# tlinford/raytracer-challenge-rs

Measured on AMD Instinct MI355X. Metric: Mrays/s (primary+secondary) on 1920×1080/1000-sphere/depth-5; 1→8 GPU scaling, higher is better.
Workload: dtype f64; 1 GPU; c3: 1920x1080, floor plane + 1000 random spheres (splitmix64 seed 0x5EED0003), 1 light, reflect+refract depth 5; width=1920, height=1080, spheres=1000, depth=5, rays_per_frame=14667325, parallelism=1 GPU: wavefront pipeline; batches of 8 frames on 4 streams, frames_in_flight=32, batch=8, render_streams_n=4, render_streams=raw

## Files before the change

### raytracer-challenge-rs_amd/csrc/pybind/rtamd_py.cpp

```cpp
#include <pybind11/numpy.h>
#include <pybind11/operators.h>
#include <pybind11/pybind11.h>
#include <pybind11/stl.h>

#include <algorithm>
#include <cstring>
#include <thread>

#include "../host/obj_parser.hpp"
#include "../host/rt_world.hpp"
#include "../host/scene_parser.hpp"

namespace py = pybind11;
using namespace rt;

static py::dict stats_dict(const rt_stats& s) {
  py::dict d;
  d["rays_primary"] = s.rays_primary;
  d["rays_reflect"] = s.rays_reflect;
  d["rays_refract"] = s.rays_refract;
  d["rays_shadow"] = s.rays_shadow;
  d["sphere_tests"] = s.sphere_tests;
  d["plane_tests"] = s.plane_tests;
  if (s.sphere_disc_ge0 == RT_STATS_NOT_COUNTED) d["sphere_disc_ge0"] = py::none();
  else d["sphere_disc_ge0"] = s.sphere_disc_ge0;
  d["other_tests"] = s.other_tests;
  d["ms_kernel"] = s.ms_kernel;
  d["ms_total"] = s.ms_total;
  d["rays_shadow_traced"] = s.rays_shadow_traced;
  d["sphere_tests_executed"] = s.sphere_tests_executed;
  d["box_tests_executed"] = s.box_tests_executed;
  d["exhaustive"] = (bool)s.exhaustive;
  return d;
}

static uint32_t render_flags(bool want_stats, const py::object& exhaustive) {
  const bool ex = exhaustive.is_none() ? want_stats : exhaustive.cast<bool>();
  return ex ? (uint32_t)RT_RENDER_EXHAUSTIVE : 0u;
}

static py::bytes pod_bytes(const void* p, size_t n) { return py::bytes((const char*)p, n); }

static py::array_t<double> check_rays(py::array_t<double, py::array::c_style | py::array::forcecast> a,
                                      size_t width) {
  if (a.ndim() != 2 || (size_t)a.shape(1) != width)
    throw std::invalid_argument("expected an (n, " + std::to_string(width) + ") float64 array");
  return a;
}

static void parallel_copy(char* dst, const char* src, size_t n) {
  const size_t kMin = (size_t)4 << 20;
  const unsigned nt = n < kMin ? 1u : (unsigned)std::min<size_t>(8, std::max(1u, std::thread::hardware_concurrency() / 2));
  if (nt <= 1) {
    std::memcpy(dst, src, n);
    return;
  }
  const size_t part = ((n + nt - 1) / nt + 4095) & ~(size_t)4095;
  std::vector<std::thread> pool;
  unsigned t = 1;
  try {
    for (; t < nt && t * part < n; ++t)
      pool.emplace_back([=] { std::memcpy(dst + t * part, src + t * part, std::min(part, n - t * part)); });
  } catch (...) {
  }
  for (unsigned u = t; u < nt && u * part < n; ++u) std::memcpy(dst + u * part, src + u * part, std::min(part, n - u * part));
  std::memcpy(dst, src, std::min(part, n));
  for (std::thread& th : pool) th.join();
}

extern "C" int rtamd_tuning_set(const char* key, int value);
extern "C" int rtamd_stream_create(int cu_masked, void** out);
extern "C" int rtamd_nccl_unique_id(unsigned char* out, size_t size);
extern "C" int rtamd_nccl_comm_init(int nranks, const unsigned char* id, size_t size, int rank, int device,
                                    int timeout_ms, void** comm);
extern "C" int rtamd_nccl_comm_abort(void* comm);
extern "C" int rtamd_nccl_gather_f64(const double* send, double* recv, size_t count, int root, void* comm, void* stream);
extern "C" int rtamd_nccl_comm_destroy(void* comm);
extern "C" int rtamd_wf_profile(const rt_scene* s, int enable, double out[40]);
extern "C" int rtamd_wf_gen_counts(const rt_scene* s, unsigned* out, int max);
extern "C" int rtamd_pngz_kernel_times(const double* d_rgb, uint32_t width, uint32_t height, uint8_t* d_out, size_t cap,
                                       float* ms, void* stream);
extern "C" int rtamd_wf_plan(const rt_scene* s, long long out[16]);
extern "C" int rtamd_csg_plan(const rt_scene* s, long long out[6]);
extern "C" int rtamd_scene_tuning_set(const rt_scene* s, const char* key, int value);
extern "C" int rtamd_render_shard_host(const rt_scene* scene, const rt_camera_desc* camera, uint32_t max_depth,
                                       uint32_t aa_samples, uint32_t row_block, uint32_t shard, uint32_t n_shards,
                                       double* out_rgb, rt_stats* stats);

static py::object child_object(const GroupChild& c) {
  if (c.shape) return py::cast(*c.shape);
  if (c.group) return py::cast(*c.group);
  return py::cast(*c.csg);
}

PYBIND11_MODULE(_rtamd, m) {
  m.doc() = "MI355X-native render path of raytracer-challenge-rs (host API over the C-ABI)";
  py::register_exception<RtError>(m, "RtError");
  m.attr("EPSILON") = EPSILON;
  m.attr("ABI_VERSION") = RT_ABI_VERSION;
  m.def("equal", &equal);
  m.def("device_count", &rt_device_count);
  m.def("abi_version", &rt_abi_version);

  py::class_<Point>(m, "Point")
      .def(py::init<double, double, double>())
      .def_static("origin", &Point::origin)
      .def_readwrite("x", &Point::x).def_readwrite("y", &Point::y).def_readwrite("z", &Point::z)
      .def("__eq__", [](const Point& a, const Point& b) { return a == b; })
      .def("__add__", [](const Point& p, const Vector& v) { return p + v; })
      .def("__sub__", [](const Point& a, const Point& b) { return a - b; })
      .def("__sub__", [](const Point& p, const Vector& v) { return p - v; })
      .def("tuple", [](const Point& p) { return py::make_tuple(p.x, p.y, p.z); })
      .def("__repr__", [](const Point& p) { return "Point(" + std::to_string(p.x) + ", " + std::to_string(p.y) + ", " + std::to_string(p.z) + ")"; });
  py::class_<Vector>(m, "Vector")
      .def(py::init<double, double, double>())
      .def_readwrite("x", &Vector::x).def_readwrite("y", &Vector::y).def_readwrite("z", &Vector::z)
      .def("magnitude", &Vector::magnitude)
      .def("normalize", &Vector::normalize)
      .def("reflect", &Vector::reflect)
      .def("__eq__", [](const Vector& a, const Vector& b) { return a == b; })
      .def("__add__", [](const Vector& a, const Vector& b) { return a + b; })
      .def("__sub__", [](const Vector& a, const Vector& b) { return a - b; })
      .def("__neg__", [](const Vector& a) { return -a; })
      .def("__mul__", [](const Vector& a, double s) { return a * s; })
      .def("tuple", [](const Vector& p) { return py::make_tuple(p.x, p.y, p.z); })
      .def("__repr__", [](const Vector& p) { return "Vector(" + std::to_string(p.x) + ", " + std::to_string(p.y) + ", " + std::to_string(p.z) + ")"; });
  m.def("dot", &dot);
  m.def("cross", &cross);
  py::class_<Color>(m, "Color")
      .def(py::init<double, double, double>())
      .def_static("black", &Color::black)
      .def_static("white", &Color::white)
      .def_readwrite("red", &Color::red).def_readwrite("green", &Color::green).def_readwrite("blue", &Color::blue)
      .def("__eq__", [](const Color& a, const Color& b) { return a == b; })
      .def("tuple", [](const Color& c) { return py::make_tuple(c.red, c.green, c.blue); })
      .def("__repr__", [](const Color& c) { return "Color(" + std::to_string(c.red) + ", " + std::to_string(c.green) + ", " + std::to_string(c.blue) + ")"; });
  py::class_<Ray>(m, "Ray")
      .def(py::init<const Point&, const Vector&>())
      .def_readwrite("origin", &Ray::origin)
      .def_readwrite("direction", &Ray::direction)
      .def("position", &Ray::position)
      .def("transform", [](const Ray& r, const Matrix& mm) { return transform(r, mm); });

  py::class_<Matrix>(m, "Matrix")
      .def(py::init<int, int>())
      .def_static("identity", &Matrix::identity)
      .def_static("from_rows", [](const std::vector<std::vector<double>>& rows) {
        int r = (int)rows.size(), c = r ? (int)rows[0].size() : 0;
        Matrix mm(r, c);
        for (int i = 0; i < r; ++i) {
          if ((int)rows[i].size() != c) throw std::invalid_argument("ragged rows");
          for (int j = 0; j < c; ++j) mm(i, j) = rows[i][j];
        }
        return mm;
      })
      .def("rows", &Matrix::rows)
      .def("columns", &Matrix::columns)
      .def("__getitem__", [](const Matrix& mm, std::pair<int, int> ij) {
        if (ij.first < 0 || ij.first >= mm.rows() || ij.second < 0 || ij.second >= mm.columns())
          throw py::index_error();
        return mm(ij.first, ij.second);
      })
      .def("__setitem__", [](Matrix& mm, std::pair<int, int> ij, double v) {
        if (ij.first < 0 || ij.first >= mm.rows() || ij.second < 0 || ij.second >= mm.columns())
          throw py::index_error();
        mm(ij.first, ij.second) = v;
      })
      .def("transpose", &Matrix::transpose)
      .def("determinant", &Matrix::determinant)
      .def("submatrix", &Matrix::submatrix)
      .def("minor", &Matrix::minor)
      .def("cofactor", &Matrix::cofactor)
      .def("is_invertible", &Matrix::is_invertible)
      .def("inverse", [](const Matrix& mm) {
        if (!mm.is_invertible()) throw RtError(RT_ERR_NOT_INVERTIBLE, "matrix is not invertible");
        return mm.inverse();
      })
      .def("translate", &Matrix::translate)
      .def("scale", &Matrix::scale)
      .def("rotate_x", &Matrix::rotate_x)
      .def("rotate_y", &Matrix::rotate_y)
      .def("rotate_z", &Matrix::rotate_z)
      .def("shear", &Matrix::shear)
      .def("__eq__", [](const Matrix& a, const Matrix& b) { return a == b; })
      .def("__mul__", [](const Matrix& a, const Matrix& b) { return a * b; })
      .def("__mul__", [](const Matrix& a, const Point& p) { return a * p; })
      .def("__mul__", [](const Matrix& a, const Vector& v) { return a * v; })
      .def("to_list", [](const Matrix& mm) {
        std::vector<double> v(mm.data(), mm.data() + mm.rows() * mm.columns());
        return v;
      });
  m.def("translation", &translation);
  m.def("scaling", &scaling);
  m.def("rotation_x", &rotation_x);
  m.def("rotation_y", &rotation_y);
  m.def("rotation_z", &rotation_z);
  m.def("shearing", &shearing);
  m.def("view_transform", &view_transform);

  py::class_<Pattern>(m, "Pattern")
      .def_readonly("kind", &Pattern::kind)
      .def_readwrite("a", &Pattern::a)
      .def_readwrite("b", &Pattern::b)
      .def_readonly("transform", &Pattern::transform)
      .def_readonly("transform_inverse", &Pattern::transform_inverse)
      .def("set_transform", &Pattern::set_transform);
  m.def("test_pattern", &test_pattern);
  m.def("stripe_pattern", &stripe_pattern);
  m.def("gradient_pattern", &gradient_pattern);
  m.def("ring_pattern", &ring_pattern);
  m.def("checkers_pattern", &checkers_pattern);

  py::class_<Material>(m, "Material")
      .def(py::init<>())
      .def_readwrite("color", &Material::color)
      .def_readwrite("ambient", &Material::ambient)
      .def_readwrite("diffuse", &Material::diffuse)
      .def_readwrite("specular", &Material::specular)
      .def_readwrite("shininess", &Material::shininess)
      .def_readwrite("reflective", &Material::reflective)
      .def_readwrite("transparency", &Material::transparency)
      .def_readwrite("refractive_index", &Material::refractive_index)
      .def_readonly("has_pattern", &Material::has_pattern)
      .def_readonly("pattern", &Material::pattern)
      .def("set_pattern", &Material::set_pattern)
      .def("copy", [](const Material& mm) { return mm; });

  py::class_<PointLight>(m, "PointLight")
      .def(py::init<const Point&, const Color&>())
      .def_readwrite("position", &PointLight::position)
      .def_readwrite("intensity", &PointLight::intensity);

  py::class_<Shape>(m, "Shape")
      .def_readonly("kind", &Shape::kind)
      .def_readwrite("material", &Shape::material)
      .def_readwrite("minimum", &Shape::minimum)
      .def_readwrite("maximum", &Shape::maximum)
      .def_readwrite("closed", &Shape::closed)
      .def_readonly("transform", &Shape::transform)
      .def_readonly("transform_inverse", &Shape::transform_inverse)
      .def("transform_inverse_transpose", &Shape::transform_inverse_transpose)
      .def("set_transform", &Shape::set_transform)
      .def("set_material", &Shape::set_material)
      .def("no_shadow", &Shape::no_shadow)
      .def("has_shadow", &Shape::has_shadow)
      .def("get_bounds", [](const Shape& s) { return s.bbox; })
      .def("parent_space_bounds", &Shape::parent_space_bounds)
      .def_readonly("p1", &Shape::p1).def_readonly("p2", &Shape::p2).def_readonly("p3", &Shape::p3)
      .def_readonly("n1", &Shape::n1).def_readonly("n2", &Shape::n2).def_readonly("n3", &Shape::n3)
      .def_readonly("e1", &Shape::e1).def_readonly("e2", &Shape::e2).def_readonly("normal", &Shape::normal)
      .def("desc_bytes", [](const Shape& s) { rt_shape_desc d = to_desc(s); return pod_bytes(&d, sizeof d); });
  py::class_<Group>(m, "Group")
      .def(py::init<>())
      .def("add_child", [](Group& g, const Shape& s) { g.add_child(s); })
      .def("add_child", [](Group& g, const Group& c) { g.add_child(c); })
      .def("add_child", [](Group& g, const Csg& c) { g.add_child(c); })
      .def("set_transform", &Group::set_transform)
      .def("set_material", &Group::set_material)
      .def_readonly("transform", &Group::transform)
      .def_readonly("transform_inverse", &Group::transform_inverse)
      .def_readonly("material", &Group::material)
      .def("n_children", [](const Group& g) { return g.children.size(); })
      .def("child", [](const Group& g, size_t i) -> py::object {
        return child_object(g.children.at(i));
      })
      .def("get_bounds", [](const Group& g) { return g.bbox; })
      .def("parent_space_bounds", &Group::parent_space_bounds)
      .def("divide", &Group::divide, py::arg("threshold"));
  py::enum_<Operation>(m, "Operation")
      .value("Union", Operation::Union).value("Intersection", Operation::Intersection)
      .value("Difference", Operation::Difference);
  py::class_<Csg>(m, "Csg")
      .def(py::init([](Operation op, py::object l, py::object r) {
        auto child = [](py::object o) -> GroupChild {
          if (py::isinstance<Shape>(o)) return make_child(o.cast<const Shape&>());
          if (py::isinstance<Group>(o)) return make_child(o.cast<const Group&>());
          if (py::isinstance<Csg>(o)) return make_child(o.cast<const Csg&>());
          throw std::invalid_argument("Csg: left / right must be a Shape, a Group or a Csg");
        };
        const GroupChild a = child(l), b = child(r);
        auto with_left = [&](auto& lv) {
          if (b.shape) return Csg(op, lv, *b.shape);
          if (b.group) return Csg(op, lv, *b.group);
          return Csg(op, lv, *b.csg);
        };
        if (a.shape) return with_left(*a.shape);
        if (a.group) return with_left(*a.group);
        return with_left(*a.csg);
      }), py::arg("operation"), py::arg("left"), py::arg("right"))
      .def_property_readonly("operation", [](const Csg& c) { return c.operation; })
      .def_property_readonly("left", [](const Csg& c) { return child_object(c.left); })
      .def_property_readonly("right", [](const Csg& c) { return child_object(c.right); })
      .def("set_transform", &Csg::set_transform)
      .def("set_material", &Csg::set_material)
      .def_readonly("transform", &Csg::transform)
      .def_readonly("transform_inverse", &Csg::transform_inverse)
      .def_readonly("material", &Csg::material)
      .def("get_bounds", [](const Csg& c) { return c.bbox; })
      .def("parent_space_bounds", &Csg::parent_space_bounds)
      .def("divide", &Csg::divide, py::arg("threshold"));
  py::class_<BoundingBox>(m, "BoundingBox")
      .def(py::init<>())
      .def(py::init<const Point&, const Point&>())
      .def_readwrite("min", &BoundingBox::min)
      .def_readwrite("max", &BoundingBox::max)
      .def("add_point", &BoundingBox::add_point)
      .def("add_bounding_box", &BoundingBox::add_box)
      .def("contains_point", &BoundingBox::contains_point)
      .def("contains_bounding_box", &BoundingBox::contains_box)
      .def("transform", &BoundingBox::transform)
      .def("intersects", &BoundingBox::intersects)
      .def("split", &BoundingBox::split);
  m.def("Sphere", &Sphere);
  m.def("glass_sphere", &glass_sphere);
  m.def("Plane", &Plane);
  m.def("Cube", &Cube);
  m.def("Cylinder", &Cylinder, py::arg("minimum") = -std::numeric_limits<double>::infinity(),
        py::arg("maximum") = std::numeric_limits<double>::infinity(), py::arg("closed") = false);
  m.def("Triangle", &Triangle, py::arg("p1"), py::arg("p2"), py::arg("p3"));
  m.def("SmoothTriangle", &SmoothTriangle, py::arg("p1"), py::arg("p2"), py::arg("p3"), py::arg("n1"), py::arg("n2"),
        py::arg("n3"));
  py::class_<ObjParser>(m, "ObjParser")
      .def(py::init<>())
      .def("parse", &ObjParser::parse)
      .def("parse_line", &ObjParser::parse_line)
      .def_readonly("ignored", &ObjParser::ignored)
      .def_readonly("vertices", &ObjParser::vertices)
      .def_readonly("normals", &ObjParser::normals)
      .def("group", [](const ObjParser& p, const std::string& name) { return p.group(name); })
      .def("group_names", &ObjParser::group_names)
      .def("as_group", &ObjParser::as_group);
  m.def("parse_obj_file", &parse_obj_file, py::arg("path"));
  m.def("parse_obj_string", &parse_obj_string, py::arg("text"));
  m.def("Cone", &Cone, py::arg("minimum") = -std::numeric_limits<double>::infinity(),
        py::arg("maximum") = std::numeric_limits<double>::infinity(), py::arg("closed") = false);

  py::enum_<AASamples>(m, "AASamples")
      .value("X1", AASamples::X1).value("X2", AASamples::X2).value("X4", AASamples::X4)
      .value("X8", AASamples::X8).value("X16", AASamples::X16);
  py::class_<RenderOpts>(m, "RenderOpts")
      .def("num_threads", &RenderOpts::num_threads)
      .def("aa_samples", &RenderOpts::aa_samples)
      .def_property_readonly("samples", [](const RenderOpts& o) { return (int)o.samples; });

  py::class_<Canvas>(m, "Canvas")
      .def(py::init<size_t, size_t>())
      .def("width", &Canvas::width)
      .def("height", &Canvas::height)
      .def("get_pixel", &Canvas::get_pixel)
      .def("set_pixel", &Canvas::set_pixel)
      .def("to_ppm", [](const Canvas& c) { return py::bytes(c.to_ppm()); })
      .def("to_png", [](const Canvas& c) { return py::bytes(c.to_png()); })
      .def("save", &Canvas::save, py::arg("path"))
      .def("to_png_deflate", [](const Canvas& c) { return py::bytes(c.to_png_deflate()); })
      .def("save_compressed", &Canvas::save_compressed, py::arg("path"))
      .def("to_numpy", [](const Canvas& c) {
        py::array_t<double> a({(py::ssize_t)c.height(), (py::ssize_t)c.width(), (py::ssize_t)3});
        std::memcpy(a.mutable_data(), c.data(), c.width() * c.height() * 3 * sizeof(double));
        return a;
      });
  m.def("canvas_to_ppm", [](py::array_t<double, py::array::c_style | py::array::forcecast> rgb) {
    if (rgb.ndim() != 3 || rgb.shape(2) != 3) throw std::invalid_argument("expected (h, w, 3)");
    size_t len = 0;
    const uint32_t h = (uint32_t)rgb.shape(0), w = (uint32_t)rgb.shape(1);
    const size_t bound = (size_t)12 * w * h + h + 32;
    PyObject* obj = PyBytes_FromStringAndSize(nullptr, (Py_ssize_t)bound);
    if (!obj) throw py::error_already_set();
    int rc;
    {
      py::gil_scoped_release nogil;
      rc = rt_canvas_to_ppm(rgb.data(), w, h, PyBytes_AS_STRING(obj), bound, &len);
    }
    if (rc != RT_OK) {
      Py_DECREF(obj);
      check(rc, "rt_canvas_to_ppm");
    }
    if (_PyBytes_Resize(&obj, (Py_ssize_t)len) != 0) throw py::error_already_set();
    return py::reinterpret_steal<py::bytes>(obj);
  });
  m.def("canvas_to_ppm_device", [](uintptr_t d_rgb, uint32_t w, uint32_t h, uintptr_t d_out, size_t cap,
                                   uintptr_t stream) {
    size_t len = 0;
    {
      py::gil_scoped_release nogil;
      check(rt_canvas_to_ppm_device((const double*)d_rgb, w, h, (char*)d_out, cap, &len, (void*)stream),
// ... 172 lines not shown
      .def_property_readonly("field_of_view", &Camera::field_of_view)
      .def("ray_for_pixel", &Camera::ray_for_pixel)
      .def("desc_bytes", [](const Camera& c) { return pod_bytes(&c.desc(), sizeof(rt_camera_desc)); })
      .def("render", [](const Camera& c, const World& w, unsigned max_depth, bool want_stats, py::object exhaustive) {
        rt_stats st{};
        Canvas* out;
        const uint32_t flags = render_flags(want_stats, exhaustive);
        {
          py::gil_scoped_release nogil;
          out = new Canvas(c.render(w, max_depth, want_stats ? &st : nullptr, flags));
        }
        return py::make_tuple(std::unique_ptr<Canvas>(out), stats_dict(st));
      }, py::arg("world"), py::arg("max_depth") = 5, py::arg("want_stats") = true, py::arg("exhaustive") = py::none())
      .def("render_ppm", [](const Camera& c, const World& w, unsigned max_depth, unsigned aa_samples, bool want_stats) {
        rt_stats st{};
        py::object out;
        {
          py::gil_scoped_release nogil;
          c.render_ppm_with(w, max_depth, aa_samples, want_stats ? &st : nullptr, [&](const char* p, size_t n) {
            char* dst = nullptr;
            {
              py::gil_scoped_acquire gil;
              PyObject* b = PyBytes_FromStringAndSize(nullptr, (Py_ssize_t)n);
              if (!b) throw py::error_already_set();
              out = py::reinterpret_steal<py::object>(b);
              dst = PyBytes_AS_STRING(b);
            }
            parallel_copy(dst, p, n);
          });
        }
        return py::make_tuple(out, stats_dict(st));
      }, py::arg("world"), py::arg("max_depth") = 5, py::arg("aa_samples") = 1, py::arg("want_stats") = false)
      .def("render_ppm_into", [](const Camera& c, const World& w, py::buffer out, unsigned max_depth,
                                 unsigned aa_samples) {
        py::buffer_info bi = out.request(true);
        if (bi.ndim != 1 || bi.itemsize != 1) throw std::invalid_argument("expected a writable 1-D byte buffer");
        size_t len = 0;
        int rc;
        {
          py::gil_scoped_release nogil;
          rc = rt_render_ppm(w.scene(), &c.desc(), max_depth, aa_samples, (char*)bi.ptr, (size_t)bi.size, &len,
                             nullptr);
        }
        check(rc, "rt_render_ppm");
        return len;
      }, py::arg("world"), py::arg("out"), py::arg("max_depth") = 5, py::arg("aa_samples") = 1)
      .def("render_png", [](const Camera& c, const World& w, unsigned max_depth, unsigned aa_samples, bool want_stats) {
        rt_stats st{};
        py::object out;
        {
          py::gil_scoped_release nogil;
          c.render_png_with(w, max_depth, aa_samples, want_stats ? &st : nullptr, [&](const char* p, size_t n) {
            char* dst = nullptr;
            {
              py::gil_scoped_acquire gil;
              PyObject* b = PyBytes_FromStringAndSize(nullptr, (Py_ssize_t)n);
              if (!b) throw py::error_already_set();
              out = py::reinterpret_steal<py::object>(b);
              dst = PyBytes_AS_STRING(b);
            }
            parallel_copy(dst, p, n);
          });
        }
        return py::make_tuple(out, stats_dict(st));
      }, py::arg("world"), py::arg("max_depth") = 5, py::arg("aa_samples") = 1, py::arg("want_stats") = false)
      .def("render_png_into", [](const Camera& c, const World& w, py::buffer out, unsigned max_depth,
                                 unsigned aa_samples) {
        py::buffer_info bi = out.request(true);
        if (bi.ndim != 1 || bi.itemsize != 1) throw std::invalid_argument("expected a writable 1-D byte buffer");
        size_t len = 0;
        int rc;
        {
          py::gil_scoped_release nogil;
          rc = rt_render_png(w.scene(), &c.desc(), max_depth, aa_samples, (uint8_t*)bi.ptr, (size_t)bi.size, &len,
                             nullptr);
        }
        check(rc, "rt_render_png");
        return len;
      }, py::arg("world"), py::arg("out"), py::arg("max_depth") = 5, py::arg("aa_samples") = 1)
      .def("render_png_deflate", [](const Camera& c, const World& w, unsigned max_depth, unsigned aa_samples,
                                    bool want_stats) {
        rt_stats st{};
        py::object out;
        {
          py::gil_scoped_release nogil;
          c.render_png_deflate_with(w, max_depth, aa_samples, want_stats ? &st : nullptr, [&](const char* p, size_t n) {
            py::gil_scoped_acquire gil;
            out = py::bytes(p, n);
          });
        }
        return py::make_tuple(out, stats_dict(st));
      }, py::arg("world"), py::arg("max_depth") = 5, py::arg("aa_samples") = 1, py::arg("want_stats") = false)
      .def("render_png_deflate_into", [](const Camera& c, const World& w, py::buffer out, unsigned max_depth,
                                         unsigned aa_samples) {
        py::buffer_info bi = out.request(true);
        if (bi.ndim != 1 || bi.itemsize != 1) throw std::invalid_argument("expected a writable 1-D byte buffer");
        size_t len = 0;
        int rc;
        {
          py::gil_scoped_release nogil;
          rc = rt_render_png_deflate(w.scene(), &c.desc(), max_depth, aa_samples, (uint8_t*)bi.ptr, (size_t)bi.size,
                                     &len, nullptr);
        }
        check(rc, "rt_render_png_deflate");
        return len;
      }, py::arg("world"), py::arg("out"), py::arg("max_depth") = 5, py::arg("aa_samples") = 1)
      .def_readwrite("render_opts", &Camera::render_opts, py::return_value_policy::reference_internal)
      .def("render_multithreaded", [](const Camera& c, const World& w, unsigned max_depth, bool want_stats,
                                      py::object exhaustive) {
        rt_stats st{};
        Canvas* out;
        const uint32_t flags = render_flags(want_stats, exhaustive);
        {
          py::gil_scoped_release nogil;
          out = new Canvas(c.render_multithreaded(w, max_depth, want_stats ? &st : nullptr, flags));
        }
        return py::make_tuple(std::unique_ptr<Canvas>(out), stats_dict(st));
      }, py::arg("world"), py::arg("max_depth") = 5, py::arg("want_stats") = true, py::arg("exhaustive") = py::none())
      .def("render_shard_device", [](const Camera& c, const World& w, unsigned max_depth, unsigned row_block,
                                     unsigned shard, unsigned n_shards, uintptr_t d_out, uintptr_t stream,
                                     bool want_stats, unsigned aa_samples, py::object exhaustive) {
        rt_stats st{};
        int rc;
        const uint32_t flags = render_flags(want_stats, exhaustive);
        {
          py::gil_scoped_release nogil;
          rc = rt_render_shard_device_ex(w.scene(), &c.desc(), max_depth, aa_samples, row_block, shard, n_shards,
                                         flags, (double*)d_out, (void*)stream, want_stats ? &st : nullptr);
        }
        check(rc, "rt_render_shard_device");
        return stats_dict(st);
      }, py::arg("world"), py::arg("max_depth"), py::arg("row_block"), py::arg("shard"), py::arg("n_shards"),
         py::arg("d_out"), py::arg("stream") = 0, py::arg("want_stats") = false, py::arg("aa_samples") = 1,
         py::arg("exhaustive") = py::none())
      .def("render_multi", [](const Camera& c, std::vector<World*> worlds, unsigned max_depth, unsigned row_block,
                              unsigned aa_samples, bool want_stats) {
        std::vector<rt_scene*> sc;
        for (size_t i = 0; i < worlds.size(); ++i) sc.push_back(const_cast<rt_scene*>(worlds[i]->scene((int)i)));
        Canvas* out = new Canvas(c.hsize(), c.vsize(), Canvas::Uninit{});
        rt_stats st{};
        int rc;
        {
          py::gil_scoped_release nogil;
          rc = rt_render_multi(sc.data(), (int)sc.size(), &c.desc(), max_depth, aa_samples, row_block, out->data(),
                               want_stats ? &st : nullptr);
        }
        if (rc != RT_OK) { delete out; check(rc, "rt_render_multi"); }
        return py::make_tuple(std::unique_ptr<Canvas>(out), stats_dict(st));
      }, py::arg("worlds"), py::arg("max_depth") = 5, py::arg("row_block") = 8, py::arg("aa_samples") = 1,
         py::arg("want_stats") = true);
  m.def("shard_rows", &rt_shard_rows);
  m.def("host_buffer", [](size_t bytes) {
    void* p = rt_host_buffer_alloc(bytes);
    if (!p) throw RtError(RT_ERR_HOST, std::string("rt_host_buffer_alloc: ") + rt_last_error());
    py::capsule owner(p, [](void* q) { rt_host_buffer_free(q); });
    return py::array_t<uint8_t>({(py::ssize_t)bytes}, {(py::ssize_t)1}, (uint8_t*)p, owner);
  }, py::arg("bytes"));
  m.def("_render_shard_host", [](const World& w, const Camera& c, unsigned max_depth, unsigned row_block,
                                 unsigned shard, unsigned n_shards,
                                 py::array_t<double, py::array::c_style> out, unsigned aa_samples, bool want_stats) {
    if (out.ndim() != 3 || (size_t)out.shape(0) != c.vsize() || (size_t)out.shape(1) != c.hsize() || out.shape(2) != 3)
      throw std::invalid_argument("expected a (vsize, hsize, 3) float64 canvas");
    double* p = out.mutable_data();
    rt_stats st{};
    int rc;
    {
      py::gil_scoped_release nogil;
      rc = rtamd_render_shard_host(w.scene(), &c.desc(), max_depth, aa_samples, row_block, shard, n_shards, p,
                                   want_stats ? &st : nullptr);
    }
    check(rc, "rtamd_render_shard_host");
    return stats_dict(st);
  }, py::arg("world"), py::arg("camera"), py::arg("max_depth"), py::arg("row_block"), py::arg("shard"),
     py::arg("n_shards"), py::arg("out"), py::arg("aa_samples") = 1, py::arg("want_stats") = false);
  m.def("render_frames_device", [](const World& w, std::vector<const Camera*> cams, unsigned max_depth,
                                   unsigned row_block, unsigned shard, unsigned n_shards, std::vector<uintptr_t> d_outs,
                                   uintptr_t stream, bool want_stats, unsigned aa_samples) {
    if (cams.size() != d_outs.size()) throw std::invalid_argument("one device buffer per camera");
    std::vector<rt_camera_desc> descs;
    for (const Camera* c : cams) descs.push_back(c->desc());
    std::vector<double*> outs;
    for (uintptr_t p : d_outs) outs.push_back((double*)p);
    rt_stats st{};
    int rc;
    {
      py::gil_scoped_release nogil;
      rc = rt_render_frames_device(w.scene(), descs.data(), (uint32_t)descs.size(), max_depth, aa_samples, row_block,
                                   shard, n_shards, outs.data(), (void*)stream, want_stats ? &st : nullptr);
    }
    check(rc, "rt_render_frames_device");
    return stats_dict(st);
  }, py::arg("world"), py::arg("cameras"), py::arg("max_depth"), py::arg("row_block"), py::arg("shard"),
     py::arg("n_shards"), py::arg("d_outs"), py::arg("stream") = 0, py::arg("want_stats") = false,
     py::arg("aa_samples") = 1);
  m.def("pattern_rows", &rt_pattern_rows);
  m.def("render_block_pattern_device", [](const World& w, std::vector<const Camera*> cams, unsigned max_depth,
                                          unsigned row_block, unsigned period, uint64_t mask,
                                          std::vector<uintptr_t> d_outs, uintptr_t stream, bool want_stats,
                                          unsigned aa_samples, bool exhaustive) {
    if (cams.size() != d_outs.size()) throw std::invalid_argument("one device buffer per camera");
    std::vector<rt_camera_desc> descs;
    for (const Camera* c : cams) descs.push_back(c->desc());
    std::vector<double*> outs;
    for (uintptr_t p : d_outs) outs.push_back((double*)p);
    rt_stats st{};
    int rc;
    {
      py::gil_scoped_release nogil;
      rc = rt_render_block_pattern_device(w.scene(), descs.data(), (uint32_t)descs.size(), max_depth, aa_samples,
                                          row_block, period, mask, exhaustive ? RT_RENDER_EXHAUSTIVE : 0u,
                                          outs.data(), (void*)stream, want_stats ? &st : nullptr);
    }
    check(rc, "rt_render_block_pattern_device");
    return stats_dict(st);
  }, py::arg("world"), py::arg("cameras"), py::arg("max_depth"), py::arg("row_block"), py::arg("period"),
     py::arg("mask"), py::arg("d_outs"), py::arg("stream") = 0, py::arg("want_stats") = false,
     py::arg("aa_samples") = 1, py::arg("exhaustive") = false);

  py::register_exception<SceneParserError>(m, "SceneParserError");
  py::register_exception<yaml::ParseError>(m, "YamlError");
  py::class_<SceneParser>(m, "SceneParser")
      .def(py::init<>())
      .def("load_file", &SceneParser::load_file)
      .def("load_str", &SceneParser::load_str, py::arg("text"), py::arg("name") = "<string>")
      .def_readonly("messages", &SceneParser::messages)
      .def_property_readonly("camera", [](const SceneParser& p) -> py::object {
        if (!p.scene().camera) return py::none();
        return py::cast(*p.scene().camera);
      })
      .def_property_readonly("lights", [](const SceneParser& p) { return p.scene().lights; })
      .def_property_readonly("shapes", [](const SceneParser& p) { return p.scene().shapes; })
      .def_property_readonly("materials", [](const SceneParser& p) { return p.scene().materials; })
      .def_property_readonly("transforms", [](const SceneParser& p) { return p.scene().transforms; })
      .def("build_world", &SceneParser::build_world)
      .def("render", [](const SceneParser& p, unsigned max_depth) {
        rt_stats st{};
        Canvas* out;
        {
          py::gil_scoped_release nogil;
          out = new Canvas(p.render(max_depth, &st));
        }
        return py::make_tuple(std::unique_ptr<Canvas>(out), stats_dict(st));
      }, py::arg("max_depth") = 5)
      .def("render_to", &SceneParser::render_to, py::arg("path"), py::arg("max_depth") = 5,
           py::arg("compress") = false);
  m.def("_wf_gen_counts", [](const World& w) {
    unsigned o[66] = {0};
    const int n = rtamd_wf_gen_counts(w.scene(), o, 66);
    if (n < 0) check(n, "wf_gen_counts");
    py::list l;
    for (int i = 0; i < n; ++i) l.append(o[i]);
    return l;
  }, py::arg("world"));
  m.def("_wf_profile", [](const World& w, int enable, bool read) {
    double o[40] = {0};
    check(rtamd_wf_profile(w.scene(), enable, read ? o : nullptr), "wf_profile");
    py::dict d;
    if (read) {
      const char* cls[5] = {"primary", "closest", "shadow", "prep", "combine"};
      py::dict ms, rays, disc;
      for (int i = 0; i < 5; ++i) ms[cls[i]] = o[i];
      for (int i = 0; i < 3; ++i) { rays[cls[i]] = o[5 + i]; disc[cls[i]] = o[8 + i]; }
      d["ms"] = ms; d["rays"] = rays; d["disc"] = disc;
      d["n_diag"] = o[11]; d["n_gen"] = o[12]; d["n_planes"] = o[13]; d["n_lights"] = o[14];
      d["n_quads"] = o[15];
      py::dict tests, boxes;
      for (int i = 0; i < 3; ++i) { tests[cls[i]] = o[16 + i]; boxes[cls[i]] = o[19 + i]; }
      d["tests"] = tests; d["boxes"] = boxes; d["bvh"] = (bool)o[22]; d["n_bvh_nodes"] = o[23]; d["bvh_depth"] = o[24];
      d["n_obvh_nodes"] = o[25]; d["n_other_culled"] = o[26];
      d["lb_res"] = o[27]; d["lb_items"] = o[28];
      py::dict shr, sht;
      shr["primary"] = o[29]; shr["closest"] = o[30]; sht["primary"] = o[31]; sht["closest"] = o[32];
      d["shadow_rays_in"] = shr; d["shadow_tests_in"] = sht; d["fused"] = (bool)o[33];
      d["n_bvh_wide"] = (int)o[34]; d["wide_stack"] = (int)o[35];
      d["n_lbvh_nodes"] = (int)o[36]; d["n_line_culled"] = (int)o[37];
      d["lane_primary"] = (int)o[38]; d["lane_secondary"] = (int)o[39];
    }
    return d;
  }, py::arg("world"), py::arg("enable") = -1, py::arg("read") = true);
  m.def("_wf_plan", [](const World& w) {
    long long o[16] = {0};
    check(rtamd_wf_plan(w.scene(), o), "wf_plan");
    py::dict d;
    const char* which[2] = {"primary", "secondary"};
    for (int i = 0; i < 2; ++i) {
      py::dict p;
      p["lane"] = (int)o[4 * i];
      p["lds_flags"] = (int)o[4 * i + 1];
      p["lds_spheres"] = (o[4 * i + 1] & 1) != 0;
      p["lds_deltas"] = (o[4 * i + 1] & 2) != 0;
      p["n_top"] = o[4 * i + 2];
      p["dyn"] = o[4 * i + 3];
      d[which[i]] = p;
    }
    py::dict t;
    t["records"] = o[8]; t["depth"] = o[9]; t["nodes"] = o[10]; t["ran"] = o[11] != 0;
    d["triangles"] = t;
    d["n_tris"] = o[12];
    d["n_csg_units"] = o[13];
    d["n_alias_members"] = o[14];
    d["n_alias_classes"] = o[15];
    return d;
  }, py::arg("world"));
  m.def("_csg_plan", [](const World& w) {
    long long o[6] = {0};
    check(rtamd_csg_plan(w.scene(), o), "csg_plan");
    py::dict d;
    d["units"] = o[0]; d["records"] = o[1]; d["remainder"] = o[2];
    d["nodes"] = o[3]; d["depth"] = o[4]; d["ran"] = o[5] != 0;
    return d;
  }, py::arg("world"));
  m.def("_tuning_set", [](const std::string& k, int v) { check(rtamd_tuning_set(k.c_str(), v), "tuning"); });
  m.def("_nccl_unique_id", []() {
    std::string id(128, '\0');
    check(rtamd_nccl_unique_id((unsigned char*)&id[0], id.size()), "nccl unique id");
    return py::bytes(id);
  });
  m.def("_nccl_comm_init", [](int nranks, py::bytes id, int rank, int device, int timeout_ms) {
    std::string s = id;
    void* comm = nullptr;
    int rc;
    {
      py::gil_scoped_release nogil;
      rc = rtamd_nccl_comm_init(nranks, (const unsigned char*)s.data(), s.size(), rank, device, timeout_ms, &comm);
    }
    check(rc, "nccl comm init");
    return (uintptr_t)comm;
  }, py::arg("nranks"), py::arg("id"), py::arg("rank"), py::arg("device"), py::arg("timeout_ms") = 60000);
  m.def("_nccl_comm_abort", [](uintptr_t comm) { check(rtamd_nccl_comm_abort((void*)comm), "nccl comm abort"); });
  m.def("_nccl_gather_f64", [](uintptr_t send, uintptr_t recv, size_t count, int root, uintptr_t comm, uintptr_t stream) {
    check(rtamd_nccl_gather_f64((const double*)send, (double*)recv, count, root, (void*)comm, (void*)stream), "nccl gather");
  });
  m.def("_nccl_comm_destroy", [](uintptr_t comm) { check(rtamd_nccl_comm_destroy((void*)comm), "nccl comm destroy"); });
  m.def("_stream_create", [](bool cu_masked) {
    void* st = nullptr;
    check(rtamd_stream_create(cu_masked ? 1 : 0, &st), "stream");
    return (uintptr_t)st;
  });
}
```

### raytracer-challenge-rs_amd/csrc/rt_api.cpp

```cpp
#include "rt_api_internal.hpp"
#include "rt_pow.hpp"

namespace rtapi {

thread_local std::string g_err;
int g_bvh_leaf = 0;
int g_bvh_ct = 70;
int g_lb_res = -1;
constexpr int kCsgHierMinDefault = 16;
int g_csg_hier_min = kCsgHierMinDefault;
int g_csg_wide_all = 0;
std::mutex g_tune_mu;
WfTuning g_tune_defaults;

namespace {
std::mutex g_pin_mu;
std::vector<std::pair<void*, size_t>> g_pin_live, g_pin_free;
size_t g_pin_free_bytes = 0;
constexpr size_t kPinPoolBytes = (size_t)1 << 30;
}

bool pinned_block(const void* p, size_t n) {
  std::lock_guard<std::mutex> lk(g_pin_mu);
  for (const auto& b : g_pin_live)
    if ((const char*)p >= (const char*)b.first && (const char*)p + n <= (const char*)b.first + b.second) return true;
  return false;
}

}

using namespace rtapi;

extern "C" __attribute__((visibility("hidden"))) int rtamd_fail(int code, const char* msg) noexcept {
  try {
    g_err = msg ? msg : "";
  } catch (...) {
    g_err.clear();
  }
  return code;
}

extern "C" {

const char* rt_last_error(void) { return g_err.c_str(); }

int rtamd_wf_profile(const rt_scene* cs, int enable, double out[40]) {
  if (!cs) return fail(RT_ERR_INVALID_ARGUMENT, "null scene");
  rt_scene* s = const_cast<rt_scene*>(cs);
  std::lock_guard<std::mutex> lk(s->mu);
  if (enable >= 0) {
    s->prof_on = enable != 0;
    s->prof_mask = enable > 1 ? (enable >> 1) : (1 << WF_NCLASS) - 1;
    for (rt_scene::WfSlot& w : s->wfs) w.wf->set_profiling(s->prof_on, s->prof_mask);
  }
  if (out) {
    RT_DEVICE(s->device);
    WfProfile p{};
    double ms_sum[WF_NCLASS] = {};
    size_t frames = 0;
    for (rt_scene::WfSlot& w : s->wfs) {
      WfProfile q;
      RT_HIP(w.wf->last_profile(&q));
      const size_t f = w.wf->profiled_frames();
      for (int c = 0; c < WF_NCLASS; ++c) ms_sum[c] += q.ms[c] * (double)(f > 1 ? f : 1);
      frames += f > 1 ? f : (f == 1 ? 1 : 0);
      if (&w == s->last_wf) p = q;
    }
    for (int c = 0; c < WF_NCLASS; ++c) p.ms[c] = frames ? ms_sum[c] / (double)frames : 0.0;
    for (int i = 0; i < 5; ++i) out[i] = p.ms[i];
    for (int i = 0; i < 3; ++i) { out[5 + i] = p.rays[i]; out[8 + i] = p.disc[i]; }
    out[11] = s->dev.n_diag; out[12] = s->dev.n_gen; out[13] = s->dev.n_planes;
    out[14] = s->dev.n_lights; out[15] = s->dev.n_quads;
    for (int i = 0; i < 3; ++i) {
      out[16 + i] = p.bvh ? p.tests[i] : p.rays[i] * s->dev.n_diag;
      out[19 + i] = p.boxes[i];
    }
    out[22] = p.bvh;
    out[23] = s->dev.n_bvh;
    out[24] = s->dev.bvh_depth;
    out[25] = s->dev.n_obvh;
    out[26] = s->dev.n_orec;
    out[27] = s->dev.lb_cells ? s->dev.lb_res : 0;
    out[28] = s->dev.lb_cells ? s->dev.lb_n_items : 0;
    for (int i = 0; i < 2; ++i) { out[29 + i] = p.sh_rays[i]; out[31 + i] = p.sh_tests[i]; }
    out[33] = p.fused;
    out[34] = s->dev.bvhw ? s->dev.n_bvhw : 0;
    out[35] = s->dev.bvhw ? s->dev.bvhw_stack : 0;
    out[36] = s->dev.n_lbvh;
    out[37] = s->dev.n_lrec;
    out[38] = s->last_wf ? p.lane_primary : -1;
    out[39] = s->last_wf ? p.lane_secondary : -1;
  }
  return RT_OK;
}

int rtamd_wf_plan(const rt_scene* cs, long long out[16]) {
  if (!cs || !out) return fail(RT_ERR_INVALID_ARGUMENT, "null scene or output");
  rt_scene* s = const_cast<rt_scene*>(cs);
  std::lock_guard<std::mutex> lk(s->mu);
  const WfImagePlan none{};
  const WfImagePlan* pl[2] = {s->last_wf ? &s->last_wf->wf->plan_primary() : &none,
                              s->last_wf ? &s->last_wf->wf->plan_secondary() : &none};
  for (int i = 0; i < 2; ++i) {
    out[4 * i] = pl[i]->lane;
    out[4 * i + 1] = (long long)pl[i]->lds_flags;
    out[4 * i + 2] = (long long)pl[i]->n_top;
    out[4 * i + 3] = (long long)pl[i]->dyn;
  }
  out[8] = s->dev.n_tbvh > 0 ? s->dev.n_trec : 0;
  out[9] = s->dev.tbvh_depth;
  out[10] = s->dev.n_tbvh;
  out[11] = s->dev.n_tbvh > 0 && (pl[0]->lane >= 0 || pl[1]->lane >= 0) ? 1 : 0;
  out[12] = s->dev.n_tris;
  out[13] = s->dev.n_csg_units;
  out[14] = s->dev.n_alias_rec;
  out[15] = s->dev.n_alias_cls;
  return RT_OK;
}

int rtamd_csg_plan(const rt_scene* cs, long long out[6]) {
  if (!cs || !out) return fail(RT_ERR_INVALID_ARGUMENT, "null scene or output");
  rt_scene* s = const_cast<rt_scene*>(cs);
  std::lock_guard<std::mutex> lk(s->mu);
  const bool fused =
      s->last_wf && (s->last_wf->wf->plan_primary().lane >= 0 || s->last_wf->wf->plan_secondary().lane >= 0);
  out[0] = s->dev.n_csg_units;
  out[1] = s->dev.n_ubvh > 0 ? s->dev.n_urec : 0;
  out[2] = s->dev.n_fx_units;
  out[3] = s->dev.n_ubvh;
  out[4] = s->dev.ubvh_depth;
  out[5] = s->dev.n_ubvh > 0 && fused ? 1 : 0;
  return RT_OK;
}

int rtamd_wf_gen_counts(const rt_scene* cs, unsigned* out, int max) {
  if (!cs || !out || max < 0) return fail(RT_ERR_INVALID_ARGUMENT, "null scene or output");
  rt_scene* s = const_cast<rt_scene*>(cs);
  std::lock_guard<std::mutex> lk(s->mu);
  if (!s->last_wf) return 0;
  RT_DEVICE(s->device);
  std::vector<unsigned> rays;
  RT_HIP(s->last_wf->wf->gen_counts(rays));
  const int n = std::min<int>((int)rays.size(), max);
  for (int i = 0; i < n; ++i) out[i] = rays[(size_t)i];
  return n;
}

int rtamd_tuning_set(const char* key, int value) {
  return guarded([&]() -> int {
  if (key && std::strcmp(key, "lb_res") == 0) {
    if (value < -1 || value > 512) return fail(RT_ERR_INVALID_ARGUMENT, "lb_res must be in [-1, 512]");
    g_lb_res = value;
    return RT_OK;
  }
  if (key && std::strcmp(key, "bvh_ct") == 0) {
    if (value < 1 || value > 10000) return fail(RT_ERR_INVALID_ARGUMENT, "bvh_ct must be in [1, 10000]");
    g_bvh_ct = value;
    return RT_OK;
  }
  if (key && std::strcmp(key, "bvh_leaf") == 0) {
    if (value < 0 || value > kBvhLeafMax) return fail(RT_ERR_INVALID_ARGUMENT, "bvh_leaf must be in [0, 127]");
    g_bvh_leaf = value;
    return RT_OK;
  }
  if (key && std::strcmp(key, "csg_hier_min") == 0) {
    if (value < 0 || value > 65536)
      return fail(RT_ERR_INVALID_ARGUMENT, "csg_hier_min must be in [1, 65536], or 0 for the default");
    g_csg_hier_min = value ? value : kCsgHierMinDefault;
    return RT_OK;
  }
  if (key && std::strcmp(key, "csg_wide_all") == 0) {
    if (value < 0 || value > 1) return fail(RT_ERR_INVALID_ARGUMENT, "csg_wide_all must be 0 or 1");
    g_csg_wide_all = value;
    return RT_OK;
  }
  std::lock_guard<std::mutex> lk(g_tune_mu);
  const int r = wf_tuning_apply(g_tune_defaults, key, value);
  if (r < 0) return fail(RT_ERR_INVALID_ARGUMENT, std::string("bad value for tuning key ") + key);
  if (r == 0) return fail(RT_ERR_INVALID_ARGUMENT, "unknown tuning key");
  return RT_OK;
  });
}
int rtamd_scene_tuning_set(const rt_scene* scene, const char* key, int value) {
  return guarded([&]() -> int {
  if (!scene) return fail(RT_ERR_INVALID_ARGUMENT, "null scene");
  rt_scene* s = const_cast<rt_scene*>(scene);
  std::lock_guard<std::mutex> lk(s->mu);
  const int r = wf_tuning_apply(s->tune, key, value);
  if (r < 0) return fail(RT_ERR_INVALID_ARGUMENT, std::string("bad value for tuning key ") + (key ? key : ""));
  if (r == 0) return fail(RT_ERR_INVALID_ARGUMENT, "unknown render-time tuning key (scene-creation keys: "
                                                   "rtamd_tuning_set before the scene is created)");
  return RT_OK;
  });
}
int rtamd_stream_create(int cu_masked, void** out) {
  if (!out) return fail(RT_ERR_INVALID_ARGUMENT, "null pointer");
  hipStream_t st = nullptr;
  if (cu_masked) {
    int dev = 0, n_cu = 0;
    RT_HIP(hipGetDevice(&dev));
    RT_HIP(hipDeviceGetAttribute(&n_cu, hipDeviceAttributeMultiprocessorCount, dev));
    std::vector<uint32_t> mask((size_t)(n_cu + 31) / 32, 0xFFFFFFFFu);
    RT_HIP(hipExtStreamCreateWithCUMask(&st, (uint32_t)mask.size(), mask.data()));
  } else {
    RT_HIP(hipStreamCreateWithFlags(&st, hipStreamNonBlocking));
  }
  *out = st;
  return RT_OK;
}
int rt_abi_version(void) { return RT_ABI_VERSION; }
size_t rt_sizeof_shape_desc(void) { return sizeof(rt_shape_desc); }
size_t rt_sizeof_camera_desc(void) { return sizeof(rt_camera_desc); }
size_t rt_sizeof_stats(void) { return sizeof(rt_stats); }
size_t rt_sizeof_node_desc(void) { return sizeof(rt_node_desc); }
static_assert(sizeof(rt_shape_desc) == 680 && sizeof(rt_camera_desc) == 160 && sizeof(rt_stats) == 112,
              "ABI struct sizes (include/rt_render.h, INTEGRATION.md)");

void* rt_host_buffer_alloc(size_t bytes) {
  if (bytes == 0) {
    g_err = "rt_host_buffer_alloc: zero bytes";
    return nullptr;
  }
  try {
    std::lock_guard<std::mutex> lk(g_pin_mu);
    for (size_t i = 0; i < g_pin_free.size(); ++i)
      if (g_pin_free[i].second >= bytes && g_pin_free[i].second <= bytes + bytes / 4) {
        const auto b = g_pin_free[i];
        g_pin_free.erase(g_pin_free.begin() + (long)i);
        g_pin_free_bytes -= b.second;
        g_pin_live.push_back(b);
        return b.first;
      }
    void* p = nullptr;
    if (hipHostMalloc(&p, bytes, hipHostMallocPortable | hipHostMallocMapped) != hipSuccess || !p) {
      (void)hipGetLastError();
      g_err = "rt_host_buffer_alloc: hipHostMalloc failed";
      return nullptr;
    }
    g_pin_live.emplace_back(p, bytes);
    return p;
  } catch (...) {
    g_err = "out of memory";
    return nullptr;
  }
}

void rt_host_buffer_free(void* p) {
  if (!p) return;
  try {
    std::lock_guard<std::mutex> lk(g_pin_mu);
    for (size_t i = 0; i < g_pin_live.size(); ++i)
      if (g_pin_live[i].first == p) {
        const auto b = g_pin_live[i];
        g_pin_live.erase(g_pin_live.begin() + (long)i);
        if (g_pin_free_bytes + b.second <= kPinPoolBytes) {
          g_pin_free.push_back(b);
          g_pin_free_bytes += b.second;
        } else {
          (void)hipHostFree(b.first);
        }
        return;
      }
  } catch (...) {
  }
}

int rt_scene_check(const rt_scene* scene) {
  return guarded([&]() -> int {
  if (!scene) return fail(RT_ERR_INVALID_ARGUMENT, "null scene");
  rt_scene* s = const_cast<rt_scene*>(scene);
  std::lock_guard<std::mutex> lk(s->mu);
  RT_DEVICE(s->device);
  for (rt_scene::WfSlot& w : s->wfs)
    if (w.done) RT_HIP(hipEventSynchronize(w.done));
  return check_faults(s);
  });
}

int rt_device_count(void) {
  return guarded([&]() -> int {
  int n = 0;
  if (hipGetDeviceCount(&n) != hipSuccess) return 0;
  return n;
  });
}

int rt_matrix_inverse(const double m[16], double out[16]) {
  return guarded([&]() -> int {
  if (!m || !out) return fail(RT_ERR_INVALID_ARGUMENT, "null pointer");
  rt::Matrix a = rt::Matrix::from_slice(4, 4, m);
  if (!a.is_invertible()) return fail(RT_ERR_NOT_INVERTIBLE, "matrix is not invertible (matrix.rs:139)");
  rt::Matrix inv = a.inverse();
  std::memcpy(out, inv.data(), 16 * sizeof(double));
  return RT_OK;
  });
}

int rt_camera_init(uint32_t hsize, uint32_t vsize, double field_of_view, const double transform[16],
                   rt_camera_desc* out) {
  return guarded([&]() -> int {
  if (!out || hsize == 0 || vsize == 0) return fail(RT_ERR_INVALID_ARGUMENT, "bad camera size");
  const double half_view = std::tan(field_of_view / 2.0);
  const double aspect = (double)hsize / (double)vsize;
  double half_width, half_height;
  if (aspect >= 1.0) {
    half_width = half_view;
    half_height = half_view / aspect;
  } else {
    half_width = half_view * aspect;
    half_height = half_view;
  }
  out->hsize = hsize;
  out->vsize = vsize;
  out->pixel_size = half_width * 2.0 / (double)hsize;
  out->half_width = half_width;
  out->half_height = half_height;
  if (transform) {
    int rc = rt_matrix_inverse(transform, out->inverse);
    if (rc != RT_OK) return rc;
  } else {
    rt::Matrix id = rt::Matrix::identity(4, 4);
    std::memcpy(out->inverse, id.data(), sizeof out->inverse);
  }
  return RT_OK;
  });
}

uint32_t rt_shard_rows(uint32_t vsize, uint32_t row_block, uint32_t shard, uint32_t n_shards) {
  if (row_block == 0 || n_shards == 0 || shard >= n_shards) return 0;
  uint32_t rows = 0;
  for (uint32_t blk = shard; (uint64_t)blk * row_block < vsize; blk += n_shards) {
    uint32_t y0 = blk * row_block;
    rows += std::min(row_block, vsize - y0);
  }
  return rows;
}

uint32_t rt_pattern_rows(uint32_t vsize, uint32_t row_block, uint32_t period, uint64_t mask) {
  if (row_block == 0 || !valid_pattern(period, mask)) return 0;
  uint32_t rows = 0;
  for (uint64_t blk = 0; blk * row_block < vsize; ++blk)
    if ((mask >> (blk % period)) & 1u) rows += std::min<uint32_t>(row_block, vsize - (uint32_t)(blk * row_block));
  return rows;
}

void rtamd_pow_host(const double* x, const double* y, size_t n, double* out) {
  for (size_t i = 0; i < n; ++i) out[i] = rtamd::pow_glibc(x[i], y[i]);
}
int rtamd_pow_device(const double* d_x, const double* d_y, size_t n, double* d_out, void* stream) {
  return guarded([&]() -> int {
  if (n >= (1ull << 31)) return fail(RT_ERR_INVALID_ARGUMENT, "batch too large");
  RT_HIP(launch_pow(d_x, d_y, (int)n, d_out, (hipStream_t)stream));
  RT_HIP(hipStreamSynchronize((hipStream_t)stream));
  return RT_OK;
  });
}

}
```

### raytracer-challenge-rs_amd/csrc/rt_render.cpp

```cpp
#include "rt_api_internal.hpp"

using namespace rtapi;

extern "C" {

int rt_render_shard_device(const rt_scene* scene, const rt_camera_desc* camera, uint32_t max_depth,
                           uint32_t aa_samples, uint32_t row_block, uint32_t shard, uint32_t n_shards,
                           double* d_out_rgb, void* stream, rt_stats* stats) {
  return guarded([&]() -> int {
  return rt_render_shard_device_ex(scene, camera, max_depth, aa_samples, row_block, shard, n_shards, 0, d_out_rgb,
                                   stream, stats);
  });
}

int rt_render_shard_device_ex(const rt_scene* scene, const rt_camera_desc* camera, uint32_t max_depth,
                              uint32_t aa_samples, uint32_t row_block, uint32_t shard, uint32_t n_shards,
                              uint32_t flags, double* d_out_rgb, void* stream, rt_stats* stats) {
  return guarded([&]() -> int {
  if (!scene || !camera || !d_out_rgb) return fail(RT_ERR_INVALID_ARGUMENT, "null pointer");
  if (row_block == 0 || n_shards == 0 || shard >= n_shards)
    return fail(RT_ERR_INVALID_ARGUMENT, "bad shard specification");
  if (camera->hsize == 0 || camera->vsize == 0) return fail(RT_ERR_INVALID_ARGUMENT, "empty camera");
  rt_scene* s = const_cast<rt_scene*>(scene);
  std::unique_lock<std::mutex> lk(s->mu);
  auto t0 = std::chrono::steady_clock::now();
  RT_DEVICE(s->device);
  const uint32_t rows = rt_shard_rows(camera->vsize, row_block, shard, n_shards);
  const uint64_t n_tasks = (uint64_t)rows * camera->hsize * aa_samples;
  if (n_tasks >= (1ull << 31)) return fail(RT_ERR_INVALID_ARGUMENT, "shard too large");
  hipStream_t st = (hipStream_t)stream;
  RenderCall call(&lk);
  call.flags = flags;
  call.stats = call.time = stats != nullptr;
  RenderResult r;
  int rc = run_render(s, WfJob::camera_shard(to_dev_camera(*camera), (uint32_t)n_tasks, aa_samples, max_depth,
                                             d_out_rgb, row_block, shard, n_shards), st, call, &r);
  if (rc != RT_OK) return rc;
  if (stats)
    fill_stats(stats, r.stats, r.ms,
               std::chrono::duration<double, std::milli>(std::chrono::steady_clock::now() - t0).count());
  return RT_OK;
  });
}

namespace {
int render_frames(const rt_scene* scene, const rt_camera_desc* cameras, uint32_t n_frames, uint32_t max_depth,
                  uint32_t aa_samples, uint32_t row_block, uint32_t shard, uint32_t n_shards, uint32_t blk_period,
                  uint64_t blk_mask, uint32_t flags, double* const* d_out_rgb, void* stream, rt_stats* stats) {
  if (!scene || (n_frames && (!cameras || !d_out_rgb))) return fail(RT_ERR_INVALID_ARGUMENT, "null pointer");
  if (row_block == 0 || n_shards == 0 || shard >= n_shards)
    return fail(RT_ERR_INVALID_ARGUMENT, "bad shard specification");
  if (blk_period && !valid_pattern(blk_period, blk_mask))
    return fail(RT_ERR_INVALID_ARGUMENT, "bad block pattern (period 1..64, a non-empty mask below 2^period)");
  if (!valid_aa(aa_samples)) return fail(RT_ERR_INVALID_ARGUMENT, "aa_samples must be 1, 2, 4, 8 or 16");
  for (uint32_t f = 0; f < n_frames; ++f) {
    if (!d_out_rgb[f]) return fail(RT_ERR_INVALID_ARGUMENT, "null pointer");
    if (cameras[f].hsize == 0 || cameras[f].vsize == 0) return fail(RT_ERR_INVALID_ARGUMENT, "empty camera");
    if (cameras[f].hsize != cameras[0].hsize || cameras[f].vsize != cameras[0].vsize)
      return fail(RT_ERR_INVALID_ARGUMENT, "the frames of a batch must share hsize and vsize");
  }
  if (n_frames == 0) {
    if (stats) std::memset(stats, 0, sizeof *stats);
    return RT_OK;
  }
  rt_scene* s = const_cast<rt_scene*>(scene);
  std::unique_lock<std::mutex> lk(s->mu);
  auto t0 = std::chrono::steady_clock::now();
  RT_DEVICE(s->device);
  const uint32_t rows = blk_period ? rt_pattern_rows(cameras[0].vsize, row_block, blk_period, blk_mask)
                                  : rt_shard_rows(cameras[0].vsize, row_block, shard, n_shards);
  const uint64_t per = (uint64_t)rows * cameras[0].hsize * aa_samples;
  const uint64_t padded = (per + 63) & ~(uint64_t)63;
  if (padded >= (1ull << 31)) return fail(RT_ERR_INVALID_ARGUMENT, "shard too large");
  hipStream_t st = (hipStream_t)stream;
  const bool batch = !stats && !(flags & RT_RENDER_EXHAUSTIVE) && fast_path(s) && per > 0;
  DevStats sum{};
  float ms_sum = 0.f;
  const uint32_t per_pass = (uint32_t)std::max<uint64_t>(1, std::min<uint64_t>(kMaxFrames, ((uint64_t)1 << 25) / std::max<uint64_t>(padded, 1)));
  RenderCall call(&lk);
  call.flags = flags;
  call.stats = call.time = stats != nullptr;
  for (uint32_t f0 = 0; f0 < n_frames;) {
    const uint32_t nf = batch ? std::min<uint32_t>(per_pass, n_frames - f0) : 1u;
    FrameTable tab{};
    for (uint32_t f = 0; f < nf; ++f) {
      tab.cam[f] = to_dev_camera(cameras[f0 + f]);
      tab.out[f] = d_out_rgb[f0 + f];
    }
    WfJob job = WfJob::camera_shard(tab.cam[0], (uint32_t)per, aa_samples, max_depth, tab.out[0], row_block, shard,
                                    n_shards);
    job.blk_period = blk_period;
    job.blk_mask = blk_mask;
    if (nf > 1) job.batch = &tab;
    job.n_frames = nf;
    RenderResult r;
    int rc = run_render(s, job, st, call, &r);
    if (rc != RT_OK) return rc;
    if (stats) {
      add_stats(sum, r.stats);
      ms_sum += r.ms;
    }
    f0 += nf;
  }
  if (stats)
    fill_stats(stats, sum, ms_sum, std::chrono::duration<double, std::milli>(std::chrono::steady_clock::now() - t0).count());
  return RT_OK;
}
}

int rt_render_frames_device(const rt_scene* scene, const rt_camera_desc* cameras, uint32_t n_frames,
                            uint32_t max_depth, uint32_t aa_samples, uint32_t row_block, uint32_t shard,
                            uint32_t n_shards, double* const* d_out_rgb, void* stream, rt_stats* stats) {
  return guarded([&]() -> int {
  return render_frames(scene, cameras, n_frames, max_depth, aa_samples, row_block, shard, n_shards, 0, 0, 0,
                       d_out_rgb, stream, stats);
  });
}

int rt_render_block_pattern_device(const rt_scene* scene, const rt_camera_desc* cameras, uint32_t n_frames,
                                   uint32_t max_depth, uint32_t aa_samples, uint32_t row_block, uint32_t period,
                                   uint64_t mask, uint32_t flags, double* const* d_out_rgb, void* stream,
                                   rt_stats* stats) {
  return guarded([&]() -> int {
  if (period == 0) return fail(RT_ERR_INVALID_ARGUMENT, "bad block pattern (period 1..64)");
  if (flags & ~(uint32_t)RT_RENDER_EXHAUSTIVE) return fail(RT_ERR_INVALID_ARGUMENT, "unknown render flags");
  return render_frames(scene, cameras, n_frames, max_depth, aa_samples, row_block, 0, 1, period, mask, flags,
                       d_out_rgb, stream, stats);
  });
}

}

namespace rtapi {
namespace {
struct BandPlan {
  int bands = 0;
  uint32_t rb = 0, nb = 0;
  uint32_t y0[kMaxBands + 1] = {};
  uint64_t mask[kMaxBands] = {};
};
bool plan_bands(const rt_scene* s, uint32_t H, BandPlan& p) {
  p.bands = std::max(2, std::min(kMaxBands, s->tune.bands));
  p.rb = (H + 63) / 64;
  p.nb = (H + p.rb - 1) / p.rb;
  if (p.nb < (uint32_t)p.bands * 2) return false;
  const uint32_t nb = p.nb;
  const int bands = p.bands;
  uint32_t b[kMaxBands + 1] = {};
  b[1] = std::max<uint32_t>(1, std::min<uint32_t>(nb - (uint32_t)bands + 1, (uint32_t)((uint64_t)nb * s->tune.band_pct / 100)));
  double wsum = 0.0, wk = 1.0;
  for (int k = 1; k < bands; ++k, wk *= s->tune.band_ratio / 100.0) wsum += wk;
  double acc = 0.0;
  wk = 1.0;
  for (int k = 2; k < bands; ++k, wk *= s->tune.band_ratio / 100.0) {
    acc += wk;
    const uint32_t at = b[1] + (uint32_t)((nb - b[1]) * acc / wsum + 0.5);
    b[k] = std::min<uint32_t>(nb - (uint32_t)(bands - k), std::max<uint32_t>(b[k - 1] + 1, at));
  }
  b[bands] = nb;
  const uint64_t all = nb == 64 ? ~0ull : ((1ull << nb) - 1ull);
  for (int k = 0; k <= bands; ++k) p.y0[k] = std::min(H, b[k] * p.rb);
  for (int k = 0; k < bands; ++k) {
    const uint64_t below_end = b[k + 1] >= 64 ? ~0ull : ((1ull << b[k + 1]) - 1ull);
    const uint64_t below_start = (1ull << b[k]) - 1ull;
    p.mask[k] = all & below_end & ~below_start;
  }
  return true;
}

struct BandRender {
  rt_scene* s;
  std::unique_lock<std::mutex>& lk;
  rt_scene::HostCtx* c;
  const BandPlan& p;
  hipStream_t st[kMaxBands] = {};
  PinGuard pins[kMaxBands];
  int n_enq = 0;
  BandRender(rt_scene* s_, std::unique_lock<std::mutex>& lk_, rt_scene::HostCtx* c_, const BandPlan& p_)
      : s(s_), lk(lk_), c(c_), p(p_) {
    for (PinGuard& g : pins) {
      g.s = s;
      g.lk = &lk;
    }
  }
  ~BandRender() {
    for (int k = 0; k < n_enq; ++k)
      if (hipStreamSynchronize(st[k]) != hipSuccess) (void)hipGetLastError();
    if (!lk.owns_lock()) lk.lock();
  }
  BandRender(const BandRender&) = delete;
  BandRender& operator=(const BandRender&) = delete;
  WfJob job(int k, const DevCamera& dc, uint32_t W, uint32_t aa, uint32_t max_depth) const {
    const uint32_t rows = p.y0[k + 1] - p.y0[k];
    return WfJob::block_pattern(dc, rows * W * aa, aa, max_depth, c->d_out + (size_t)p.y0[k] * W * 3, p.rb, p.nb,
                                p.mask[k]);
  }
  int open() {
    st[0] = c->stream;
    for (int k = 1; k < p.bands; ++k) {
      if (!c->band_stream[k - 1]) RT_HIP(hipStreamCreateWithFlags(&c->band_stream[k - 1], hipStreamNonBlocking));
      st[k] = c->band_stream[k - 1];
    }
    for (int k = 0; k < p.bands; ++k)
      if (!c->band_ev[k]) RT_HIP(hipEventCreateWithFlags(&c->band_ev[k], hipEventDisableTiming));
    return RT_OK;
  }
  int render(int k, const DevCamera& dc, uint32_t W, uint32_t aa, uint32_t max_depth) {
    if (k > 0) RT_HIP(hipStreamWaitEvent(st[k], c->band_ev[k - 1], 0));
    WfJob j = job(k, dc, W, aa, max_depth);
    if (s->tune.band_gen >= 0 && k + 1 < p.bands) {
      j.gen_ev = c->band_ev[k];
      j.gen_ev_g = s->tune.band_gen;
    }
    RenderCall call(&lk);
    call.keep_pin = &pins[k];
    call.sizing = &s->band_sizing;
    RenderResult r;
    n_enq = k + 1;
    int rc = run_render(s, j, st[k], call, &r);
    if (rc != RT_OK) return rc;
    if (!r.gen_ev_recorded) RT_HIP(hipEventRecord(c->band_ev[k], st[k]));
    return RT_OK;
  }
  int wait_all() {
    lk.unlock();
    hipError_t first = hipSuccess;
    for (int k = 0; k < n_enq; ++k) {
      const hipError_t e = hipStreamSynchronize(st[k]);
      if (e != hipSuccess && first == hipSuccess) first = e;
    }
    lk.lock();
    if (first != hipSuccess) return fail(RT_ERR_HIP, std::string("banded render: ") + hipGetErrorString(first));
    return RT_OK;
  }
};
}

int render_banded(rt_scene* s, std::unique_lock<std::mutex>& lk, rt_scene::HostCtx* c, const rt_camera_desc& cam,
                  uint32_t max_depth, uint32_t aa, double* out_rgb, bool host_ready) {
  const uint32_t W = cam.hsize, H = cam.vsize;
  BandPlan p;
  if (!plan_bands(s, H, p)) return RT_ERR_NO_DEVICE;
  const size_t bytes = (size_t)W * H * 3 * sizeof(double);
  bool registered = false;
  if (!host_ready && !pinned_block(out_rgb, bytes)) {
    if (s->tune.d2h != 1 || hipHostRegister(out_rgb, bytes, hipHostRegisterDefault) != hipSuccess) {
      (void)hipGetLastError();
      return RT_ERR_NO_DEVICE;
    }
    registered = true;
  }
  struct Unregister {
    void* p;
    bool on;
    ~Unregister() {
      if (on && hipHostUnregister(p) != hipSuccess) (void)hipGetLastError();
    }
  } unreg{out_rgb, registered};
  BandRender br(s, lk, c, p);
  int rc = br.open();
  if (rc != RT_OK) return rc;
  const DevCamera dc = to_dev_camera(cam);
  auto copy = [&](int k) -> int {
    const size_t off = (size_t)p.y0[k] * W * 3;
    RT_HIP(hipMemcpyAsync(out_rgb + off, c->d_out + off, (size_t)(p.y0[k + 1] - p.y0[k]) * W * 3 * sizeof(double),
                          hipMemcpyDeviceToHost, br.st[k]));
    return RT_OK;
  };
  for (int k = 0; k < p.bands; ++k) {
    if ((rc = br.render(k, dc, W, aa, max_depth)) != RT_OK) return rc;
    if ((rc = copy(k)) != RT_OK) return rc;
  }
  if ((rc = br.wait_all()) != RT_OK) return rc;
  for (int k = 0; k < p.bands; ++k) {
    bool over = false;
    if ((rc = settle(br.pins[k], s->band_sizing, &over)) != RT_OK) return rc;
    if (!over) continue;
    RenderCall again(&lk);
    again.sync = true;
    again.sizing = &s->band_sizing;
    if ((rc = run_render(s, br.job(k, dc, W, aa, max_depth), br.st[k], again)) != RT_OK) return rc;
    if ((rc = copy(k)) != RT_OK) return rc;
    lk.unlock();
    const hipError_t e = hipStreamSynchronize(br.st[k]);
    lk.lock();
    if (e != hipSuccess) return fail(RT_ERR_HIP, std::string("banded render: ") + hipGetErrorString(e));
  }
  return RT_OK;
}

}

extern "C" {

int rt_render_aa(const rt_scene* scene, const rt_camera_desc* camera, uint32_t max_depth, uint32_t aa_samples,
                 double* out_rgb, rt_stats* stats) {
  return guarded([&]() -> int {
  return rt_render_ex(scene, camera, max_depth, aa_samples, 0, out_rgb, stats);
  });
}

int rt_render_ex(const rt_scene* scene, const rt_camera_desc* camera, uint32_t max_depth, uint32_t aa_samples,
                 uint32_t flags, double* out_rgb, rt_stats* stats) {
  return guarded([&]() -> int {
  if (!scene || !camera || !out_rgb) return fail(RT_ERR_INVALID_ARGUMENT, "null pointer");
  if (camera->hsize == 0 || camera->vsize == 0) return fail(RT_ERR_INVALID_ARGUMENT, "empty camera");
  if (!valid_aa(aa_samples)) return fail(RT_ERR_INVALID_ARGUMENT, "aa_samples must be 1, 2, 4, 8 or 16");
  rt_scene* s = const_cast<rt_scene*>(scene);
  std::unique_lock<std::mutex> lk(s->mu);
  auto t0 = std::chrono::steady_clock::now();
  RT_DEVICE(s->device);
  const uint64_t n_pix = (uint64_t)camera->hsize * camera->vsize;
  if (n_pix * aa_samples >= (1ull << 31)) return fail(RT_ERR_INVALID_ARGUMENT, "canvas too large for one launch");
  CtxLease cx{s, lk};
  RT_TAKE_CTX(cx);
  int rc = ensure_dev_buffer(&cx.c->d_out, &cx.c->out_cap, n_pix * 3);
  if (rc != RT_OK) return rc;
  if (!stats && flags == 0 && s->tune.bands > 1 && fast_path(s) && n_pix * aa_samples >= ((uint64_t)1 << 20)) {
    rc = render_banded(s, lk, cx.c, *camera, max_depth, aa_samples, out_rgb);
    if (rc != RT_ERR_NO_DEVICE) return rc;
  }
  RenderCall call(&lk);
  call.flags = flags;
  call.stats = stats != nullptr;
  call.time = true;
  RenderResult r;
  rc = run_render(s, WfJob::camera_shard(to_dev_camera(*camera), (uint32_t)(n_pix * aa_samples), aa_samples, max_depth,
                                         cx.c->d_out, camera->vsize), cx.c->stream, call, &r);
  if (rc != RT_OK) return rc;
  const int d2h = s->tune.d2h;
  lk.unlock();
  if ((rc = copy_to_host(cx.c, d2h, out_rgb, cx.c->d_out, n_pix * 3 * sizeof(double), cx.c->stream)) != RT_OK)
    return rc;
  if (stats)
    fill_stats(stats, r.stats, r.ms,
               std::chrono::duration<double, std::milli>(std::chrono::steady_clock::now() - t0).count());
  return RT_OK;
  });
}

int rt_render_ppm(const rt_scene* scene, const rt_camera_desc* camera, uint32_t max_depth, uint32_t aa_samples,
                  char* out, size_t cap, size_t* out_len, rt_stats* stats) {
  return guarded([&]() -> int {
  if (!scene || !camera || !out_len) return fail(RT_ERR_INVALID_ARGUMENT, "null pointer");
  if (camera->hsize == 0 || camera->vsize == 0) return fail(RT_ERR_INVALID_ARGUMENT, "empty camera");
  if (!valid_aa(aa_samples)) return fail(RT_ERR_INVALID_ARGUMENT, "aa_samples must be 1, 2, 4, 8 or 16");
  if (camera->hsize > kPpmMaxWidth)
    return fail(RT_ERR_INVALID_ARGUMENT, "canvas wider than the device PPM encoder's row (use rt_canvas_to_ppm)");
  rt_scene* s = const_cast<rt_scene*>(scene);
  std::unique_lock<std::mutex> lk(s->mu);
  auto t0 = std::chrono::steady_clock::now();
  RT_DEVICE(s->device);
  const uint32_t W = camera->hsize, H = camera->vsize;
  const uint64_t n_pix = (uint64_t)W * H;
  if (n_pix * aa_samples >= (1ull << 31)) return fail(RT_ERR_INVALID_ARGUMENT, "canvas too large for one launch");
  CtxLease cx{s, lk};
  RT_TAKE_CTX(cx);
  rt_scene::HostCtx* c = cx.c;
  int rc = ensure_dev_buffer(&c->d_out, &c->out_cap, n_pix * 3);
  if (rc != RT_OK) return rc;
  const PpmHeader hd = ppm_header(W, H);
  const size_t bound = hd.n + (size_t)12 * n_pix + H;
  if (c->ppm_cap < bound) {
    if (c->d_ppm) (void)hipFree(c->d_ppm);
    c->d_ppm = nullptr;
    c->ppm_cap = 0;
    RT_HIP(hipMalloc(&c->d_ppm, bound));
    c->ppm_cap = bound;
  }
  if (c->ppm_rows_cap < H) {
    if (c->d_ppm_rows) (void)hipFree(c->d_ppm_rows);
    c->d_ppm_rows = nullptr;
    c->ppm_rows_cap = 0;
    RT_HIP(hipMalloc(&c->d_ppm_rows, (size_t)H * 4 + ((size_t)H + 1) * 8 + 8));
    c->ppm_rows_cap = H;
  }
  unsigned long long* d_off = (unsigned long long*)(((uintptr_t)c->d_ppm_rows + (size_t)H * 4 + 7) & ~(uintptr_t)7);
  if (!c->h_len) RT_HIP(hipHostMalloc((void**)&c->h_len, sizeof(unsigned long long), hipHostMallocDefault));
  struct Drain {
    hipStream_t st;
    ~Drain() {
      if (hipStreamSynchronize(st) != hipSuccess) (void)hipGetLastError();
    }
  } drain{c->stream};
  const WfJob job = WfJob::camera_shard(to_dev_camera(*camera), (uint32_t)(n_pix * aa_samples), aa_samples, max_depth,
                                        c->d_out, H);
  PinGuard pin(s, &lk);
  RenderCall call(&lk);
  call.stats = call.time = stats != nullptr;
  if (!stats) call.keep_pin = &pin;
  RenderResult r;
  if ((rc = run_render(s, job, c->stream, call, &r)) != RT_OK) return rc;
  auto encode = [&]() -> int {
    RT_HIP(ppm_encode_device(c->d_out, W, H, c->d_ppm, c->ppm_cap, (unsigned*)c->d_ppm_rows, d_off, hd, c->stream));
    RT_HIP(hipMemcpyAsync(c->h_len, d_off + H, sizeof(unsigned long long), hipMemcpyDeviceToHost, c->stream));
    lk.unlock();
    const hipError_t e = hipStreamSynchronize(c->stream);
// ... 388 lines not shown
```

### raytracer-challenge-rs_amd/csrc/rt_wavefront.hip

```cpp
#include "rt_wf_launch.hpp"

#include <algorithm>
#include <cstring>

#pragma clang fp contract(off)

namespace rtamd {

int wf_tuning_apply(WfTuning& t, const char* key, int value) {
  struct Knob {
    const char* name;
    int WfTuning::*field;
    int lo, hi;
  };
  static const Knob knobs[] = {
      {"accel", &WfTuning::accel, 0, 1},           {"skip_shadow", &WfTuning::skip_shadow, 0, 1},
      {"shadow_lb", &WfTuning::shadow_lb, 0, 1},   {"image", &WfTuning::image, 0, 3},
      {"treelet", &WfTuning::treelet, 0, 1},       {"treelet_deltas", &WfTuning::treelet_deltas, 0, 1},
      {"shadow_stream", &WfTuning::shadow_stream, 0, 2}, {"adaptive_block", &WfTuning::adaptive_block, 0, 1},
      {"prim_lane", &WfTuning::prim_lane, 0, 2},   {"arena_pct", &WfTuning::arena_pct, 1, 100},
      {"wide", &WfTuning::wide, 0, 1},
      {"lds_wide", &WfTuning::lds_wide, 0, 1},
      {"d2h", &WfTuning::d2h, 0, 1},               {"bands", &WfTuning::bands, 1, 4},
      {"band_pct", &WfTuning::band_pct, 5, 95},   {"band_gen", &WfTuning::band_gen, -1, 8},
      {"band_ratio", &WfTuning::band_ratio, 30, 100}, {"multi_gather", &WfTuning::multi_gather, 0, 1},
      {"own_sphere", &WfTuning::own_sphere, 0, 2}, {"spread", &WfTuning::spread, 0, 1}};
  if (!key) return 0;
  for (const Knob& k : knobs) {
    if (std::strcmp(key, k.name) != 0) continue;
    if (value < k.lo || value > k.hi || (k.field == &WfTuning::image && value == 2)) return -1;
    t.*(k.field) = value;
    return 1;
  }
  return 0;
}

static thread_local hipEvent_t t_ev_start = nullptr, t_ev_stop = nullptr;
static thread_local int t_ev_used = 0;

Wavefront::~Wavefront() {
  for (auto& g : gens_) {
    (void)hipFree(g.rays); (void)hipFree(g.hits); (void)hipFree(g.nodes); (void)hipFree(g.colors);
    (void)hipFree(g.shadow_nodes); (void)hipFree(g.geo); (void)hipFree(g.surf);
  }
  (void)hipFree(colors_); (void)hipFree(parents_); (void)hipFree(rays_[0]); (void)hipFree(rays_[1]);
  if (d_gtab_) (void)hipFree(d_gtab_);
  if (d_gsh_) (void)hipFree(d_gsh_);
  if (d_cnt_) (void)hipFree(d_cnt_);
  if (d_shard_) (void)hipFree(d_shard_);
  if (d_prim_) (void)hipFree(d_prim_);
  if (d_frames_) (void)hipFree(d_frames_);
  if (h_rec_) (void)hipHostFree(h_rec_);
  if (ev0_) (void)hipEventDestroy(ev0_);
  if (ev1_) (void)hipEventDestroy(ev1_);
  for (hipEvent_t e : fork_ev_)
    if (e) (void)hipEventDestroy(e);
  if (join_ev_) (void)hipEventDestroy(join_ev_);
  if (side_) (void)hipStreamDestroy(side_);
  for (hipEvent_t e : pev_) (void)hipEventDestroy(e);
}

hipError_t Wavefront::pmark(hipStream_t s, int cls, bool begin) {
  (void)s;
  if (!profiling_ || !(pmask_ & (1 << cls))) return hipSuccess;
  if (begin) {
    const size_t idx = 2 * pn_;
    while (pev_.size() <= idx + 1) {
      hipEvent_t e;
      WF_CHECK(hipEventCreate(&e));
      pev_.push_back(e);
    }
    if (pcls_.size() <= pn_) pcls_.resize(pn_ + 1);
    pcls_[pn_] = cls;
    t_ev_start = pev_[idx];
    t_ev_stop = pev_[idx + 1];
    t_ev_used = 0;
  } else {
    t_ev_start = t_ev_stop = nullptr;
    if (t_ev_used != 1) return hipErrorInvalidValue;
    ++pn_;
  }
  return hipSuccess;
}

hipError_t Wavefront::last_profile(WfProfile* out) {
  *out = WfProfile{};
  for (size_t i = 0; i < pn_; ++i) {
    WF_CHECK(hipEventSynchronize(pev_[2 * i + 1]));
    float ms = 0.f;
    WF_CHECK(hipEventElapsedTime(&ms, pev_[2 * i], pev_[2 * i + 1]));
    out->ms[pcls_[i]] += ms;
  }
  if (pframes_ > 1)
    for (int c = 0; c < WF_NCLASS; ++c) out->ms[c] /= (double)pframes_;
  WfCounters hc{};
  if (d_cnt_) WF_CHECK(hipMemcpy(&hc, d_cnt_, sizeof hc, hipMemcpyDeviceToHost));
  for (int c = 0; c < 3; ++c) {
    out->rays[c] = prof_rays_[c];
    out->disc[c] = (double)hc.disc(c);
    out->tests[c] = (double)hc.tests(c);
    out->boxes[c] = (double)hc.boxes(c);
  }
  if (last_fused_) {
    std::vector<unsigned> rays;
    WF_CHECK(last_counts(rays));
    out->rays[WF_PRIMARY] = rays.empty() ? 0.0 : (double)rays[0];
    double sec = 0.0;
    for (size_t g = 1; g < rays.size(); ++g) sec += (double)rays[g];
    out->rays[WF_CLOSEST] = sec;
  }
  for (int c = 0; c < 2; ++c) {
    out->sh_rays[c] = (double)hc.sh_rays(c);
    out->sh_tests[c] = (double)hc.sh_tests(c);
  }
  if (last_fused_) out->rays[WF_SHADOW] = out->sh_rays[0] + out->sh_rays[1];
  out->bvh = last_bvh_ ? 1 : 0;
  out->fused = last_fused_ ? 1 : 0;
  out->lane_primary = plan_primary_.lane;
  out->lane_secondary = plan_secondary_.lane;
  return hipSuccess;
}

template <typename T>
static hipError_t grow(T*& p, size_t& cap, size_t need) {
  need = std::max<size_t>(need, 1);
  if (cap >= need) return hipSuccess;
  (void)hipFree(p);
  p = nullptr;
  cap = 0;
  const size_t n = need + need / 8;
  WF_CHECK(hipMalloc(&p, n * sizeof(T)));
  cap = n;
  return hipSuccess;
}
hipError_t Wavefront::ensure_gen(size_t g, size_t slots, size_t n_lights, size_t list_slots) {
  if (gens_.size() <= g) gens_.resize(g + 1);
  WfGenBuf& b = gens_[g];
  WF_CHECK(grow(b.rays, b.cap_rays, slots));
  WF_CHECK(grow(b.colors, b.cap_colors, slots * 3));
  WF_CHECK(grow(b.hits, b.cap_hits, slots));
  WF_CHECK(grow(b.nodes, b.cap_nodes, slots));
  WF_CHECK(grow(b.geo, b.cap_geo, slots));
  WF_CHECK(grow(b.surf, b.cap_surf, slots * std::max<size_t>(n_lights, 1) * 3));
  WF_CHECK(grow(b.shadow_nodes, b.cap_list, list_slots));
  return hipSuccess;
}

hipError_t Wavefront::ensure_arenas(unsigned long long colors, unsigned long long parents, unsigned long long rays,
                                    bool exact) {
  auto fit = [&](auto*& p, unsigned long long& cap, unsigned long long need, size_t elem, int n_bufs) -> hipError_t {
    need = std::max<unsigned long long>(need, 1);
    if (exact ? cap == need : cap >= need) return hipSuccess;
    const unsigned long long n = exact ? need : need + need / 8;
    for (int k = 0; k < n_bufs; ++k) {
      (void)hipFree((&p)[k]);
      (&p)[k] = nullptr;
    }
    cap = 0;
    for (int k = 0; k < n_bufs; ++k) WF_CHECK(hipMalloc((void**)&(&p)[k], n * elem));
    cap = n;
    return hipSuccess;
  };
  WF_CHECK(fit(colors_, color_cap_, colors, 3 * sizeof(double), 1));
  WF_CHECK(fit(parents_, par_cap_, parents, sizeof(ParentRec), 1));
  WF_CHECK(fit(rays_[0], ray_cap_, rays, sizeof(WfRay), 2));
  return hipSuccess;
}

hipError_t Wavefront::take_overflow(bool* was) {
  *was = false;
  if (!h_rec_) return hipSuccess;
  volatile WfHostRec* r = h_rec_;
  if (!r->overflow) return hipSuccess;
  *was = true;
  const unsigned long long nc = r->need_colors, np = r->need_parents, nr = r->need_rays;
  r->overflow = 0;
  auto next = [](unsigned long long cap, unsigned long long need) {
    return need > cap ? std::max(need + need / 4, 2 * cap) : cap;
  };
  return ensure_arenas(next(color_cap_, nc), next(par_cap_, np), next(ray_cap_, nr), false);
}

void Wavefront::learn(WfSizing& sz) const {
  if (!h_rec_) return;
  const volatile WfHostRec* r = h_rec_;
  if (r->frames == 0) return;
  const unsigned n0 = r->n_real, ng = std::min<unsigned>((unsigned)r->n_gens, (unsigned)kMaxGen);
  if (n0 == 0 || ng == 0) return;
  double sum = 0.0, mx = 0.0;
  for (unsigned g = 0; g < ng; ++g) {
    const double c = (double)r->counts[g];
    if (g + 1 < ng) sum += c;
    mx = std::max(mx, c);
  }
  sz.rho = std::max(sz.rho, sum / n0);
  sz.mu = std::max(sz.mu, mx / n0);
}

hipError_t Wavefront::last_counts(std::vector<unsigned>& rays) {
  rays.clear();
  if (!lr_.fused) {
    rays = lr_.rays;
    return hipSuccess;
  }
  WF_CHECK(hipStreamSynchronize(lr_.stream));
  const volatile WfHostRec* r = h_rec_;
  const unsigned ng = std::min<unsigned>((unsigned)r->n_gens, (unsigned)kMaxGen);
  for (unsigned g = 0; g < ng; ++g) rays.push_back((unsigned)r->counts[g]);
  while (rays.size() > 1 && rays.back() == 0) rays.pop_back();
  return hipSuccess;
}

hipError_t Wavefront::ensure_side() {
  int dev = 0;
  WF_CHECK(hipGetDevice(&dev));
  if (side_ && side_dev_ == dev) return hipSuccess;
  if (side_) {
    WF_CHECK(hipStreamSynchronize(side_));
    (void)hipStreamDestroy(side_);
    for (hipEvent_t& e : fork_ev_)
      if (e) { (void)hipEventDestroy(e); e = nullptr; }
    if (join_ev_) { (void)hipEventDestroy(join_ev_); join_ev_ = nullptr; }
    side_ = nullptr;
  }
  WF_CHECK(hipStreamCreateWithFlags(&side_, hipStreamNonBlocking));
  for (hipEvent_t& e : fork_ev_) WF_CHECK(hipEventCreateWithFlags(&e, hipEventDisableTiming));
  WF_CHECK(hipEventCreateWithFlags(&join_ev_, hipEventDisableTiming));
  side_dev_ = dev;
  return hipSuccess;
}

hipError_t Wavefront::ensure_misc(size_t n_diag, unsigned n_frames) {
  if (!d_cnt_) WF_CHECK(hipMalloc(&d_cnt_, sizeof(WfCounters)));
  if (!h_rec_) {
    WF_CHECK(hipHostMalloc((void**)&h_rec_, sizeof(WfHostRec), hipHostMallocMapped));
    std::memset((void*)h_rec_, 0, sizeof(WfHostRec));
    WF_CHECK(hipHostGetDevicePointer((void**)&d_rec_, h_rec_, 0));
  }
  if (!d_gtab_) WF_CHECK(hipMalloc(&d_gtab_, (kMaxGen + 1) * sizeof(WfGenTab)));
  if (!d_gsh_) WF_CHECK(hipMalloc(&d_gsh_, kMaxGen * sizeof(unsigned)));
  if (!d_shard_) WF_CHECK(hipMalloc(&d_shard_, (size_t)kMaxGen * 2 * kShards * kShardStride * sizeof(unsigned)));
  if (!ev0_) WF_CHECK(hipEventCreate(&ev0_));
  if (!ev1_) WF_CHECK(hipEventCreate(&ev1_));
  if (n_frames > 1 && !d_frames_) WF_CHECK(hipMalloc(&d_frames_, sizeof(FrameTable)));
  const size_t np = (n_diag + 4) * n_frames;
  if (prim_cap_ < np) {
    if (d_prim_) (void)hipFree(d_prim_);
    d_prim_ = nullptr;
    WF_CHECK(hipMalloc(&d_prim_, np * sizeof(PrimRec)));
    prim_cap_ = np;
  }
  return hipSuccess;
}

static int trace_block(unsigned n, int adaptive) {
  if (!adaptive) return kTraceBlock;
  static int n_cu = 0;
  if (n_cu == 0) {
    int dev = 0;
    (void)hipGetDevice(&dev);
    (void)hipDeviceGetAttribute(&n_cu, hipDeviceAttributeMultiprocessorCount, dev);
    if (n_cu < 1) n_cu = 1;
  }
  const unsigned per = ((n + (unsigned)n_cu - 1) / (unsigned)n_cu + 63u) & ~63u;
  return (int)std::min<unsigned>(std::max<unsigned>(per, 64u), (unsigned)kTraceBlock);
}

#define WF_LAUNCH(kern, grid, block, lds, stream, ...)                                                  \
  do {                                                                                                 \
    if (t_ev_start) {                                                                                  \
      hipExtLaunchKernelGGL(kern, grid, block, lds, stream, t_ev_start, t_ev_stop, 0, __VA_ARGS__);    \
      ++t_ev_used;                                                                                     \
    } else {                                                                                           \
      hipLaunchKernelGGL(kern, grid, block, lds, stream, __VA_ARGS__);                                 \
    }                                                                                                  \
  } while (0)

template <typename K, typename... Args>
static hipError_t launch_timed(K kern, int block, size_t dyn, unsigned n, hipStream_t stream, const Args&... args) {
  if (t_ev_start) ++t_ev_used;
  return wf_launch(kern, block, dyn, n, stream, t_ev_start, t_ev_stop, args...);
}

template <bool QUADS, bool CSG = false, bool ALIAS = false>
static hipError_t launch_closest_exh(const DevScene& sc, const DevCamera& cam, const WfArgs& a, bool primary,
                                     bool lds_ok, unsigned n, hipStream_t stream, const WfTuning& tn) {
  const int tb = trace_block(n, tn.adaptive_block);
  if (primary)
    return launch_timed(wf_trace_closest<true, true, QUADS, 8, CSG, ALIAS>, tb, wf_lds_bytes(sc.n_diag, sc.n_gen, sc.n_planes, true),
                        n, stream, sc, cam, a);
  if (lds_ok)
    return launch_timed(wf_trace_closest<true, false, QUADS, 8, CSG, ALIAS>, tb,
                        wf_lds_bytes(sc.n_diag, sc.n_gen, sc.n_planes, false), n, stream, sc, cam, a);
  return launch_timed(wf_trace_closest<false, false, QUADS, 8, CSG, ALIAS>, tb, 0, n, stream, sc, cam, a);
}
template <bool QUADS, bool CSG = false, bool ALIAS = false>
static hipError_t launch_shadow_exh(const DevScene& sc, const WfArgs& a, bool lds_ok, hipStream_t stream,
                                    const WfTuning& tn) {
  const int tb = trace_block(a.n_shadow, tn.adaptive_block);
  if (lds_ok)
    return launch_timed(wf_trace_shadow<true, QUADS, 8, CSG, ALIAS>, tb, wf_lds_bytes(sc.n_diag, sc.n_gen, sc.n_planes, false),
                        a.n_shadow, stream, sc, a);
  return launch_timed(wf_trace_shadow<false, QUADS, 8, CSG, ALIAS>, tb, 0, a.n_shadow, stream, sc, a);
}

template <bool QUADS, bool TALLY, bool TRIS = false, bool CSG = false, bool ALIAS = false>
static hipError_t launch_fused_q(const DevScene& sc, const DevCamera& cam, WfArgs a, bool primary, unsigned n,
                                 hipStream_t stream, const WfTuning& tn, WfImagePlan* ran) {
  if (a.spread && !tn.adaptive_block) n = 1u << 30;
  const int tb = trace_block(n, tn.adaptive_block);
  const WfImagePlan plan = *ran = wf_plan_image(sc, tn, primary, a.use_lb != 0);
  a.lds_flags = plan.lds_flags;
  a.n_top = plan.n_top;
  const bool cam_rays = a.g == 0 && a.camera_mode;
#define RT_LDS(P, L, C) launch_timed(wf_trace_fused<P, QUADS, L, TALLY, C, TRIS, CSG, ALIAS>, tb, plan.dyn, n, stream, sc, cam, a)
  switch (plan.lane) {
    case kLaneWave: return RT_LDS(true, kLaneWave, true);
    case kLaneWideLds: return cam_rays ? RT_LDS(false, kLaneWideLds, true) : RT_LDS(false, kLaneWideLds, false);
    case kLanePair: return cam_rays ? RT_LDS(false, kLanePair, true) : RT_LDS(false, kLanePair, false);
  }
#undef RT_LDS
  if (t_ev_start) ++t_ev_used;
  return wf_launch_global(plan.lane, QUADS, TRIS, CSG, ALIAS, TALLY, cam_rays, sc, cam, a, plan.dyn, n, stream, tb, t_ev_start, t_ev_stop);
}
static hipError_t launch_fused(const DevScene& sc, const DevCamera& cam, const WfArgs& a, bool primary, unsigned n,
                               hipStream_t stream, bool tally, const WfTuning& tn, WfImagePlan* ran) {
  const bool quads = sc.n_fx_quads > 0 || sc.n_obvh > 0 || sc.n_lbvh > 0;
  if (sc.n_alias_rec > 0)
    return tally ? launch_fused_q<true, true, true, true, true>(sc, cam, a, primary, n, stream, tn, ran)
                 : launch_fused_q<true, false, true, true, true>(sc, cam, a, primary, n, stream, tn, ran);
  if (sc.n_csg_units > 0)
    return tally ? launch_fused_q<true, true, true, true>(sc, cam, a, primary, n, stream, tn, ran)
                 : launch_fused_q<true, false, true, true>(sc, cam, a, primary, n, stream, tn, ran);
  if (sc.n_tris > 0)
    return tally ? launch_fused_q<true, true, true>(sc, cam, a, primary, n, stream, tn, ran)
                 : launch_fused_q<true, false, true>(sc, cam, a, primary, n, stream, tn, ran);
  if (tally)
    return quads ? launch_fused_q<true, true>(sc, cam, a, primary, n, stream, tn, ran)
                 : launch_fused_q<false, true>(sc, cam, a, primary, n, stream, tn, ran);
  return quads ? launch_fused_q<true, false>(sc, cam, a, primary, n, stream, tn, ran)
               : launch_fused_q<false, false>(sc, cam, a, primary, n, stream, tn, ran);
}

WfArgs Wavefront::job_args(const WfJob& job, unsigned n0, unsigned frame_real) const {
  WfArgs a{};
  a.aa = job.aa;
  a.rows = frame_real / job.aa / (job.cam.hsize ? job.cam.hsize : 1);
  a.n_frames = job.n_frames; a.frame_rays = n0 / job.n_frames; a.frame_real = frame_real; a.frames = d_frames_;
  a.cnt = d_cnt_;
  a.prim = d_prim_;
  a.max_depth = job.max_depth;
  a.camera_mode = job.camera_mode() ? 1u : 0u;
  a.row_block = job.row_block; a.shard = job.shard; a.n_shards = job.n_shards;
  a.blk_period = job.blk_period; a.blk_mask = job.blk_period ? job.blk_mask : 0ull;
  return a;
}

hipError_t Wavefront::render(const DevScene& sc, const WfJob& job, hipStream_t stream, WfSizing& sz,
                             const WfTuning& tn, bool solo) {
  if (!wf_job_valid(job)) return hipErrorInvalidValue;
  const DevCamera& cam = job.cam;
  const bool camera_mode = job.camera_mode();
  const unsigned max_depth = job.max_depth, n_frames = job.n_frames, flags = job.flags;
  unsigned n0 = job.n0;
  gen_ev_done_ = false;
  WF_CHECK(ensure_misc((size_t)sc.n_diag, n_frames));
  const bool exhaustive = (flags & WF_EXHAUSTIVE) != 0;
  const bool count = (flags & WF_COUNT) != 0;
  const bool bvh = tn.accel != 0 && !exhaustive && (sc.n_bvh > 0 || sc.n_obvh > 0 || sc.n_lbvh > 0 || sc.n_tbvh > 0 ||
                                                      sc.n_ubvh > 0);
  const bool fused = bvh;
  const bool skip_shadow = !exhaustive && tn.skip_shadow != 0 && !(count && sc.n_groups > 0);
  const unsigned frame_real = n0;
  if (n_frames > 1) {
    if (!camera_mode || !fused || count || n0 == 0) return hipErrorInvalidValue;
    n0 = n_frames * ((n0 + 63u) & ~63u);
  }
  const bool use_prim = camera_mode && sc.n_diag > 0 &&
                        (fused || wf_lds_bytes(sc.n_diag, sc.n_gen, sc.n_planes, true) <= kFusedLdsLimit);
  {
    static_assert(sizeof(WfCounters) % 16 == 0, "WfCounters is zeroed in 16-B words");
    const unsigned n_a = (unsigned)(sizeof(WfCounters) / 16);
    const unsigned n_b = (unsigned)((size_t)(max_depth + 2) * 2 * kShards * kShardStride * sizeof(unsigned) / 16);
    const unsigned work = std::max<unsigned>(std::max(n_a, n_b), use_prim ? n_frames * ((unsigned)sc.n_diag + 4) : 0u);
    const FrameTable none{};
    WF_LAUNCH(wf_frame_init, dim3(std::min<unsigned>((work + 255) / 256, 256u)), dim3(256), 0, stream, sc, cam,
              d_prim_, use_prim ? 1u : 0u, (uint4*)d_cnt_, n_a, (uint4*)d_shard_, n_b, n_frames > 1 ? *job.batch : none,
              d_frames_, n_frames, fused ? d_gtab_ : (WfGenTab*)nullptr);
    WF_CHECK(hipGetLastError());
  }
  const bool timed = (flags & WF_TIME) != 0;
  if (timed) WF_CHECK(hipEventRecord(ev0_, stream));
  if (profiling_) pframes_ += n_frames;
  prof_rays_[0] = prof_rays_[1] = prof_rays_[2] = 0;
  last_bvh_ = bvh;
  last_fused_ = fused;
  plan_primary_ = plan_secondary_ = WfImagePlan{};
  lr_.stream = stream;
  lr_.fused = fused;
  if (fused)
    WF_CHECK(render_fast(sc, job, n0, frame_real, stream, sz, skip_shadow, tn));
  else
    WF_CHECK(render_exhaustive(sc, job, stream, skip_shadow, tn, solo));
  if (timed) WF_CHECK(hipEventRecord(ev1_, stream));
  lr_.L = (unsigned)sc.n_lights; lr_.n0 = n0; lr_.max_depth = max_depth;
  lr_.counted = count; lr_.exact_disc = !bvh && !skip_shadow; lr_.bvh = bvh;
  lr_.n_diag = (unsigned long long)sc.n_diag;
  lr_.n_gen = (unsigned long long)sc.n_gen + (unsigned long long)sc.n_csg_sph + (unsigned long long)sc.n_alias_sph;
  lr_.n_planes = (unsigned long long)sc.n_planes + (unsigned long long)sc.n_csg_planes + (unsigned long long)sc.n_alias_planes;
  lr_.n_quads = (unsigned long long)sc.n_quads + (unsigned long long)sc.n_tris + (unsigned long long)sc.n_csg_other +
                (unsigned long long)sc.n_alias_other;
  return hipSuccess;
}

static unsigned long long gen_slots(unsigned long long n) {
  const unsigned long long groups = ((n + 63) / 64 + kShardGroup - 1) / kShardGroup;
  return (unsigned long long)kShards * 128ull * kShardGroup * ((groups + kShards - 1) / kShards);
}

hipError_t Wavefront::render_fast(const DevScene& sc, const WfJob& job, unsigned n0, unsigned frame_real,
                                  hipStream_t stream, WfSizing& sz, bool skip_shadow, const WfTuning& tn) {
  const DevCamera& cam = job.cam;
  const bool camera_mode = job.camera_mode(), count = (job.flags & WF_COUNT) != 0;
  const unsigned aa = job.aa, max_depth = job.max_depth, n_frames = job.n_frames;
  double* const d_out = job.d_out;
  const bool averaged = aa > 1;
  const unsigned n_real = frame_real * n_frames;
  learn(sz);
  const unsigned D = max_depth;
  double c_bound = (double)n0, p_bound = 0.0, r_bound = camera_mode ? 0.0 : (double)n0;
  {
    double ng = (double)n0;
    for (unsigned g = 0; g < D; ++g) {
      const double s = (double)gen_slots((unsigned long long)std::min(ng, 4.0e9));
      c_bound += s;
      p_bound += s / 2.0;
      r_bound = std::max(r_bound, s);
      ng = std::min(ng * (double)sz.branch, 4.0e9);
      if (ng == 0.0) break;
    }
  }
  const double rho = sz.rho > 0.0 ? sz.rho : 8.0, mu = sz.mu > 0.0 ? sz.mu : 2.0;
  const double min_region = (double)gen_slots(1);
  const double c_learn = (double)n0 + 2.5 * rho * n_real + min_region * D;
  const double p_learn = 1.25 * rho * n_real + min_region / 2.0 * D;
  const double r_learn = std::max(camera_mode ? 0.0 : (double)n0, 2.5 * mu * n_real + min_region);
  double want_c = std::min(c_bound, c_learn), want_p = std::min(p_bound, p_learn), want_r = std::min(r_bound, r_learn);
  const bool squeeze = tn.arena_pct < 100 && tn.arena_pct != squeezed_pct_;
  squeezed_pct_ = tn.arena_pct;
  if (squeeze) {
    want_c = std::max((double)n0, want_c * tn.arena_pct / 100.0);
    want_p *= tn.arena_pct / 100.0;
    want_r = std::max(camera_mode ? 0.0 : (double)n0, want_r * tn.arena_pct / 100.0);
  }
  hipError_t ea = ensure_arenas((unsigned long long)want_c, (unsigned long long)want_p, (unsigned long long)want_r,
                                squeeze);
  const double floor_c = (double)n0 + min_region * D, floor_p = min_region / 2.0 * D;
  const double floor_r = std::max(camera_mode ? 0.0 : (double)n0, min_region);
  for (int k = 0; ea == hipErrorOutOfMemory && k < 16 && (want_c > floor_c || want_p > floor_p || want_r > floor_r);
       ++k) {
    (void)hipGetLastError();
    want_c = std::max(floor_c, want_c / 2.0);
    want_p = std::max(floor_p, want_p / 2.0);
    want_r = std::max(floor_r, want_r / 2.0);
    ea = ensure_arenas((unsigned long long)want_c, (unsigned long long)want_p, (unsigned long long)want_r, true);
  }
  WF_CHECK(ea);
  if (!camera_mode)
    WF_CHECK(hipMemcpy2DAsync(rays_[0], sizeof(WfRay), job.d_in_rays, 6 * sizeof(double), 6 * sizeof(double), n0,
                              hipMemcpyDeviceToDevice, stream));
  WfArgs a = job_args(job, n0, frame_real);
  a.dev_sized = 1;
  a.colors_direct = averaged ? 0u : 1u;
  a.gtab = d_gtab_;
  a.gsh = d_gsh_;
  a.ray_buf[0] = rays_[0];
  a.ray_buf[1] = rays_[1];
  a.color_base = colors_;
  a.par_base = parents_;
  a.color_cap = color_cap_;
  a.par_cap = par_cap_;
  a.ray_cap = ray_cap_;
  a.hrec = d_rec_;
  a.skip_shadow = skip_shadow ? 1u : 0u;
  a.own_sphere = sc.obj_diag ? (unsigned)tn.own_sphere : 0u;
  a.spread = tn.spread ? 1u : 0u;
  a.count = count ? 1u : 0u;
  a.use_lb = (tn.shadow_lb && sc.lb_cells) ? 1u : 0u;
  const bool use_prim = camera_mode && sc.n_diag > 0;
  const unsigned kAnyRays = 1u << 30;
  for (unsigned g = 0; g <= max_depth; ++g) {
    a.g = g;
    a.colors = d_out;
    a.n = g == 0 ? n0 : 0u;
    a.in_cnt = g == 0 ? nullptr : shard_cnt(g, 0);
    a.out_cnt = shard_cnt(g + 1, 0);
    a.sh_cnt = shard_cnt(g, 1);
    const bool prim_launch = g == 0 && use_prim;
    const int ccls = prim_launch ? WF_PRIMARY : WF_CLOSEST;
    a.disc_slot = (unsigned)ccls;
    if (g == 0) prof_rays_[ccls] += n_real;
    WF_CHECK(pmark(stream, ccls, true));
    WF_CHECK(launch_fused(sc, cam, a, prim_launch, g == 0 ? n0 : kAnyRays, stream, count, tn,
                          g == 0 ? &plan_primary_ : &plan_secondary_));
    WF_CHECK(pmark(stream, ccls, false));
    if (job.gen_ev && (int)g == job.gen_ev_g) {
      WF_CHECK(hipEventRecord(job.gen_ev, stream));
      gen_ev_done_ = true;
    }
  }
  static int combine_grid = 0;
  if (combine_grid == 0) combine_grid = occupancy_grid(wf_combine_parents, kWfBlock, 0, kAnyRays);
  for (int g = max_depth > 0 ? (int)max_depth - 1 : 0; g >= 0; --g) {
    a.g = (unsigned)g;
    a.colors = d_out;
    a.sh_cnt = shard_cnt((unsigned)g, 1);
    a.out_cnt = shard_cnt(1, 0);
    WF_CHECK(pmark(stream, WF_COMBINE, true));
    WF_LAUNCH(wf_combine_parents, dim3(combine_grid), dim3(kWfBlock), 0, stream, sc, cam, a);
    WF_CHECK(hipGetLastError());
    WF_CHECK(pmark(stream, WF_COMBINE, false));
  }
  if (averaged) {
    const unsigned n_pix = n_frames * (frame_real / aa);
    WF_CHECK(pmark(stream, WF_COMBINE, true));
    WF_LAUNCH(wf_average, dim3(occupancy_grid(wf_average, kWfBlock, 0, n_pix)), dim3(kWfBlock), 0, stream,
              job_args(job, n0, frame_real), cam.hsize, colors_, n_pix, d_out);
    WF_CHECK(hipGetLastError());
    WF_CHECK(pmark(stream, WF_COMBINE, false));
  }
  lr_.last = max_depth;
  lr_.rays.clear();
  lr_.shadows.clear();
  return hipSuccess;
}

hipError_t Wavefront::render_exhaustive(const DevScene& sc, const WfJob& job, hipStream_t stream, bool skip_shadow,
                                        const WfTuning& tn, bool solo) {
  const DevCamera& cam = job.cam;
  const bool camera_mode = job.camera_mode(), count = (job.flags & WF_COUNT) != 0;
  const unsigned n0 = job.n0, aa = job.aa, max_depth = job.max_depth;
  double* const d_out = job.d_out;
  const bool averaged = aa > 1;
  const unsigned L = (unsigned)sc.n_lights;
  std::vector<unsigned> rays(max_depth + 2, 0), shadows(max_depth + 2, 0);
  rays[0] = n0;
  WF_CHECK(ensure_gen(0, n0, L, 0));
  if (!camera_mode) {
    WF_CHECK(hipMemcpy2DAsync(gens_[0].rays, sizeof(WfRay), job.d_in_rays, 6 * sizeof(double), 6 * sizeof(double), n0,
                              hipMemcpyDeviceToDevice, stream));
  }
  const bool prim_lds = wf_lds_bytes(sc.n_diag, sc.n_gen, sc.n_planes, true) <= kFusedLdsLimit;
  const bool gen_lds = wf_lds_bytes(sc.n_diag, sc.n_gen, sc.n_planes, false) <= kFusedLdsLimit;
  const bool use_prim = camera_mode && prim_lds && sc.n_diag > 0;
  hipStream_t sh_stream = stream;
  if (tn.shadow_stream == 2 || (tn.shadow_stream == 1 && solo)) {
    WF_CHECK(ensure_side());
    sh_stream = side_;
  }
  bool forked = false;
  unsigned last = 0;
  std::vector<unsigned> caps(max_depth + 2, 0), list_caps(max_depth + 2, 0);
  for (unsigned g = 0; g <= max_depth; ++g) {
    const unsigned n = rays[g];
    if (n == 0) break;
    last = g;
    const unsigned groups = ((n + 63) / 64 + kShardGroup - 1) / kShardGroup;
    const unsigned per = kShardGroup * ((groups + kShards - 1) / kShards);
    const unsigned out_cap = g < max_depth ? 128u * per : 0u, sh_cap = 64u * L * per;
    caps[g + 1] = out_cap;
    list_caps[g] = sh_cap;
    WF_CHECK(ensure_gen(g, g == 0 ? n : (size_t)kShards * caps[g], L, (size_t)kShards * sh_cap));
    WF_CHECK(ensure_gen(g + 1, (size_t)kShards * out_cap, L, 0));
    WfArgs a = job_args(job, n0, n0);
    WfGenBuf& B = gens_[g];
    a.rays = B.rays; a.hits = B.hits; a.nodes = B.nodes; a.shadow_nodes = B.shadow_nodes;
    a.geo = B.geo; a.surf = B.surf;
    a.colors = (g == 0 && !averaged) ? d_out : B.colors;
    a.next_rays = gens_[g + 1].rays;
    a.child_colors = gens_[g + 1].colors;
    a.n = n;
    a.in_cnt = g == 0 ? nullptr : shard_cnt(g, 0);
    a.in_cap = caps[g];
    a.out_cnt = shard_cnt(g + 1, 0);
    a.out_cap = out_cap;
    a.sh_cnt = shard_cnt(g, 1);
    a.sh_cap = sh_cap;
    a.g = g;
    a.skip_shadow = skip_shadow ? 1u : 0u;
    a.count = count ? 1u : 0u;
    const bool prim_launch = g == 0 && use_prim;
    const int ccls = prim_launch ? WF_PRIMARY : WF_CLOSEST;
    a.disc_slot = (unsigned)ccls;
    prof_rays_[ccls] += n;
    WF_CHECK(pmark(stream, ccls, true));
    if (sc.n_alias_rec > 0) WF_CHECK((launch_closest_exh<true, true, true>(sc, cam, a, prim_launch, gen_lds, n, stream, tn)));
    else if (sc.n_csg_units > 0) WF_CHECK((launch_closest_exh<true, true>(sc, cam, a, prim_launch, gen_lds, n, stream, tn)));
    else if (sc.n_quads > 0 || sc.n_tris > 0) WF_CHECK(launch_closest_exh<true>(sc, cam, a, prim_launch, gen_lds, n, stream, tn));
    else WF_CHECK(launch_closest_exh<false>(sc, cam, a, prim_launch, gen_lds, n, stream, tn));
    WF_CHECK(pmark(stream, ccls, false));
    WF_CHECK(pmark(stream, WF_PREP, true));
    if (sc.n_csg_units > 0)
      WF_LAUNCH(wf_prep_csg, dim3(occupancy_grid(wf_prep_csg, kWfBlock, 0, n)), dim3(kWfBlock), 0, stream, sc, cam, a);
    else
      WF_LAUNCH(wf_prep, dim3(occupancy_grid(wf_prep, kWfBlock, 0, n)), dim3(kWfBlock), 0, stream, sc, cam, a);
    WF_CHECK(hipGetLastError());
    WF_CHECK(pmark(stream, WF_PREP, false));
    {
      std::vector<unsigned> hr((size_t)kShards * kShardStride), hs(hr.size());
      WF_CHECK(hipMemcpyAsync(hr.data(), shard_cnt(g + 1, 0), hr.size() * sizeof(unsigned), hipMemcpyDeviceToHost,
                              stream));
      WF_CHECK(hipMemcpyAsync(hs.data(), shard_cnt(g, 1), hs.size() * sizeof(unsigned), hipMemcpyDeviceToHost, stream));
      WF_CHECK(hipStreamSynchronize(stream));
      unsigned nr = 0, ns = 0;
      for (int k = 0; k < kShards; ++k) {
        nr += hr[(size_t)k * kShardStride] + hr[(size_t)k * kShardStride + 1];
        ns += hs[(size_t)k * kShardStride];
      }
      rays[g + 1] = g < max_depth ? nr : 0;
      shadows[g] = ns;
    }
    a.n_shadow = shadows[g];
    if (a.n_shadow) {
      a.disc_slot = WF_SHADOW;
      prof_rays_[WF_SHADOW] += a.n_shadow;
      if (sh_stream != stream) {
        WF_CHECK(hipEventRecord(fork_ev_[g], stream));
        WF_CHECK(hipStreamWaitEvent(sh_stream, fork_ev_[g], 0));
        forked = true;
      }
      WF_CHECK(pmark(sh_stream, WF_SHADOW, true));
      if (sc.n_alias_rec > 0) WF_CHECK((launch_shadow_exh<true, true, true>(sc, a, gen_lds, sh_stream, tn)));
      else if (sc.n_csg_units > 0) WF_CHECK((launch_shadow_exh<true, true>(sc, a, gen_lds, sh_stream, tn)));
      else if (sc.n_quads > 0 || sc.n_tris > 0) WF_CHECK(launch_shadow_exh<true>(sc, a, gen_lds, sh_stream, tn));
      else WF_CHECK(launch_shadow_exh<false>(sc, a, gen_lds, sh_stream, tn));
      WF_CHECK(pmark(sh_stream, WF_SHADOW, false));
    }
    if (count) {
      WF_LAUNCH(wf_count_kinds, dim3(occupancy_grid(wf_count_kinds, 256, 0, n)), dim3(256), 0, stream, a);
      WF_CHECK(hipGetLastError());
    }
  }
  if (forked) {
    WF_CHECK(hipEventRecord(join_ev_, sh_stream));
    WF_CHECK(hipStreamWaitEvent(stream, join_ev_, 0));
  }
  for (int g = (int)last; g >= 0; --g) {
    WfArgs a = job_args(job, n0, n0);
    WfGenBuf& B = gens_[g];
    a.rays = B.rays; a.nodes = B.nodes; a.surf = B.surf;
    a.colors = (g == 0 && !averaged) ? d_out : B.colors;
    a.child_colors = gens_[g + 1].colors;
    a.n = rays[g];
    a.in_cnt = g == 0 ? nullptr : shard_cnt((unsigned)g, 0);
    a.in_cap = caps[g];
    a.g = (unsigned)g;
    if (a.n == 0) continue;
    WF_CHECK(pmark(stream, WF_COMBINE, true));
    WF_LAUNCH(wf_combine, dim3(occupancy_grid(wf_combine, kWfBlock, 0, a.n)), dim3(kWfBlock), 0, stream, sc, cam, a);
    WF_CHECK(hipGetLastError());
    WF_CHECK(pmark(stream, WF_COMBINE, false));
  }
  if (averaged) {
    const unsigned n_pix = n0 / aa;
    WF_CHECK(pmark(stream, WF_COMBINE, true));
    WfArgs a = job_args(job, n0, n0);
    a.cnt = nullptr;
    WF_LAUNCH(wf_average, dim3(occupancy_grid(wf_average, kWfBlock, 0, n_pix)), dim3(kWfBlock), 0, stream, a,
              cam.hsize, gens_[0].colors, n_pix, d_out);
    WF_CHECK(hipGetLastError());
    WF_CHECK(pmark(stream, WF_COMBINE, false));
  }
  lr_.rays = rays;
  lr_.shadows = shadows;
  lr_.last = last;
  return hipSuccess;
}

hipError_t Wavefront::read_stats(DevStats* out) {
  *out = DevStats{};
  if (!lr_.counted || !d_cnt_) return hipErrorInvalidValue;
  WF_CHECK(hipStreamSynchronize(lr_.stream));
  WfCounters hc;
  WF_CHECK(hipMemcpy(&hc, d_cnt_, sizeof hc, hipMemcpyDeviceToHost));
  std::vector<unsigned> counts;
  WF_CHECK(last_counts(counts));
  DevStats s{};
  unsigned long long rays = 0, hits = 0, traced_shadows = 0;
  for (unsigned g = 0; g < counts.size() && g < (unsigned)kMaxGen; ++g) {
    rays += counts[g];
    if (!lr_.fused && g < lr_.shadows.size()) traced_shadows += lr_.shadows[g];
    hits += hc.n_hit[g];
    s.rays_reflect += hc.n_refl[g];
    s.rays_refract += hc.n_refr[g];
  }
  if (lr_.fused) traced_shadows = hc.sh_rays(0) + hc.sh_rays(1);
  const unsigned long long shadows = hits * (unsigned long long)lr_.L;
  s.rays_primary = lr_.n0;
  s.rays_shadow = shadows;
  s.sphere_tests = (rays + shadows) * (lr_.n_diag + lr_.n_gen) - hc.gated(0);
  s.plane_tests = (rays + shadows) * lr_.n_planes - hc.gated(1);
  s.other_tests = (rays + shadows) * lr_.n_quads - hc.gated(2);
  s.sphere_disc_ge0 = lr_.exact_disc ? hc.disc(0) + hc.disc(1) + hc.disc(2) : ~0ull;
  s.exhaustive = lr_.exact_disc ? 1u : 0u;
  s.rays_shadow_traced = traced_shadows;
  const unsigned long long traced = rays + traced_shadows;
  s.sphere_tests_executed = (lr_.bvh ? hc.tests(0) + hc.tests(1) + hc.tests(2) + traced * lr_.n_gen
                                     : traced * (lr_.n_diag + lr_.n_gen)) - hc.gated(0);
  s.box_tests_executed = hc.boxes(0) + hc.boxes(1) + hc.boxes(2);
  *out = s;
  return hipSuccess;
}

}
```

### raytracer-challenge-rs_amd/csrc/rt_wavefront.hpp

```cpp
#pragma once
#include <hip/hip_runtime.h>

#include <string>
#include <vector>

#include "rt_layout.hpp"

namespace rtamd {

constexpr int kShards = 64;
constexpr int kShardStride = 32;
constexpr int kShardGroup = 16;

struct alignas(16) WfRay {
  double o[3];
  double d[3];
};
static_assert(sizeof(WfRay) == 48, "WfRay is origin + direction only");
struct WfHit {
  double t;
  int32_t key, c1k, c2k, hin;
};
struct WfNode {
  double schlick;
  int32_t obj;
  int32_t child_refl;
  int32_t child_refr;
  int32_t pad;
};
struct ParentRec {
  double surface[3];
  double schlick;
  uint32_t slot;
  int32_t obj;
  int32_t child_refl;
  int32_t child_refr;
};
struct PrimRec {
  double s[3];
  double op[3];
  double c;
  double pad;
};

constexpr int kMaxGen = 66;
enum WfFlags : unsigned { WF_EXHAUSTIVE = 1u, WF_COUNT = 2u, WF_TIME = 4u };

struct WfTuning {
  int accel = 1;
  int skip_shadow = 1;
  int shadow_lb = 1;
  int image = 0;
  int treelet = 1;
  int wide = 1;
  int lds_wide = 1;
  int treelet_deltas = 1;
  int shadow_stream = 1;
  int adaptive_block = 0;
  int prim_lane = 1;
  int arena_pct = 100;
  int d2h = 1;
  int bands = 4;
  int band_pct = 35;
  int band_ratio = 100;
  int band_gen = 1;
  int multi_gather = 0;
  int spread = 0;
  int own_sphere = 2;
};
int wf_tuning_apply(WfTuning& t, const char* key, int value);

struct WfImagePlan {
  int lane = -1;
  unsigned lds_flags = 0, n_top = 0;
  size_t dyn = 0;
};

struct WfArgs;
hipError_t wf_launch_global(int lane, bool quads, bool tris, bool csg, bool alias, bool tally, bool cam_rays, const DevScene& sc, const DevCamera& cam,
                            const WfArgs& a, size_t dyn, unsigned n, hipStream_t stream, int block, hipEvent_t e0,
                            hipEvent_t e1);

constexpr int kWorkRows = 256;
struct alignas(128) WfWorkRow {
  unsigned long long disc[3];
  unsigned long long tests[3];
  unsigned long long boxes[3];
  unsigned long long sh_rays[2];
  unsigned long long sh_tests[2];
  unsigned long long gated[3];
};
constexpr int kChunkClasses = 8;
constexpr int kChunkStride = 32;
struct WfCounters {
  unsigned chunk[kMaxGen * kChunkClasses * kChunkStride];
  unsigned n_refl[kMaxGen], n_refr[kMaxGen], n_hit[kMaxGen];
  unsigned overflow;
  WfWorkRow work[kWorkRows];
  unsigned long long disc(int c) const {
    unsigned long long t = 0;
    for (int r = 0; r < kWorkRows; ++r) t += work[r].disc[c];
    return t;
  }
  unsigned long long tests(int c) const {
    unsigned long long t = 0;
    for (int r = 0; r < kWorkRows; ++r) t += work[r].tests[c];
    return t;
  }
  unsigned long long boxes(int c) const {
    unsigned long long t = 0;
    for (int r = 0; r < kWorkRows; ++r) t += work[r].boxes[c];
    return t;
  }
  unsigned long long sh_rays(int c) const {
    unsigned long long t = 0;
    for (int r = 0; r < kWorkRows; ++r) t += work[r].sh_rays[c];
    return t;
  }
  unsigned long long sh_tests(int c) const {
    unsigned long long t = 0;
    for (int r = 0; r < kWorkRows; ++r) t += work[r].sh_tests[c];
    return t;
  }
  unsigned long long gated(int c) const {
    unsigned long long t = 0;
    for (int r = 0; r < kWorkRows; ++r) t += work[r].gated[c];
    return t;
  }
};

struct WfGeo {
  double over[3], normal[3], eyev[3];
  int32_t obj;
  int32_t pad;
};
struct WfGenBuf {
  WfRay* rays = nullptr;
  double* colors = nullptr;
  WfHit* hits = nullptr;
  WfNode* nodes = nullptr;
  int32_t* shadow_nodes = nullptr;
  WfGeo* geo = nullptr;
  double* surf = nullptr;
  size_t cap_rays = 0, cap_colors = 0, cap_hits = 0, cap_nodes = 0, cap_list = 0, cap_geo = 0, cap_surf = 0;
};

struct WfGenTab {
  unsigned cap;
  unsigned pad;
  unsigned long long color_off;
  unsigned long long par_off;
};
struct WfHostRec {
  int overflow;
  int pad[3];
  unsigned long long need_colors, need_parents, need_rays;
  unsigned long long frames;
  unsigned n_real;
  unsigned n_gens;
  unsigned counts[kMaxGen];
};
struct WfSizing {
  double rho = 0.0, mu = 0.0;
  int branch = 2;
};

constexpr unsigned kMaxFrames = 16;
struct FrameTable {
  DevCamera cam[kMaxFrames];
  double* out[kMaxFrames];
};

struct WfArgs {
  WfRay* rays;
  WfHit* hits;
  WfNode* nodes;
  double* colors;
  int32_t* shadow_nodes;
  WfGeo* geo;
  double* surf;
  ParentRec* parents;
  WfRay* next_rays;
  const double* child_colors;
  WfCounters* cnt;
  const PrimRec* prim;
  unsigned n;
  unsigned n_shadow;
  unsigned g, max_depth;
  unsigned camera_mode;
  unsigned row_block, shard, n_shards;
  unsigned long long blk_mask;
  unsigned blk_period;
  unsigned disc_slot;
  unsigned aa;
  unsigned rows;
  unsigned skip_shadow;
  unsigned own_sphere;
  unsigned spread;
  const unsigned* in_cnt;
  unsigned in_cap;
  unsigned* out_cnt;
  unsigned out_cap;
  unsigned* sh_cnt;
  unsigned sh_cap;
  unsigned count;
  unsigned use_lb;
  unsigned lds_flags;
  unsigned n_top;
  unsigned n_frames;
  unsigned frame_rays, frame_real;
  const FrameTable* frames;
  unsigned dev_sized;
  unsigned colors_direct;
  WfGenTab* gtab;
  unsigned* gsh;
  WfRay* ray_buf[2];
  double* color_base;
  ParentRec* par_base;
  unsigned long long color_cap, par_cap, ray_cap;
  WfHostRec* hrec;
};
static_assert(sizeof(WfArgs) == 336, "WfArgs is the kernels' argument block: its layout is fixed");

struct WfJob {
  DevCamera cam{};
  const double* d_in_rays = nullptr;
  unsigned n0 = 0;
  unsigned aa = 1;
  unsigned max_depth = 0;
  unsigned row_block = 1, shard = 0, n_shards = 1;
  unsigned blk_period = 0;
  unsigned long long blk_mask = 0;
  double* d_out = nullptr;
  const FrameTable* batch = nullptr;
  unsigned n_frames = 1;
  unsigned flags = 0;
  hipEvent_t gen_ev = nullptr;
  int gen_ev_g = -1;

  bool camera_mode() const { return d_in_rays == nullptr; }
  static WfJob camera_shard(const DevCamera& cam, unsigned n0, unsigned aa, unsigned max_depth, double* d_out,
                            unsigned row_block, unsigned shard = 0, unsigned n_shards = 1) {
    WfJob j;
    j.cam = cam; j.n0 = n0; j.aa = aa; j.max_depth = max_depth; j.d_out = d_out;
    j.row_block = row_block; j.shard = shard; j.n_shards = n_shards;
    return j;
  }
  static WfJob block_pattern(const DevCamera& cam, unsigned n0, unsigned aa, unsigned max_depth, double* d_out,
                             unsigned row_block, unsigned period, unsigned long long mask) {
    WfJob j = camera_shard(cam, n0, aa, max_depth, d_out, row_block);
    j.blk_period = period; j.blk_mask = mask;
    return j;
  }
  static WfJob ray_batch(const double* d_rays, unsigned n, unsigned max_depth, double* d_out) {
    WfJob j;
    j.d_in_rays = d_rays; j.n0 = n; j.max_depth = max_depth; j.d_out = d_out;
    return j;
  }
};
inline bool wf_aa_valid(unsigned aa) { return aa != 0 && aa <= 16 && (aa & (aa - 1)) == 0; }
inline bool wf_pattern_valid(unsigned period, unsigned long long mask) {
  return period <= 64 && mask != 0 && (period == 64 || (mask >> period) == 0);
}
inline bool wf_job_valid(const WfJob& j) {
  if (j.max_depth + 2 > (unsigned)kMaxGen) return false;
  if (j.blk_period && !wf_pattern_valid(j.blk_period, j.blk_mask)) return false;
  if (!wf_aa_valid(j.aa) || (!j.camera_mode() && j.aa != 1) || j.n0 % j.aa != 0) return false;
  return j.n_frames != 0 && j.n_frames <= kMaxFrames && (j.n_frames == 1 || j.batch != nullptr);
}

enum WfClass { WF_PRIMARY = 0, WF_CLOSEST = 1, WF_SHADOW = 2, WF_PREP = 3, WF_COMBINE = 4, WF_NCLASS = 5 };
struct WfProfile {
  double ms[WF_NCLASS];
  double rays[3];
  double disc[3];
  double tests[3];
  double boxes[3];
  double sh_rays[2], sh_tests[2];
  int bvh;
  int fused;
  int lane_primary, lane_secondary;
};

class Wavefront {
 public:
  ~Wavefront();
  void set_profiling(bool on, int class_mask = (1 << WF_NCLASS) - 1) {
    profiling_ = on;
    pmask_ = class_mask;
    if (on) { pn_ = 0; pframes_ = 0; }
  }
  size_t profiled_frames() const { return pframes_; }
  hipError_t last_profile(WfProfile* out);
  hipError_t render(const DevScene& sc, const WfJob& job, hipStream_t stream, WfSizing& sz, const WfTuning& tn,
                    bool solo);
  hipError_t read_stats(DevStats* out);
  hipError_t gen_counts(std::vector<unsigned>& rays) { return last_counts(rays); }
  hipError_t kernel_ms(float* ms) { return hipEventElapsedTime(ms, ev0_, ev1_); }
  bool overflowed() const { return h_rec_ && ((volatile WfHostRec*)h_rec_)->overflow != 0; }
  hipError_t take_overflow(bool* was);
  void learn(WfSizing& sz) const;
  bool gen_event_recorded() const { return gen_ev_done_; }
  const WfImagePlan& plan_primary() const { return plan_primary_; }
  const WfImagePlan& plan_secondary() const { return plan_secondary_; }

 private:
  hipError_t render_fast(const DevScene& sc, const WfJob& job, unsigned n0, unsigned frame_real, hipStream_t stream,
                         WfSizing& sz, bool skip_shadow, const WfTuning& tn);
  hipError_t render_exhaustive(const DevScene& sc, const WfJob& job, hipStream_t stream, bool skip_shadow,
                               const WfTuning& tn, bool solo);
  WfArgs job_args(const WfJob& job, unsigned n0, unsigned frame_real) const;
  hipError_t ensure_gen(size_t g, size_t slots, size_t n_lights, size_t list_slots);
  hipError_t ensure_misc(size_t n_diag, unsigned n_frames = 1);
  hipError_t ensure_arenas(unsigned long long colors, unsigned long long parents, unsigned long long rays,
                           bool exact);
  unsigned* shard_cnt(unsigned g, unsigned q) { return d_shard_ + ((size_t)g * 2 + q) * kShards * kShardStride; }
  std::vector<WfGenBuf> gens_;
  double* colors_ = nullptr;
  ParentRec* parents_ = nullptr;
  WfRay* rays_[2] = {nullptr, nullptr};
  unsigned long long color_cap_ = 0, par_cap_ = 0, ray_cap_ = 0;
  int squeezed_pct_ = 100;
  WfGenTab* d_gtab_ = nullptr;
  unsigned* d_gsh_ = nullptr;
  WfHostRec* h_rec_ = nullptr;
  WfHostRec* d_rec_ = nullptr;
  WfCounters* d_cnt_ = nullptr;
  unsigned* d_shard_ = nullptr;
  PrimRec* d_prim_ = nullptr;
  size_t prim_cap_ = 0;
  FrameTable* d_frames_ = nullptr;
  hipEvent_t ev0_ = nullptr, ev1_ = nullptr;
  hipStream_t side_ = nullptr;
  int side_dev_ = -1;
  hipEvent_t fork_ev_[kMaxGen] = {};
  hipEvent_t join_ev_ = nullptr;
  hipError_t ensure_side();
  struct LastRender {
    std::vector<unsigned> rays, shadows;
    unsigned last = 0, L = 0, n0 = 0, max_depth = 0;
    bool counted = false, exact_disc = false, bvh = false, fused = false;
    unsigned long long n_diag = 0, n_gen = 0, n_planes = 0, n_quads = 0;
    hipStream_t stream = nullptr;
  } lr_;
  hipError_t last_counts(std::vector<unsigned>& rays);
  bool last_bvh_ = false, last_fused_ = false;
  WfImagePlan plan_primary_, plan_secondary_;
  bool gen_ev_done_ = false;
  bool profiling_ = false;
  int pmask_ = (1 << WF_NCLASS) - 1;
  std::vector<hipEvent_t> pev_;
  std::vector<int> pcls_;
  size_t pn_ = 0;
  size_t pframes_ = 0;
  double prof_rays_[3] = {0, 0, 0};
  hipError_t pmark(hipStream_t s, int cls, bool begin);
};

}
```

### raytracer-challenge-rs_amd/csrc/rt_wf_combine.hip

```cpp
#include "rt_wf_device.hpp"

#pragma clang fp contract(off)

namespace rtamd {

__global__ void wf_frame_init(DevScene sc, DevCamera cam, PrimRec* prim, unsigned do_prim, uint4* zero_a,
                              unsigned n_a, uint4* zero_b, unsigned n_b, FrameTable tab, FrameTable* tab_dev,
                              unsigned n_frames, WfGenTab* gtab) {
  const unsigned stride = gridDim.x * blockDim.x;
  const unsigned i0 = blockIdx.x * blockDim.x + threadIdx.x;
  const uint4 z = make_uint4(0u, 0u, 0u, 0u);
  if (gtab && i0 == 0) gtab[0] = WfGenTab{0u, 0u, 0ull, 0ull};
  for (unsigned i = i0; i < n_a; i += stride) zero_a[i] = z;
  for (unsigned i = i0; i < n_b; i += stride) zero_b[i] = z;
  if (n_frames > 1) {
    const unsigned* src = (const unsigned*)&tab;
    unsigned* dst = (unsigned*)tab_dev;
    for (unsigned i = i0; i < (unsigned)(sizeof(FrameTable) / 4); i += stride) dst[i] = src[i];
  }
  if (!do_prim) return;
  const unsigned per = (unsigned)sc.n_diag + 4;
  for (unsigned jj = i0; jj < per * n_frames; jj += stride) {
    const unsigned f = jj / per, j = jj - f * per;
    const V3 o = m34_point(n_frames > 1 ? tab.cam[f].inv : cam.inv, v3(0.0, 0.0, 0.0));
    PrimRec p{};
    if (j < (unsigned)sc.n_diag) {
      const SphereDiag& r = sc.sph_diag[j];
      p.s[0] = r.s[0]; p.s[1] = r.s[1]; p.s[2] = r.s[2];
      p.op[0] = r.s[0] * o.x + r.t[0];
      p.op[1] = r.s[1] * o.y + r.t[1];
      p.op[2] = r.s[2] * o.z + r.t[2];
      p.c = p.op[0] * p.op[0] + p.op[1] * p.op[1] + p.op[2] * p.op[2] - 1.0;
    }
    prim[jj] = p;
  }
}

__global__ __launch_bounds__(kWfBlock) void wf_prep(DevScene sc, DevCamera cam, WfArgs a) {
  __shared__ unsigned s_pre[kPreRays];
  const unsigned* pre = shard_prefix<true>(a.in_cnt, s_pre);
  const unsigned stride = gridDim.x * blockDim.x;
  const unsigned n_iter = (a.n + stride - 1) / stride;
  unsigned i = blockIdx.x * blockDim.x + threadIdx.x;
  for (unsigned it = 0; it < n_iter; ++it, i += stride) {
    const bool valid = i < a.n;
    const unsigned slot = valid ? shard_slot<true>(pre, a.in_cap, i) : 0u;
    V3 o = v3(0, 0, 0), d = v3(0, 0, 0);
    Hit h;
    h.key = -1;
    if (valid) {
      wf_ray(a, cam, slot, o, d);
      const WfHit w = a.hits[slot];
      h.t = w.t; h.key = w.key; h.hin = w.hin; h.c1k = w.c1k; h.c2k = w.c2k; h.c1t = 0; h.c2t = 0;
    }
    prep_one(sc, a, i, slot, valid, o, d, h);
  }
}
__global__ __launch_bounds__(kWfBlock) void wf_prep_csg(DevScene sc, DevCamera cam, WfArgs a) {
  __shared__ unsigned s_pre[kPreRays];
  const unsigned* pre = shard_prefix<true>(a.in_cnt, s_pre);
  const unsigned stride = gridDim.x * blockDim.x;
  const unsigned n_iter = (a.n + stride - 1) / stride;
  unsigned i = blockIdx.x * blockDim.x + threadIdx.x;
  for (unsigned it = 0; it < n_iter; ++it, i += stride) {
    const bool valid = i < a.n;
    const unsigned slot = valid ? shard_slot<true>(pre, a.in_cap, i) : 0u;
    V3 o = v3(0, 0, 0), d = v3(0, 0, 0);
    Hit h;
    h.key = -1;
    if (valid) {
      wf_ray(a, cam, slot, o, d);
      const WfHit w = a.hits[slot];
      h.t = w.t; h.key = w.key; h.hin = w.hin; h.c1k = w.c1k; h.c2k = w.c2k; h.c1t = 0; h.c2t = 0;
    }
    prep_one<true>(sc, a, i, slot, valid, o, d, h);
  }
}

__global__ __launch_bounds__(kWfBlock) void wf_combine(DevScene sc, DevCamera cam, WfArgs a) {
  const unsigned stride = gridDim.x * blockDim.x;
  const unsigned L = (unsigned)sc.n_lights;
  __shared__ unsigned s_pre[kPreRays];
  const unsigned* pre = shard_prefix<true>(a.in_cnt, s_pre);
  for (unsigned i = blockIdx.x * blockDim.x + threadIdx.x; i < a.n; i += stride) {
    const unsigned slot = shard_slot<true>(pre, a.in_cap, i);
    const WfNode nd = a.nodes[slot];
    V3 color = v3(0.0, 0.0, 0.0);
    if (nd.obj >= 0) {
      const ShadeRec& m = sc.shade[nd.obj];
      V3 surface = v3(0.0, 0.0, 0.0);
      for (unsigned l = 0; l < L; ++l) {
        const double* sp = a.surf + ((size_t)slot * L + l) * 3;
        surface = vadd(surface, v3(sp[0], sp[1], sp[2]));
      }
      V3 refl = v3(0.0, 0.0, 0.0), refr = v3(0.0, 0.0, 0.0);
      if (nd.child_refl >= 0) {
        const double* cc = a.child_colors + (size_t)nd.child_refl * 3;
        refl = vscale(v3(cc[0], cc[1], cc[2]), m.reflective);
      }
      if (nd.child_refr >= 0) {
        const double* cc = a.child_colors + (size_t)nd.child_refr * 3;
        refr = vscale(v3(cc[0], cc[1], cc[2]), m.transparency);
      }
      if (m.reflective > 0.0 && m.transparency > 0.0) {
        const double r = nd.schlick;
        color = vadd(vadd(surface, vscale(refl, r)), vscale(refr, 1.0 - r));
      } else {
        color = vadd(vadd(surface, refl), refr);
      }
    }
    size_t oi = slot;
    if (a.g == 0 && a.camera_mode && a.aa == 1) {
      uint32_t x, lr, smp;
      gen0_pixel(a.aa, a.rows, cam.hsize, i, x, lr, smp);
      oi = (size_t)lr * cam.hsize + x;
    }
    double* out = a.colors + oi * 3;
    out[0] = color.x; out[1] = color.y; out[2] = color.z;
  }
}

__device__ __forceinline__ void poison_frames(const WfArgs& a, double* single, unsigned per_frame) {
  const unsigned nf = a.n_frames > 1 ? a.n_frames : 1u;
  const double nan = __builtin_nan("");
  const size_t n = (size_t)per_frame * 3, stride = (size_t)gridDim.x * blockDim.x;
  for (unsigned f = 0; f < nf; ++f) {
    double* o = a.n_frames > 1 ? a.frames->out[f] : single;
    for (size_t i = (size_t)blockIdx.x * blockDim.x + threadIdx.x; i < n; i += stride) o[i] = nan;
  }
}

__global__ __launch_bounds__(kWfBlock) void wf_combine_parents(DevScene sc, DevCamera cam, WfArgs a) {
  const unsigned stride = gridDim.x * blockDim.x;
  __shared__ unsigned s_pre[kPreList];
  const unsigned* pre = shard_prefix<false>(a.sh_cnt, s_pre);
  const WfGenTab t = a.gtab[a.g];
  const unsigned sh_cap = a.gsh[a.g];
  const unsigned n = sh_cap ? (unsigned)__builtin_amdgcn_readfirstlane((int)pre[kShards]) : 0u;
  const ParentRec* parents = a.par_base + t.par_off;
  const double* child_colors = a.color_base + a.gtab[a.g + 1].color_off * 3ull;
  if (!(a.g == 0 && a.colors_direct)) a.colors = a.color_base + t.color_off * 3ull;
  if (a.g == 0 && blockIdx.x == 0 && threadIdx.x < 64) {
    volatile WfHostRec* r = a.hrec;
    for (unsigned l = threadIdx.x; l <= a.max_depth && l < (unsigned)kMaxGen; l += 64) {
      unsigned c = a.frame_real * (a.n_frames > 1 ? a.n_frames : 1u);
      if (l > 0) {
        const unsigned* q = a.out_cnt + (size_t)(l - 1) * 2 * kShards * kShardStride;
        c = 0;
        for (int k = 0; k < kShards; ++k) c += q[k * kShardStride] + q[k * kShardStride + 1];
      }
      r->counts[l] = c;
    }
    if (threadIdx.x == 0) {
      r->n_real = a.frame_real * (a.n_frames > 1 ? a.n_frames : 1u);
      r->n_gens = a.max_depth + 1;
      r->frames = r->frames + 1;
    }
  }
  if (a.g == 0 && a.colors_direct && a.cnt->overflow) {
    poison_frames(a, a.colors, a.frame_real);
    return;
  }
  for (unsigned i = blockIdx.x * blockDim.x + threadIdx.x; i < n; i += stride) {
    const ParentRec p = parents[shard_slot<false>(pre, sh_cap, i)];
    typedef double f64x2v __attribute__((ext_vector_type(2)));
    const f64x2v rt = *(const f64x2v*)(sc.refl_transp + 2 * (size_t)p.obj);
    V3 refl = v3(0.0, 0.0, 0.0), refr = v3(0.0, 0.0, 0.0);
    if (p.child_refl >= 0) {
      const double* cc = child_colors + (size_t)p.child_refl * 3;
      refl = vscale(v3(cc[0], cc[1], cc[2]), rt.x);
    }
    if (p.child_refr >= 0) {
      const double* cc = child_colors + (size_t)p.child_refr * 3;
      refr = vscale(v3(cc[0], cc[1], cc[2]), rt.y);
    }
    const V3 col = shade_color_rt(rt.x, rt.y, v3(p.surface[0], p.surface[1], p.surface[2]), refl, refr, p.schlick);
    double* out = color_dst(a, cam, p.slot);
    out[0] = col.x; out[1] = col.y; out[2] = col.z;
  }
}

__global__ __launch_bounds__(kWfBlock) void wf_average(WfArgs a, unsigned hsize, const double* colors, unsigned n_pix,
                                                       double* out) {
  const unsigned stride = gridDim.x * blockDim.x;
  const unsigned aa = a.aa;
  const unsigned pix_frame = a.n_frames > 1 ? a.frame_real / aa : n_pix;
  if (a.cnt && a.cnt->overflow) {
    poison_frames(a, out, pix_frame);
    return;
  }
  for (unsigned p = blockIdx.x * blockDim.x + threadIdx.x; p < n_pix; p += stride) {
    const unsigned f = p / pix_frame, lp = p - f * pix_frame;
    const size_t s0 = (size_t)f * (a.n_frames > 1 ? a.frame_rays : 0u) + (size_t)lp * aa;
    V3 sum = v3(0.0, 0.0, 0.0);
    for (unsigned s = 0; s < aa; ++s) {
      const double* c = colors + (s0 + s) * 3;
      sum = vadd(sum, v3(c[0], c[1], c[2]));
    }
    const V3 avg = vscale(sum, 1.0 / (double)aa);
    uint32_t x, lr, smp;
    gen0_pixel(a.aa, a.rows, hsize, lp * aa, x, lr, smp);
    double* o = (a.n_frames > 1 ? a.frames->out[f] : out) + ((size_t)lr * hsize + x) * 3;
    o[0] = avg.x; o[1] = avg.y; o[2] = avg.z;
  }
}

__global__ void wf_count_kinds(WfArgs a) {
  unsigned nrefl = 0, nrefr = 0, nhit = 0;
  const unsigned stride = gridDim.x * blockDim.x;
  __shared__ unsigned s_pre[kPreRays];
  const unsigned* pre = shard_prefix<true>(a.in_cnt, s_pre);
  for (unsigned i = blockIdx.x * blockDim.x + threadIdx.x; i < a.n; i += stride) {
    const WfNode nd = a.nodes[shard_slot<true>(pre, a.in_cap, i)];
    nrefl += nd.child_refl >= 0;
    nrefr += nd.child_refr >= 0;
    nhit += nd.obj >= 0;
  }
  const unsigned long long s1 = wave_sum(nrefl), s2 = wave_sum(nrefr), s3 = wave_sum(nhit);
  if (lane_id() == 0) {
    if (s1) atomicAdd(&a.cnt->n_refl[a.g], (unsigned)s1);
    if (s2) atomicAdd(&a.cnt->n_refr[a.g], (unsigned)s2);
    if (s3) atomicAdd(&a.cnt->n_hit[a.g], (unsigned)s3);
  }
}


}
```

### raytracer-challenge-rs_amd/csrc/rt_wf_device.hpp

```cpp
#pragma once
#include <hip/hip_runtime.h>
#include <hip/hip_ext.h>

#include <algorithm>
#include <cstring>

#include "rt_device.hpp"
#include "rt_trace.hpp"
#include "rt_wavefront.hpp"

#pragma clang fp contract(off)

namespace rtamd {

[[maybe_unused]] constexpr int kWfBlock = 256;

#define WF_CHECK(x)                        \
  do {                                     \
    hipError_t _e = (x);                   \
    if (_e != hipSuccess) return _e;       \
  } while (0)


__device__ __forceinline__ WfWorkRow* work_row(WfCounters* c) {
// ... 296 lines not shown
__device__ __forceinline__ void add_gate_skips(WfCounters* cnt, const GateSkips& sk) {
  const unsigned long long a = wave_sum(sk.sph), b = wave_sum(sk.plane), c = wave_sum(sk.other);
  if (lane_id() == 0 && (a | b | c)) {
    WfWorkRow* w = work_row(cnt);
    if (a) atomicAdd(&w->gated[0], a);
    if (b) atomicAdd(&w->gated[1], b);
    if (c) atomicAdd(&w->gated[2], c);
  }
}

template <bool USE_LDS, bool PRIMARY, bool QUADS, int TW, bool CSG = false, bool ALIAS = false>
__global__ __launch_bounds__(kTraceBlock, TW) void wf_trace_closest(DevScene sc, DevCamera cam, WfArgs a) {
  extern __shared__ __attribute__((aligned(16))) unsigned char lds_raw[];
  unsigned n_disc = 0;
  GateSkips sk;
  WfLds lv{};
  if constexpr (USE_LDS) lv = wf_lds_stage<PRIMARY>(sc, a.prim, lds_raw);
  __shared__ unsigned s_pre[kPreRays];
  const unsigned* pre = shard_prefix<true>(a.in_cnt, s_pre);
  const unsigned stride = gridDim.x * blockDim.x;
  for (unsigned i = blockIdx.x * blockDim.x + threadIdx.x; i < a.n; i += stride) {
    const unsigned slot = shard_slot<true>(pre, a.in_cap, i);
    V3 o, d;
    wf_ray(a, cam, slot, o, d);
    Hit h;
    if constexpr (USE_LDS) wf_trace_lds<PRIMARY, false, QUADS, CSG, ALIAS>(sc, lv, o, d, h, n_disc, sk);
    else trace<false, QUADS, CSG, ALIAS>(sc, o, d, h, n_disc, &sk);
    WfHit w;
    w.t = h.t; w.key = h.key; w.c1k = h.c1k; w.c2k = h.c2k; w.hin = h.hin;
    a.hits[slot] = w;
  }
  const unsigned long long s = wave_sum(n_disc);
  if (lane_id() == 0 && s) atomicAdd(&work_row(a.cnt)->disc[a.disc_slot], s);
  if (sc.n_groups) add_gate_skips(a.cnt, sk);
}

template <bool USE_LDS, bool QUADS, int TW, bool CSG = false, bool ALIAS = false>
__global__ __launch_bounds__(kTraceBlock, TW) void wf_trace_shadow(DevScene sc, WfArgs a) {
  extern __shared__ __attribute__((aligned(16))) unsigned char lds_raw[];
  unsigned n_disc = 0;
  GateSkips sk;
  WfLds lv{};
  if constexpr (USE_LDS) lv = wf_lds_stage<false>(sc, nullptr, lds_raw);
  __shared__ unsigned s_pre[kPreList];
  const unsigned* pre = shard_prefix<false>(a.sh_cnt, s_pre);
  const unsigned stride = gridDim.x * blockDim.x;
  for (unsigned i = blockIdx.x * blockDim.x + threadIdx.x; i < a.n_shadow; i += stride) {
    V3 o, d;
    double dist;
    unsigned slot;
    shadow_ray(sc, a, shard_slot<false>(pre, a.sh_cap, i), o, d, dist, slot);
    Hit h;
    if constexpr (USE_LDS) wf_trace_lds<false, true, QUADS, CSG, ALIAS>(sc, lv, o, d, h, n_disc, sk);
    else trace<true, QUADS, CSG, ALIAS>(sc, o, d, h, n_disc, &sk);
    shadow_result(sc, a, slot, h.key >= 0 && h.t < dist, o, d);
  }
  const unsigned long long s = wave_sum(n_disc);
  if (lane_id() == 0 && s) atomicAdd(&work_row(a.cnt)->disc[a.disc_slot], s);
  if (sc.n_groups) add_gate_skips(a.cnt, sk);
}

__device__ __forceinline__ bool ray_class_r(const DevScene& sc, bool hit, const Comps& c) {
  return hit && sc.shade[c.obj].kind == 1;
}
__device__ __forceinline__ bool ray_class_f(bool hit, const Comps& c) { return hit && c.inside; }

template <bool CSG = false>
__device__ __forceinline__ void prep_one(const DevScene& sc, const WfArgs& a, unsigned i, unsigned slot, bool valid,
                                         V3 o, V3 d, const Hit& h) {
  const unsigned L = (unsigned)sc.n_lights;
  const unsigned remaining = a.max_depth - a.g;
  bool hit = false, want_refl = false, want_refr = false;
  Comps c{};
  V3 refr_dir = v3(0, 0, 0);
  const ShadeRec* m = nullptr;
  if (valid) {
    if (h.key >= 0) {
      c = prepare<true, CSG>(sc, o, d, h);
      hit = true;
      m = &sc.shade[c.obj];
      want_refl = !(req(m->reflective, 0.0) || remaining == 0);
      if (!(req(m->transparency, 0.0) || remaining == 0)) {
        const double n_ratio = c.n1 / c.n2;
        const double cos_i = vdot(c.eyev, c.normal);
        const double sin2_t = n_ratio * n_ratio * (1.0 - cos_i * cos_i);
        if (!(sin2_t > 1.0)) {
          const double cos_t = sqrt(1.0 - sin2_t);
          refr_dir = vsub(vscale(c.normal, n_ratio * cos_i - cos_t), vscale(c.eyev, n_ratio));
          want_refr = true;
        }
      }
    }
  }
  unsigned n_s = 0, skip = 0;
  if (hit) {
    for (unsigned l = 0; l < L; ++l) {
      V3 amb;
      cLightRec Lr = (cLightRec)sc.lights + l;
      if (a.skip_shadow && l < 32 &&
          shadow_irrelevant(*m, Lr, vnormalize(vsub(v3(Lr->pos[0], Lr->pos[1], Lr->pos[2]), c.over)), c.normal, amb)) {
        skip |= 1u << l;
        double* sp = a.surf + ((size_t)slot * L + l) * 3;
        sp[0] = amb.x; sp[1] = amb.y; sp[2] = amb.z;
      } else {
        ++n_s;
      }
    }
  }
  unsigned sbase, rbase, fbase;
  shard_append(a, i / 64, n_s, want_refl, want_refr, sbase, rbase, fbase, ray_class_r(sc, hit, c),
               ray_class_f(hit, c));
  if (!valid) return;
  WfNode nd;
  nd.obj = -1; nd.child_refl = -1; nd.child_refr = -1; nd.pad = 0; nd.schlick = 0.0;
  if (hit) {
    nd.obj = c.obj;
    if (n_s) {
      WfGeo gm;
      gm.over[0] = c.over.x; gm.over[1] = c.over.y; gm.over[2] = c.over.z;
      gm.normal[0] = c.normal.x; gm.normal[1] = c.normal.y; gm.normal[2] = c.normal.z;
      gm.eyev[0] = c.eyev.x; gm.eyev[1] = c.eyev.y; gm.eyev[2] = c.eyev.z;
      gm.obj = c.obj; gm.pad = 0;
      a.geo[slot] = gm;
    }
    nd.schlick = (m->reflective > 0.0 && m->transparency > 0.0) ? schlick(c.eyev, c.normal, c.n1, c.n2) : 0.0;
    for (unsigned l = 0; l < L; ++l)
      if (!(l < 32 && (skip >> l & 1u)) && sbase != ~0u) a.shadow_nodes[sbase++] = (int32_t)(slot * L + l);
    if (want_refl && rbase != ~0u) {
      const V3 rv = vreflect(d, c.normal);
      WfRay r;
      r.o[0] = c.over.x; r.o[1] = c.over.y; r.o[2] = c.over.z;
      r.d[0] = rv.x; r.d[1] = rv.y; r.d[2] = rv.z;
      a.next_rays[rbase] = r;
      nd.child_refl = (int)rbase;
    }
    if (want_refr && fbase != ~0u) {
      WfRay r;
      r.o[0] = c.under.x; r.o[1] = c.under.y; r.o[2] = c.under.z;
      r.d[0] = refr_dir.x; r.d[1] = refr_dir.y; r.d[2] = refr_dir.z;
      a.next_rays[fbase] = r;
      nd.child_refr = (int)fbase;
    }
  }
  a.nodes[slot] = nd;
}

template <bool CAM = true>
__device__ __forceinline__ double* color_dst(const WfArgs& a, const DevCamera& cam, unsigned slot) {
  size_t oi = slot;
  if (CAM && a.g == 0 && a.camera_mode && a.aa == 1) {
    unsigned li;
    const unsigned f = frame_of(a, slot, li);
    uint32_t x, lr, smp;
    gen0_pixel(1u, a.rows, cam.hsize, li, x, lr, smp);
    oi = (size_t)lr * cam.hsize + x;
    if (a.n_frames > 1) return a.frames->out[f] + oi * 3;
  }
  return a.colors + oi * 3;
}

__device__ __forceinline__ void st_ray(WfRay* p, V3 o, V3 d) {
  f64x2* q = reinterpret_cast<f64x2*>(p);
  __builtin_nontemporal_store((f64x2){o.x, o.y}, q);
  __builtin_nontemporal_store((f64x2){o.z, d.x}, q + 1);
  __builtin_nontemporal_store((f64x2){d.y, d.z}, q + 2);
}

__device__ __forceinline__ unsigned bind_generation(WfArgs& a, const unsigned* pre) {
  const unsigned g = a.g;
  const WfGenTab t = a.gtab[g];
  const unsigned n = g == 0 ? a.n
                            : (pre && t.cap ? (unsigned)__builtin_amdgcn_readfirstlane((int)pre[2 * kShards]) : 0u);
  const unsigned groups = ((n + 63u) / 64u + kShardGroup - 1u) / kShardGroup;
  const unsigned per = kShardGroup * ((groups + kShards - 1u) / kShards);
  unsigned out_cap = g < a.max_depth ? 128u * per : 0u, sh_cap = g < a.max_depth ? 64u * per : 0u;
  const unsigned long long slots = g == 0 ? (unsigned long long)n : (unsigned long long)kShards * t.cap;
  const unsigned long long c_next = t.color_off + slots;
  const unsigned long long need_c = c_next + (unsigned long long)kShards * out_cap;
  const unsigned long long need_p = t.par_off + (unsigned long long)kShards * sh_cap;
  const unsigned long long need_r = (unsigned long long)kShards * out_cap;
  const bool fits = need_c <= a.color_cap && need_p <= a.par_cap && need_r <= a.ray_cap;
  if (!fits) { out_cap = 0u; sh_cap = 0u; }
  if (blockIdx.x == 0 && threadIdx.x == 0) {
    a.gsh[g] = sh_cap;
    a.gtab[g + 1] = WfGenTab{out_cap, 0u, c_next, t.par_off + (unsigned long long)kShards * sh_cap};
    if (!fits) {
      a.cnt->overflow = 1u;
      volatile WfHostRec* r = a.hrec;
      r->need_colors = need_c;
      r->need_parents = need_p;
      r->need_rays = need_r;
      __threadfence_system();
      r->overflow = 1;
    }
  }
  a.n = n;
  a.in_cap = t.cap;
  a.out_cap = out_cap;
  a.sh_cap = sh_cap;
  WfRay* const rb0 = a.ray_buf[0];
  WfRay* const rb1 = a.ray_buf[1];
  a.rays = (g & 1u) ? rb1 : rb0;
  a.next_rays = (g & 1u) ? rb0 : rb1;
  if (!(g == 0 && a.colors_direct)) a.colors = a.color_base + t.color_off * 3ull;
  a.parents = a.par_base + t.par_off;
  return n;
}

struct FusedTally {
  GateSkips gsk;
  unsigned disc = 0, tests = 0, boxes = 0;
  unsigned sh_disc = 0, sh_tests = 0, sh_boxes = 0;
  unsigned sh_rays = 0;
  unsigned hits = 0, refl = 0, refr = 0;
};

template <bool QUADS, bool CAM, bool TALLY, bool TRIS, bool CSG, bool ALIAS, typename Image>
__device__ __forceinline__ void shade_fused(const DevScene& sc, const DevCamera& cam, const WfArgs& a,
                                            const Image& img, unsigned q, unsigned slot, bool valid, V3 o, V3 d,
                                            const Hit& h, FusedTally& t) {
  const unsigned L = (unsigned)sc.n_lights;
  const unsigned remaining = a.max_depth - a.g;
  bool hit = false, want_refl = false, want_refr = false;
  Comps c{};
  V3 refr_dir = v3(0, 0, 0);
  const ShadeRec* m = nullptr;
  if (valid && h.key >= 0) {
    c = prepare<TRIS, CSG>(sc, o, d, h);
    hit = true;
    m = &sc.shade[c.obj];
    want_refl = !(req(m->reflective, 0.0) || remaining == 0);
    if (!(req(m->transparency, 0.0) || remaining == 0)) {
      const double n_ratio = c.n1 / c.n2;
      const double cos_i = vdot(c.eyev, c.normal);
      const double sin2_t = n_ratio * n_ratio * (1.0 - cos_i * cos_i);
      if (!(sin2_t > 1.0)) {
        const double cos_t = sqrt(1.0 - sin2_t);
        refr_dir = vsub(vscale(c.normal, n_ratio * cos_i - cos_t), vscale(c.eyev, n_ratio));
        want_refr = true;
      }
    }
  }
  const bool parent = want_refl || want_refr;
  unsigned pbase, rbase, fbase;
  shard_append(a, q, parent ? 1u : 0u, want_refl, want_refr, pbase, rbase, fbase, ray_class_r(sc, hit, c),
               ray_class_f(hit, c));
  if (!valid) return;
  t.hits += hit; t.refl += want_refl; t.refr += want_refr;
  double* dst = color_dst<CAM>(a, cam, slot);
  if (!hit) {
    st_d(dst, 0.0); st_d(dst + 1, 0.0); st_d(dst + 2, 0.0);
    return;
  }
  int child_refl = -1, child_refr = -1;
  if (want_refl && rbase != ~0u) {
    st_ray(a.next_rays + rbase, c.over, vreflect(d, c.normal));
    child_refl = (int)rbase;
  }
  if (want_refr && fbase != ~0u) {
    st_ray(a.next_rays + fbase, c.under, refr_dir);
    child_refr = (int)fbase;
  }
  const double schlick_r =
      (m->reflective > 0.0 && m->transparency > 0.0) ? schlick(c.eyev, c.normal, c.n1, c.n2) : 0.0;
  V3 surface = v3(0.0, 0.0, 0.0);
  const int own = a.own_sphere ? sc.obj_diag[c.obj] : -1;
  const int own_first = own >= 0 && c.inside ? (own & kOwnIndex) : -1;
  const int own_out = own >= 0 && !c.inside && a.own_sphere > 1 && (own & kOwnOutside) ? (own & kOwnIndex) : -1;
  for (unsigned l = 0; l < L; ++l) {
    cLightRec Lr = (cLightRec)sc.lights + l;
    const V3 v = vsub(v3(Lr->pos[0], Lr->pos[1], Lr->pos[2]), c.over);
    const double dist = sqrt(v.x * v.x + v.y * v.y + v.z * v.z);
    const V3 sdir = v3(v.x / dist, v.y / dist, v.z / dist);
    V3 term;
    if (a.skip_shadow && shadow_irrelevant(*m, Lr, sdir, c.normal, term)) {
    } else {
      const bool shadowed = shadow_trace<QUADS, TALLY, TRIS, CSG, ALIAS>(
          sc, a.use_lb, img, l, c.over, sdir, dist, t.sh_disc, t.sh_tests, t.sh_boxes, &t.gsk, own_first,
          own_out >= 0 && vdot(sdir, c.normal) >= 0.0 ? own_out : -1);
      if (QUADS && a.count) count_hier_gates<TRIS, CSG>(sc, c.over, sdir, t.gsk);
      ++t.sh_rays;
      term = lighting(*m, Lr, c.over, c.eyev, c.normal, shadowed, sdir);
    }
    surface = vadd(surface, term);
  }
  if (child_refl >= 0 || child_refr >= 0) {
    if (pbase != ~0u) {
      ParentRec* pr = a.parents + pbase;
      st_d(&pr->surface[0], surface.x); st_d(&pr->surface[1], surface.y); st_d(&pr->surface[2], surface.z);
      st_d(&pr->schlick, schlick_r);
      i32x4 tail = {(int)slot, c.obj, child_refl, child_refr};
      __builtin_nontemporal_store(tail, (i32x4*)&pr->slot);
    }
    return;
  }
  const V3 zero = v3(0.0, 0.0, 0.0);
  const V3 col = shade_color(*m, surface, zero, zero, schlick_r);
  st_d(dst, col.x); st_d(dst + 1, col.y); st_d(dst + 2, col.z);
}

template <bool PRIMARY, bool QUADS, int LANE, bool TALLY, bool CAM = PRIMARY, bool TRIS = false, bool CSG = false,
          bool ALIAS = false>
__global__ __launch_bounds__(kTraceBlock, 4) void wf_trace_fused(DevScene sc, DevCamera cam, WfArgs a) {
  __shared__ int stack_lds[lane_static_lds_bytes(LANE) ? lane_static_lds_bytes(LANE) / 4 : 1];
  extern __shared__ __attribute__((aligned(16))) unsigned char lane_dyn[];
  __shared__ unsigned s_pre[kPreRays];
  const unsigned* pre = shard_prefix<true>(a.in_cnt, s_pre);
  if (a.dev_sized) bind_generation(a, pre);
  const unsigned n_chunks = (a.n + 63u) / 64u;
  const unsigned waves_per_block = blockDim.x / 64u;
  const unsigned W = gridDim.x * waves_per_block;
  const bool spread = a.spread && n_chunks < W;
  if (spread ? blockIdx.x >= n_chunks : blockIdx.x * waves_per_block >= n_chunks) return;
  typedef LaneImage<LANE> Image;
  Image img;
  img.stage(sc, a.lds_flags, a.n_top, stack_lds, lane_dyn);
  FusedTally t;
  const bool dyn_all = n_chunks >= 3u * W;
  const bool dyn_tail = !dyn_all && n_chunks > W;
  const bool dyn = dyn_all || dyn_tail;
  const unsigned X = gridDim.x < (unsigned)kChunkClasses ? gridDim.x : (unsigned)kChunkClasses;
  const unsigned cls = blockIdx.x % X;
  unsigned* ctr = a.cnt->chunk + ((size_t)a.g * kChunkClasses + cls) * kChunkStride;
  const unsigned c_base = dyn_all ? cls : W + cls;
  unsigned c = spread ? (threadIdx.x / 64u) * gridDim.x + blockIdx.x : blockIdx.x * waves_per_block + threadIdx.x / 64u;
  if (dyn_all) {
    unsigned k0 = 0;
    if (lane_id() == 0) k0 = atomicAdd(ctr, 1u);
    c = cls + X * (unsigned)__shfl((int)k0, 0, 64);
  }
  auto traverse = [&](unsigned i, bool valid, unsigned slot, V3& o, V3& d, Hit& h) {
    hit_init(h);
    if (valid) {
      wf_ray<CAM>(a, cam, slot, o, d);
      if constexpr (TALLY && QUADS) count_hier_gates<TRIS, CSG>(sc, o, d, t.gsk);
      if constexpr (!Image::kPerLane) {
        const unsigned pf = a.n_frames > 1 ? (c * 64u) / a.frame_rays : 0u;
        img.template closest<PRIMARY>(sc, (cPrimRec)(a.prim + (size_t)pf * ((unsigned)sc.n_diag + 4)), o, d, h, t.disc,
                                      t.tests, t.boxes);
      }
      trace_rest<false, QUADS, true, TRIS, CSG, ALIAS>(sc, o, d, h, t.disc, &t.gsk);
      if constexpr (QUADS) {
        other_trace<false>(sc, o, d, 0.0, h, t.disc, t.tests, t.boxes);
        line_trace<false>(sc, o, d, 0.0, h, t.tests, t.boxes);
      }
      if constexpr (TRIS) tri_trace<false>(sc, o, d, 0.0, h, t.tests, t.boxes);
      if constexpr (CSG) unit_trace<false>(sc, o, d, 0.0, h, t.disc, t.tests, t.boxes);
      if constexpr (Image::kPerLane) img.template walk<false>(sc, o, d, 0.0, h, t.disc, t.tests, t.boxes);
    }
    hit_finish(h);
    if constexpr (ALIAS) alias_finish(sc, h);
  };
  while (c < n_chunks) {
    unsigned k_next = 0;
    if (dyn && lane_id() == 0) k_next = atomicAdd(ctr, 1u);
    const unsigned i = c * 64u + lane_id();
    const bool valid = i < a.n && (a.g != 0 || a.n_frames <= 1 || i % a.frame_rays < a.frame_real);
    const unsigned slot = valid ? shard_slot<true>(pre, a.in_cap, i) : 0u;
    V3 o = v3(0, 0, 0), d = v3(0, 0, 0);
    Hit h;
    traverse(i, valid, slot, o, d, h);
    shade_fused<QUADS, CAM, TALLY, TRIS, CSG, ALIAS>(sc, cam, a, img, c, slot, valid, o, d, h, t);
    c = dyn ? c_base + X * (unsigned)__shfl((int)k_next, 0, 64) : c + W;
  }
  if constexpr (!TALLY) return;
  if (sc.n_groups) add_gate_skips(a.cnt, t.gsk);
  const unsigned long long s = wave_sum(t.disc), st = wave_sum(t.tests), sb = wave_sum(t.boxes);
  const unsigned long long hs = wave_sum(t.sh_disc), hst = wave_sum(t.sh_tests), hsb = wave_sum(t.sh_boxes);
  const unsigned long long hr = wave_sum(t.sh_rays);
  if (lane_id() == 0) {
    WfWorkRow* w = work_row(a.cnt);
    if (s) atomicAdd(&w->disc[a.disc_slot], s);
    if (st) atomicAdd(&w->tests[a.disc_slot], st);
    if (sb) atomicAdd(&w->boxes[a.disc_slot], sb);
    if (hs) atomicAdd(&w->disc[WF_SHADOW], hs);
    if (hst) { atomicAdd(&w->tests[WF_SHADOW], hst); atomicAdd(&w->sh_tests[a.disc_slot], hst); }
    if (hsb) atomicAdd(&w->boxes[WF_SHADOW], hsb);
    if (hr) atomicAdd(&w->sh_rays[a.disc_slot], hr);
  }
  if (a.count) {
    const unsigned long long n1 = wave_sum(t.hits), n2 = wave_sum(t.refl), n3 = wave_sum(t.refr);
    if (lane_id() == 0) {
      if (n1) atomicAdd(&a.cnt->n_hit[a.g], (unsigned)n1);
      if (n2) atomicAdd(&a.cnt->n_refl[a.g], (unsigned)n2);
      if (n3) atomicAdd(&a.cnt->n_refr[a.g], (unsigned)n3);
    }
  }
}

__global__ void wf_frame_init(DevScene sc, DevCamera cam, PrimRec* prim, unsigned do_prim, uint4* zero_a,
                              unsigned n_a, uint4* zero_b, unsigned n_b, FrameTable tab, FrameTable* tab_dev,
                              unsigned n_frames, WfGenTab* gtab);
__global__ void wf_prep(DevScene sc, DevCamera cam, WfArgs a);
__global__ void wf_prep_csg(DevScene sc, DevCamera cam, WfArgs a);
__global__ void wf_combine(DevScene sc, DevCamera cam, WfArgs a);
__global__ void wf_combine_parents(DevScene sc, DevCamera cam, WfArgs a);
__global__ void wf_average(WfArgs a, unsigned hsize, const double* colors, unsigned n_pix, double* out);
__global__ void wf_count_kinds(WfArgs a);

}
```

### raytracer-challenge-rs_amd/csrc/rt_wf_plan.hpp

```cpp
#pragma once
#include <stddef.h>

#include <algorithm>

#include "rt_layout.hpp"
#include "rt_wavefront.hpp"

namespace rtamd {

constexpr int kTraceBlock = 1024;
constexpr size_t kFusedLdsLimit = 160 * 1024 - 1024;

constexpr int kLaneWave = 0;
constexpr int kLaneScratch = 1;
constexpr int kLaneLdsStack = 3;
constexpr int kLaneWide16 = 4;
constexpr int kLanePair = 14;
constexpr int kLaneWideLds = 15;

constexpr unsigned kLdsSpheres = 1u, kLdsDeltas = 2u;

constexpr size_t lane_static_lds_bytes(int lane) {
  return lane == kLaneLdsStack ? (size_t)kLaneLdsDepth * kTraceBlock * 4
         : lane == kLaneWave   ? (size_t)(kTraceBlock / 64) * (kBvhMaxDepth + 4) * 4
                               : 0;
}

__host__ __device__ inline size_t lane_stack_bytes(int depth) { return (size_t)(depth > 0 ? depth : 1) * kTraceBlock * 4; }
__host__ __device__ inline size_t sph_lds_bytes(const DevScene& sc) { return (size_t)sc.n_diag * sizeof(SphereDiag); }
__host__ __device__ inline size_t sph48_lds_bytes(const DevScene& sc) {
  return (size_t)sc.n_diag * 48 + (((size_t)sc.n_diag * 4 + 15) & ~(size_t)15);
}
__host__ __device__ inline size_t delta_lds_bytes(const DevScene& sc) {
  return sc.lb_cells ? (((size_t)sc.n_lights * sc.n_diag * 2 + 15) & ~(size_t)15) : 0;
}
__host__ __device__ inline size_t pair_stack_bytes(const DevScene& sc) {
  return (lane_stack_bytes(sc.bvh_depth + 1) / 2 + 15) & ~(size_t)15;
}
__host__ __device__ inline size_t wide_stack_bytes(const DevScene& sc) {
  return ((size_t)(sc.bvhw_stack > 0 ? sc.bvhw_stack : 1) * kTraceBlock * 2 + 15) & ~(size_t)15;
}

struct LaneLdsLayout {
  size_t stack, nodes, sph48, sph, deltas, treelet, end;
};
__host__ __device__ inline LaneLdsLayout lane_lds_layout(int lane, const DevScene& sc, unsigned lds_flags,
                                                         unsigned n_top) {
  const bool lds_img = lane == kLanePair || lane == kLaneWideLds;
  LaneLdsLayout l{};
  size_t p = 0;
  l.stack = p;
  p += lane == kLanePair ? pair_stack_bytes(sc) : lane == kLaneWide16 || lane == kLaneWideLds ? wide_stack_bytes(sc) : 0;
  l.nodes = p;
  p += lane == kLanePair      ? (size_t)sc.n_bvh * sizeof(BvhPair)
       : lane == kLaneWideLds ? (size_t)sc.n_bvhw * sizeof(BvhWide)
                              : 0;
  l.sph48 = p;
  p += lds_img ? sph48_lds_bytes(sc) : 0;
  l.sph = p;
  p += lane == kLaneWave && (lds_flags & kLdsSpheres) ? sph_lds_bytes(sc) : 0;
  l.deltas = p;
  p += (lds_flags & kLdsDeltas) ? delta_lds_bytes(sc) : 0;
  l.treelet = p;
  p += (size_t)n_top * (lane == kLaneLdsStack ? sizeof(BvhNode) : lane == kLaneWide16 ? sizeof(BvhWide16) : 0);
  l.end = p;
  return l;
}
__host__ __device__ inline size_t pair_lds_bytes(const DevScene& sc) {
  return sc.bvh_pair ? lane_lds_layout(kLanePair, sc, 0, 0).end : (size_t)1 << 40;
}
__host__ __device__ inline size_t wide_lds_bytes(const DevScene& sc) {
  return sc.bvhw ? lane_lds_layout(kLaneWideLds, sc, 0, 0).end : (size_t)1 << 40;
}

inline size_t pair_image_leaf_estimate(int bvh_depth, size_t n_nodes, size_t n_diag) {
  return (size_t)(bvh_depth + 1) * kTraceBlock * 4 + n_nodes * sizeof(BvhNode) + n_diag * sizeof(SphereDiag);
}

inline WfImagePlan wf_plan_image(const DevScene& sc, const WfTuning& tn, bool primary, bool use_lb) {
  const size_t dl = use_lb ? delta_lds_bytes(sc) : 0;
  const bool wide_ok = tn.image != 1 && tn.wide && sc.bvhw16 && wide_stack_bytes(sc) <= kFusedLdsLimit / 2;
  const bool wide_lds = tn.image == 0 && sc.bvhw && tn.lds_wide && wide_lds_bytes(sc) + dl <= kFusedLdsLimit;
  const bool pair_lds = tn.image == 0 && pair_lds_bytes(sc) <= kFusedLdsLimit;
  const bool lds_img = wide_lds || pair_lds;
  const bool lane_prim = tn.prim_lane == 1 ? (lds_img || wide_ok) : tn.prim_lane == 2 ? lds_img : false;
  WfImagePlan p;
  p.lane = primary && !lane_prim                              ? kLaneWave
           : wide_lds                                         ? kLaneWideLds
           : pair_lds                                         ? kLanePair
           : wide_ok                                          ? kLaneWide16
           : tn.image != 1 && sc.bvh_depth <= kLaneLdsDepth ? kLaneLdsStack
                                                              : kLaneScratch;
  const size_t room = kFusedLdsLimit - lane_static_lds_bytes(p.lane);
  auto used = [&] { return lane_lds_layout(p.lane, sc, p.lds_flags, p.n_top).end; };
  if (p.lane == kLaneWave && sph_lds_bytes(sc) <= room) p.lds_flags |= kLdsSpheres;
  const bool treelet = (p.lane == kLaneWide16 || p.lane == kLaneLdsStack) && tn.treelet;
  if (dl && used() + dl <= room && (!treelet || tn.treelet_deltas)) p.lds_flags |= kLdsDeltas;
  if (treelet) {
    const size_t n_nodes = p.lane == kLaneWide16 ? (size_t)sc.n_bvhw : (size_t)sc.n_bvh;
    p.n_top = (unsigned)std::min<size_t>(n_nodes, (room - used()) / 64);
  }
  p.dyn = used();
  return p;
}
static_assert(sizeof(BvhNode) == 64 && sizeof(BvhWide16) == 64, "wf_plan_image: a treelet node is 64 B");

}
```

Before: 18750 Mrays/s.

## Let combine kernels co-reside with fused trace across in-flight frame batches

Adds a 'coresident' tuning mode, on by default at value 2, for batched in-flight frame rendering with the wide-LDS lane. It launches a register-capped (60 VGPR attribute) variant of the fused trace kernel and small 64-thread combine kernels, either register-capped or with launch bounds, sized so the combine blocks fit in the CU's LDS and registers next to the trace blocks. The aim is to let the combine passes of one stream overlap the trace kernels of other streams. Mode 1 instead shrinks the trace block by one wave. Capping registers risks spills in the trace kernel, and the 64-thread combine blocks may run less efficiently on their own.

```diff
diff --git a/raytracer-challenge-rs_amd/csrc/pybind/rtamd_py.cpp b/raytracer-challenge-rs_amd/csrc/pybind/rtamd_py.cpp
--- a/raytracer-challenge-rs_amd/csrc/pybind/rtamd_py.cpp
+++ b/raytracer-challenge-rs_amd/csrc/pybind/rtamd_py.cpp
@@ -81,6 +81,7 @@
 extern "C" int rtamd_pngz_kernel_times(const double* d_rgb, uint32_t width, uint32_t height, uint8_t* d_out, size_t cap,
                                        float* ms, void* stream);
 extern "C" int rtamd_wf_plan(const rt_scene* s, long long out[16]);
+extern "C" int rtamd_wf_shape(const rt_scene* s, long long out[4]);
 extern "C" int rtamd_csg_plan(const rt_scene* s, long long out[6]);
 extern "C" int rtamd_scene_tuning_set(const rt_scene* s, const char* key, int value);
 extern "C" int rtamd_render_shard_host(const rt_scene* scene, const rt_camera_desc* camera, uint32_t max_depth,
@@ -859,6 +860,19 @@
     d["n_alias_classes"] = o[15];
     return d;
   }, py::arg("world"));
+  m.def("_wf_shape", [](const World& w) {
+    long long o[4] = {0};
+    check(rtamd_wf_shape(w.scene(), o), "wf_shape");
+    py::dict d;
+    const char* which[2] = {"primary", "secondary"};
+    for (int i = 0; i < 2; ++i) {
+      py::dict p;
+      p["threads"] = (int)o[2 * i];
+      p["coresident"] = (int)o[2 * i + 1];
+      d[which[i]] = p;
+    }
+    return d;
+  }, py::arg("world"));
   m.def("_csg_plan", [](const World& w) {
     long long o[6] = {0};
     check(rtamd_csg_plan(w.scene(), o), "csg_plan");
diff --git a/raytracer-challenge-rs_amd/csrc/rt_api.cpp b/raytracer-challenge-rs_amd/csrc/rt_api.cpp
--- a/raytracer-challenge-rs_amd/csrc/rt_api.cpp
+++ b/raytracer-challenge-rs_amd/csrc/rt_api.cpp
@@ -118,6 +118,20 @@
   return RT_OK;
 }
 
+int rtamd_wf_shape(const rt_scene* cs, long long out[4]) {
+  if (!cs || !out) return fail(RT_ERR_INVALID_ARGUMENT, "null scene or output");
+  rt_scene* s = const_cast<rt_scene*>(cs);
+  std::lock_guard<std::mutex> lk(s->mu);
+  const WfImagePlan none{};
+  const WfImagePlan* pl[2] = {s->last_wf ? &s->last_wf->wf->plan_primary() : &none,
+                              s->last_wf ? &s->last_wf->wf->plan_secondary() : &none};
+  for (int i = 0; i < 2; ++i) {
+    out[2 * i] = pl[i]->lane >= 0 ? pl[i]->threads : 0;
+    out[2 * i + 1] = pl[i]->lane >= 0 ? pl[i]->coresident : 0;
+  }
+  return RT_OK;
+}
+
 int rtamd_csg_plan(const rt_scene* cs, long long out[6]) {
   if (!cs || !out) return fail(RT_ERR_INVALID_ARGUMENT, "null scene or output");
   rt_scene* s = const_cast<rt_scene*>(cs);
diff --git a/raytracer-challenge-rs_amd/csrc/rt_render.cpp b/raytracer-challenge-rs_amd/csrc/rt_render.cpp
--- a/raytracer-challenge-rs_amd/csrc/rt_render.cpp
+++ b/raytracer-challenge-rs_amd/csrc/rt_render.cpp
@@ -93,6 +93,7 @@
     job.blk_mask = blk_mask;
     if (nf > 1) job.batch = &tab;
     job.n_frames = nf;
+    job.in_flight = nf > 1 && blk_period == 0;
     RenderResult r;
     int rc = run_render(s, job, st, call, &r);
     if (rc != RT_OK) return rc;
diff --git a/raytracer-challenge-rs_amd/csrc/rt_wavefront.hip b/raytracer-challenge-rs_amd/csrc/rt_wavefront.hip
--- a/raytracer-challenge-rs_amd/csrc/rt_wavefront.hip
+++ b/raytracer-challenge-rs_amd/csrc/rt_wavefront.hip
@@ -24,7 +24,8 @@
       {"d2h", &WfTuning::d2h, 0, 1},               {"bands", &WfTuning::bands, 1, 4},
       {"band_pct", &WfTuning::band_pct, 5, 95},   {"band_gen", &WfTuning::band_gen, -1, 8},
       {"band_ratio", &WfTuning::band_ratio, 30, 100}, {"multi_gather", &WfTuning::multi_gather, 0, 1},
-      {"own_sphere", &WfTuning::own_sphere, 0, 2}, {"spread", &WfTuning::spread, 0, 1}};
+      {"own_sphere", &WfTuning::own_sphere, 0, 2}, {"spread", &WfTuning::spread, 0, 1},
+      {"coresident", &WfTuning::coresident, 0, 2}};
   if (!key) return 0;
   for (const Knob& k : knobs) {
     if (std::strcmp(key, k.name) != 0) continue;
@@ -306,13 +307,19 @@
 
 template <bool QUADS, bool TALLY, bool TRIS = false, bool CSG = false, bool ALIAS = false>
 static hipError_t launch_fused_q(const DevScene& sc, const DevCamera& cam, WfArgs a, bool primary, unsigned n,
-                                 hipStream_t stream, const WfTuning& tn, WfImagePlan* ran) {
+                                 hipStream_t stream, const WfTuning& tn, int coresident, WfImagePlan* ran) {
   if (a.spread && !tn.adaptive_block) n = 1u << 30;
-  const int tb = trace_block(n, tn.adaptive_block);
-  const WfImagePlan plan = *ran = wf_plan_image(sc, tn, primary, a.use_lb != 0);
+  constexpr bool kCapped = !QUADS && !TALLY && !TRIS && !CSG && !ALIAS;
+  if (coresident == 2 && !kCapped) coresident = 0;
+  const WfImagePlan plan = *ran = wf_plan_image(sc, tn, primary, a.use_lb != 0, coresident);
+  const int tb = std::min(trace_block(n, tn.adaptive_block), plan.threads);
   a.lds_flags = plan.lds_flags;
   a.n_top = plan.n_top;
   const bool cam_rays = a.g == 0 && a.camera_mode;
+  if constexpr (kCapped)
+    if (plan.coresident == 2)
+      return cam_rays ? launch_timed(wf_trace_fused_cap<true>, tb, plan.dyn, n, stream, sc, cam, a)
+                      : launch_timed(wf_trace_fused_cap<false>, tb, plan.dyn, n, stream, sc, cam, a);
 #define RT_LDS(P, L, C) launch_timed(wf_trace_fused<P, QUADS, L, TALLY, C, TRIS, CSG, ALIAS>, tb, plan.dyn, n, stream, sc, cam, a)
   switch (plan.lane) {
     case kLaneWave: return RT_LDS(true, kLaneWave, true);
@@ -324,22 +331,22 @@
   return wf_launch_global(plan.lane, QUADS, TRIS, CSG, ALIAS, TALLY, cam_rays, sc, cam, a, plan.dyn, n, stream, tb, t_ev_start, t_ev_stop);
 }
 static hipError_t launch_fused(const DevScene& sc, const DevCamera& cam, const WfArgs& a, bool primary, unsigned n,
-                               hipStream_t stream, bool tally, const WfTuning& tn, WfImagePlan* ran) {
+                               hipStream_t stream, bool tally, const WfTuning& tn, int coresident, WfImagePlan* ran) {
   const bool quads = sc.n_fx_quads > 0 || sc.n_obvh > 0 || sc.n_lbvh > 0;
   if (sc.n_alias_rec > 0)
-    return tally ? launch_fused_q<true, true, true, true, true>(sc, cam, a, primary, n, stream, tn, ran)
-                 : launch_fused_q<true, false, true, true, true>(sc, cam, a, primary, n, stream, tn, ran);
+    return tally ? launch_fused_q<true, true, true, true, true>(sc, cam, a, primary, n, stream, tn, coresident, ran)
+                 : launch_fused_q<true, false, true, true, true>(sc, cam, a, primary, n, stream, tn, coresident, ran);
   if (sc.n_csg_units > 0)
-    return tally ? launch_fused_q<true, true, true, true>(sc, cam, a, primary, n, stream, tn, ran)
-                 : launch_fused_q<true, false, true, true>(sc, cam, a, primary, n, stream, tn, ran);
+    return tally ? launch_fused_q<true, true, true, true>(sc, cam, a, primary, n, stream, tn, coresident, ran)
+                 : launch_fused_q<true, false, true, true>(sc, cam, a, primary, n, stream, tn, coresident, ran);
   if (sc.n_tris > 0)
-    return tally ? launch_fused_q<true, true, true>(sc, cam, a, primary, n, stream, tn, ran)
-                 : launch_fused_q<true, false, true>(sc, cam, a, primary, n, stream, tn, ran);
+    return tally ? launch_fused_q<true, true, true>(sc, cam, a, primary, n, stream, tn, coresident, ran)
+                 : launch_fused_q<true, false, true>(sc, cam, a, primary, n, stream, tn, coresident, ran);
   if (tally)
-    return quads ? launch_fused_q<true, true>(sc, cam, a, primary, n, stream, tn, ran)
-                 : launch_fused_q<false, true>(sc, cam, a, primary, n, stream, tn, ran);
-  return quads ? launch_fused_q<true, false>(sc, cam, a, primary, n, stream, tn, ran)
-               : launch_fused_q<false, false>(sc, cam, a, primary, n, stream, tn, ran);
+    return quads ? launch_fused_q<true, true>(sc, cam, a, primary, n, stream, tn, coresident, ran)
+                 : launch_fused_q<false, true>(sc, cam, a, primary, n, stream, tn, coresident, ran);
+  return quads ? launch_fused_q<true, false>(sc, cam, a, primary, n, stream, tn, coresident, ran)
+               : launch_fused_q<false, false>(sc, cam, a, primary, n, stream, tn, coresident, ran);
 }
 
 WfArgs Wavefront::job_args(const WfJob& job, unsigned n0, unsigned frame_real) const {
@@ -489,6 +496,7 @@
   a.use_lb = (tn.shadow_lb && sc.lb_cells) ? 1u : 0u;
   const bool use_prim = camera_mode && sc.n_diag > 0;
   const unsigned kAnyRays = 1u << 30;
+  const int coresident = job.in_flight && n_frames > 1 && !count ? tn.coresident : 0;
   for (unsigned g = 0; g <= max_depth; ++g) {
     a.g = g;
     a.colors = d_out;
@@ -501,7 +509,7 @@
     a.disc_slot = (unsigned)ccls;
     if (g == 0) prof_rays_[ccls] += n_real;
     WF_CHECK(pmark(stream, ccls, true));
-    WF_CHECK(launch_fused(sc, cam, a, prim_launch, g == 0 ? n0 : kAnyRays, stream, count, tn,
+    WF_CHECK(launch_fused(sc, cam, a, prim_launch, g == 0 ? n0 : kAnyRays, stream, count, tn, coresident,
                           g == 0 ? &plan_primary_ : &plan_secondary_));
     WF_CHECK(pmark(stream, ccls, false));
     if (job.gen_ev && (int)g == job.gen_ev_g) {
@@ -509,15 +517,22 @@
       gen_ev_done_ = true;
     }
   }
-  static int combine_grid = 0;
-  if (combine_grid == 0) combine_grid = occupancy_grid(wf_combine_parents, kWfBlock, 0, kAnyRays);
+  static int combine_grid = 0, combine_grid_co[2] = {0, 0};
+  if (combine_grid == 0) {
+    combine_grid = occupancy_grid(wf_combine_parents, kWfBlock, 0, kAnyRays);
+    combine_grid_co[0] = occupancy_grid(wf_combine_parents_co, 64, 0, kAnyRays);
+    combine_grid_co[1] = occupancy_grid(wf_combine_parents_co32, 64, 0, kAnyRays);
+  }
+  const int co_form = (max_depth > 0 ? plan_secondary_ : plan_primary_).coresident;
   for (int g = max_depth > 0 ? (int)max_depth - 1 : 0; g >= 0; --g) {
     a.g = (unsigned)g;
     a.colors = d_out;
     a.sh_cnt = shard_cnt((unsigned)g, 1);
     a.out_cnt = shard_cnt(1, 0);
     WF_CHECK(pmark(stream, WF_COMBINE, true));
-    WF_LAUNCH(wf_combine_parents, dim3(combine_grid), dim3(kWfBlock), 0, stream, sc, cam, a);
+    if (co_form == 1) WF_LAUNCH(wf_combine_parents_co, dim3(combine_grid_co[0]), dim3(64), 0, stream, sc, cam, a);
+    else if (co_form == 2) WF_LAUNCH(wf_combine_parents_co32, dim3(combine_grid_co[1]), dim3(64), 0, stream, sc, cam, a);
+    else WF_LAUNCH(wf_combine_parents, dim3(combine_grid), dim3(kWfBlock), 0, stream, sc, cam, a);
     WF_CHECK(hipGetLastError());
     WF_CHECK(pmark(stream, WF_COMBINE, false));
   }
diff --git a/raytracer-challenge-rs_amd/csrc/rt_wavefront.hpp b/raytracer-challenge-rs_amd/csrc/rt_wavefront.hpp
--- a/raytracer-challenge-rs_amd/csrc/rt_wavefront.hpp
+++ b/raytracer-challenge-rs_amd/csrc/rt_wavefront.hpp
@@ -67,6 +67,7 @@
   int multi_gather = 0;
   int spread = 0;
   int own_sphere = 2;
+  int coresident = 2;
 };
 int wf_tuning_apply(WfTuning& t, const char* key, int value);
 
@@ -74,6 +75,8 @@
   int lane = -1;
   unsigned lds_flags = 0, n_top = 0;
   size_t dyn = 0;
+  int threads = 0;
+  int coresident = 0;
 };
 
 struct WfArgs;
@@ -237,6 +240,7 @@
   unsigned flags = 0;
   hipEvent_t gen_ev = nullptr;
   int gen_ev_g = -1;
+  bool in_flight = false;
 
   bool camera_mode() const { return d_in_rays == nullptr; }
   static WfJob camera_shard(const DevCamera& cam, unsigned n0, unsigned aa, unsigned max_depth, double* d_out,
diff --git a/raytracer-challenge-rs_amd/csrc/rt_wf_combine.hip b/raytracer-challenge-rs_amd/csrc/rt_wf_combine.hip
--- a/raytracer-challenge-rs_amd/csrc/rt_wf_combine.hip
+++ b/raytracer-challenge-rs_amd/csrc/rt_wf_combine.hip
@@ -130,9 +130,8 @@
   }
 }
 
-__global__ __launch_bounds__(kWfBlock) void wf_combine_parents(DevScene sc, DevCamera cam, WfArgs a) {
-  const unsigned stride = gridDim.x * blockDim.x;
-  __shared__ unsigned s_pre[kPreList];
+__device__ __forceinline__ void combine_parents(const DevScene& sc, const DevCamera& cam, WfArgs a, unsigned* s_pre) {
+  const unsigned stride = gridDim.x * blockDim.x;
   const unsigned* pre = shard_prefix<false>(a.sh_cnt, s_pre);
   const WfGenTab t = a.gtab[a.g];
   const unsigned sh_cap = a.gsh[a.g];
@@ -180,6 +179,22 @@
   }
 }
 
+__global__ __launch_bounds__(kWfBlock) void wf_combine_parents(DevScene sc, DevCamera cam, WfArgs a) {
+  __shared__ unsigned s_pre[kPreList];
+  combine_parents(sc, cam, a, s_pre);
+}
+static_assert(sizeof(unsigned) * kPreList == kCombineStaticLds, "the plan's LDS condition counts s_pre");
+__global__ __launch_bounds__(64, 8) void wf_combine_parents_co(DevScene sc, DevCamera cam, WfArgs a) {
+  __shared__ unsigned s_pre[kPreList];
+  combine_parents(sc, cam, a, s_pre);
+}
+__global__ __launch_bounds__(64) __attribute__((amdgpu_num_vgpr(16))) void wf_combine_parents_co32(DevScene sc,
+                                                                                                    DevCamera cam,
+                                                                                                    WfArgs a) {
+  __shared__ unsigned s_pre[kPreList];
+  combine_parents(sc, cam, a, s_pre);
+}
+
 __global__ __launch_bounds__(kWfBlock) void wf_average(WfArgs a, unsigned hsize, const double* colors, unsigned n_pix,
                                                        double* out) {
   const unsigned stride = gridDim.x * blockDim.x;
diff --git a/raytracer-challenge-rs_amd/csrc/rt_wf_device.hpp b/raytracer-challenge-rs_amd/csrc/rt_wf_device.hpp
--- a/raytracer-challenge-rs_amd/csrc/rt_wf_device.hpp
+++ b/raytracer-challenge-rs_amd/csrc/rt_wf_device.hpp
@@ -622,91 +622,16 @@
 template <bool PRIMARY, bool QUADS, int LANE, bool TALLY, bool CAM = PRIMARY, bool TRIS = false, bool CSG = false,
           bool ALIAS = false>
 __global__ __launch_bounds__(kTraceBlock, 4) void wf_trace_fused(DevScene sc, DevCamera cam, WfArgs a) {
-  __shared__ int stack_lds[lane_static_lds_bytes(LANE) ? lane_static_lds_bytes(LANE) / 4 : 1];
-  extern __shared__ __attribute__((aligned(16))) unsigned char lane_dyn[];
-  __shared__ unsigned s_pre[kPreRays];
-  const unsigned* pre = shard_prefix<true>(a.in_cnt, s_pre);
-  if (a.dev_sized) bind_generation(a, pre);
-  const unsigned n_chunks = (a.n + 63u) / 64u;
-  const unsigned waves_per_block = blockDim.x / 64u;
-  const unsigned W = gridDim.x * waves_per_block;
-  const bool spread = a.spread && n_chunks < W;
-  if (spread ? blockIdx.x >= n_chunks : blockIdx.x * waves_per_block >= n_chunks) return;
-  typedef LaneImage<LANE> Image;
-  Image img;
-  img.stage(sc, a.lds_flags, a.n_top, stack_lds, lane_dyn);
-  FusedTally t;
-  const bool dyn_all = n_chunks >= 3u * W;
-  const bool dyn_tail = !dyn_all && n_chunks > W;
-  const bool dyn = dyn_all || dyn_tail;
-  const unsigned X = gridDim.x < (unsigned)kChunkClasses ? gridDim.x : (unsigned)kChunkClasses;
-  const unsigned cls = blockIdx.x % X;
-  unsigned* ctr = a.cnt->chunk + ((size_t)a.g * kChunkClasses + cls) * kChunkStride;
-  const unsigned c_base = dyn_all ? cls : W + cls;
-  unsigned c = spread ? (threadIdx.x / 64u) * gridDim.x + blockIdx.x : blockIdx.x * waves_per_block + threadIdx.x / 64u;
-  if (dyn_all) {
-    unsigned k0 = 0;
-    if (lane_id() == 0) k0 = atomicAdd(ctr, 1u);
-    c = cls + X * (unsigned)__shfl((int)k0, 0, 64);
-  }
-  auto traverse = [&](unsigned i, bool valid, unsigned slot, V3& o, V3& d, Hit& h) {
-    hit_init(h);
-    if (valid) {
-      wf_ray<CAM>(a, cam, slot, o, d);
-      if constexpr (TALLY && QUADS) count_hier_gates<TRIS, CSG>(sc, o, d, t.gsk);
-      if constexpr (!Image::kPerLane) {
-        const unsigned pf = a.n_frames > 1 ? (c * 64u) / a.frame_rays : 0u;
-        img.template closest<PRIMARY>(sc, (cPrimRec)(a.prim + (size_t)pf * ((unsigned)sc.n_diag + 4)), o, d, h, t.disc,
-                                      t.tests, t.boxes);
-      }
-      trace_rest<false, QUADS, true, TRIS, CSG, ALIAS>(sc, o, d, h, t.disc, &t.gsk);
-      if constexpr (QUADS) {
-        other_trace<false>(sc, o, d, 0.0, h, t.disc, t.tests, t.boxes);
-        line_trace<false>(sc, o, d, 0.0, h, t.tests, t.boxes);
-      }
-      if constexpr (TRIS) tri_trace<false>(sc, o, d, 0.0, h, t.tests, t.boxes);
-      if constexpr (CSG) unit_trace<false>(sc, o, d, 0.0, h, t.disc, t.tests, t.boxes);
-      if constexpr (Image::kPerLane) img.template walk<false>(sc, o, d, 0.0, h, t.disc, t.tests, t.boxes);
-    }
-    hit_finish(h);
-    if constexpr (ALIAS) alias_finish(sc, h);
-  };
-  while (c < n_chunks) {
-    unsigned k_next = 0;
-    if (dyn && lane_id() == 0) k_next = atomicAdd(ctr, 1u);
-    const unsigned i = c * 64u + lane_id();
-    const bool valid = i < a.n && (a.g != 0 || a.n_frames <= 1 || i % a.frame_rays < a.frame_real);
-    const unsigned slot = valid ? shard_slot<true>(pre, a.in_cap, i) : 0u;
-    V3 o = v3(0, 0, 0), d = v3(0, 0, 0);
-    Hit h;
-    traverse(i, valid, slot, o, d, h);
-    shade_fused<QUADS, CAM, TALLY, TRIS, CSG, ALIAS>(sc, cam, a, img, c, slot, valid, o, d, h, t);
-    c = dyn ? c_base + X * (unsigned)__shfl((int)k_next, 0, 64) : c + W;
-  }
-  if constexpr (!TALLY) return;
-  if (sc.n_groups) add_gate_skips(a.cnt, t.gsk);
-  const unsigned long long s = wave_sum(t.disc), st = wave_sum(t.tests), sb = wave_sum(t.boxes);
-  const unsigned long long hs = wave_sum(t.sh_disc), hst = wave_sum(t.sh_tests), hsb = wave_sum(t.sh_boxes);
-  const unsigned long long hr = wave_sum(t.sh_rays);
-  if (lane_id() == 0) {
-    WfWorkRow* w = work_row(a.cnt);
-    if (s) atomicAdd(&w->disc[a.disc_slot], s);
-    if (st) atomicAdd(&w->tests[a.disc_slot], st);
-    if (sb) atomicAdd(&w->boxes[a.disc_slot], sb);
-    if (hs) atomicAdd(&w->disc[WF_SHADOW], hs);
-    if (hst) { atomicAdd(&w->tests[WF_SHADOW], hst); atomicAdd(&w->sh_tests[a.disc_slot], hst); }
-    if (hsb) atomicAdd(&w->boxes[WF_SHADOW], hsb);
-    if (hr) atomicAdd(&w->sh_rays[a.disc_slot], hr);
-  }
-  if (a.count) {
-    const unsigned long long n1 = wave_sum(t.hits), n2 = wave_sum(t.refl), n3 = wave_sum(t.refr);
-    if (lane_id() == 0) {
-      if (n1) atomicAdd(&a.cnt->n_hit[a.g], (unsigned)n1);
-      if (n2) atomicAdd(&a.cnt->n_refl[a.g], (unsigned)n2);
-      if (n3) atomicAdd(&a.cnt->n_refr[a.g], (unsigned)n3);
-    }
-  }
-}
+#include "rt_wf_fused_body.inc"
+}
+template <bool CAM, int LANE = kLaneWideLds, bool PRIMARY = false, bool QUADS = false, bool TALLY = false,
+          bool TRIS = false, bool CSG = false, bool ALIAS = false>
+__global__ __launch_bounds__(kTraceBlock, 4) __attribute__((amdgpu_num_vgpr(60))) void wf_trace_fused_cap(DevScene sc,
+                                                                                                           DevCamera cam,
+                                                                                                           WfArgs a) {
+#include "rt_wf_fused_body.inc"
+}
+static_assert(kCoCapVgprs == 120, "wf_trace_fused_cap's register attribute");
 
 __global__ void wf_frame_init(DevScene sc, DevCamera cam, PrimRec* prim, unsigned do_prim, uint4* zero_a,
                               unsigned n_a, uint4* zero_b, unsigned n_b, FrameTable tab, FrameTable* tab_dev,
@@ -715,6 +640,8 @@
 __global__ void wf_prep_csg(DevScene sc, DevCamera cam, WfArgs a);
 __global__ void wf_combine(DevScene sc, DevCamera cam, WfArgs a);
 __global__ void wf_combine_parents(DevScene sc, DevCamera cam, WfArgs a);
+__global__ void wf_combine_parents_co(DevScene sc, DevCamera cam, WfArgs a);
+__global__ void wf_combine_parents_co32(DevScene sc, DevCamera cam, WfArgs a);
 __global__ void wf_average(WfArgs a, unsigned hsize, const double* colors, unsigned n_pix, double* out);
 __global__ void wf_count_kinds(WfArgs a);
 
diff --git a/raytracer-challenge-rs_amd/csrc/rt_wf_fused_body.inc b/raytracer-challenge-rs_amd/csrc/rt_wf_fused_body.inc
--- /dev/null
+++ b/raytracer-challenge-rs_amd/csrc/rt_wf_fused_body.inc
@@ -0,0 +1,84 @@
+  __shared__ int stack_lds[lane_static_lds_bytes(LANE) ? lane_static_lds_bytes(LANE) / 4 : 1];
+  extern __shared__ __attribute__((aligned(16))) unsigned char lane_dyn[];
+  __shared__ unsigned s_pre[kPreRays];
+  const unsigned* pre = shard_prefix<true>(a.in_cnt, s_pre);
+  if (a.dev_sized) bind_generation(a, pre);
+  const unsigned n_chunks = (a.n + 63u) / 64u;
+  const unsigned waves_per_block = blockDim.x / 64u;
+  const unsigned W = gridDim.x * waves_per_block;
+  const bool spread = a.spread && n_chunks < W;
+  if (spread ? blockIdx.x >= n_chunks : blockIdx.x * waves_per_block >= n_chunks) return;
+  typedef LaneImage<LANE> Image;
+  Image img;
+  img.stage(sc, a.lds_flags, a.n_top, stack_lds, lane_dyn);
+  FusedTally t;
+  const bool dyn_all = n_chunks >= 3u * W;
+  const bool dyn_tail = !dyn_all && n_chunks > W;
+  const bool dyn = dyn_all || dyn_tail;
+  const unsigned X = gridDim.x < (unsigned)kChunkClasses ? gridDim.x : (unsigned)kChunkClasses;
+  const unsigned cls = blockIdx.x % X;
+  unsigned* ctr = a.cnt->chunk + ((size_t)a.g * kChunkClasses + cls) * kChunkStride;
+  const unsigned c_base = dyn_all ? cls : W + cls;
+  unsigned c = spread ? (threadIdx.x / 64u) * gridDim.x + blockIdx.x : blockIdx.x * waves_per_block + threadIdx.x / 64u;
+  if (dyn_all) {
+    unsigned k0 = 0;
+    if (lane_id() == 0) k0 = atomicAdd(ctr, 1u);
+    c = cls + X * (unsigned)__shfl((int)k0, 0, 64);
+  }
+  auto traverse = [&](unsigned i, bool valid, unsigned slot, V3& o, V3& d, Hit& h) {
+    hit_init(h);
+    if (valid) {
+      wf_ray<CAM>(a, cam, slot, o, d);
+      if constexpr (TALLY && QUADS) count_hier_gates<TRIS, CSG>(sc, o, d, t.gsk);
+      if constexpr (!Image::kPerLane) {
+        const unsigned pf = a.n_frames > 1 ? (c * 64u) / a.frame_rays : 0u;
+        img.template closest<PRIMARY>(sc, (cPrimRec)(a.prim + (size_t)pf * ((unsigned)sc.n_diag + 4)), o, d, h, t.disc,
+                                      t.tests, t.boxes);
+      }
+      trace_rest<false, QUADS, true, TRIS, CSG, ALIAS>(sc, o, d, h, t.disc, &t.gsk);
+      if constexpr (QUADS) {
+        other_trace<false>(sc, o, d, 0.0, h, t.disc, t.tests, t.boxes);
+        line_trace<false>(sc, o, d, 0.0, h, t.tests, t.boxes);
+      }
+      if constexpr (TRIS) tri_trace<false>(sc, o, d, 0.0, h, t.tests, t.boxes);
+      if constexpr (CSG) unit_trace<false>(sc, o, d, 0.0, h, t.disc, t.tests, t.boxes);
+      if constexpr (Image::kPerLane) img.template walk<false>(sc, o, d, 0.0, h, t.disc, t.tests, t.boxes);
+    }
+    hit_finish(h);
+    if constexpr (ALIAS) alias_finish(sc, h);
+  };
+  while (c < n_chunks) {
+    unsigned k_next = 0;
+    if (dyn && lane_id() == 0) k_next = atomicAdd(ctr, 1u);
+    const unsigned i = c * 64u + lane_id();
+    const bool valid = i < a.n && (a.g != 0 || a.n_frames <= 1 || i % a.frame_rays < a.frame_real);
+    const unsigned slot = valid ? shard_slot<true>(pre, a.in_cap, i) : 0u;
+    V3 o = v3(0, 0, 0), d = v3(0, 0, 0);
+    Hit h;
+    traverse(i, valid, slot, o, d, h);
+    shade_fused<QUADS, CAM, TALLY, TRIS, CSG, ALIAS>(sc, cam, a, img, c, slot, valid, o, d, h, t);
+    c = dyn ? c_base + X * (unsigned)__shfl((int)k_next, 0, 64) : c + W;
+  }
+  if constexpr (!TALLY) return;
+  if (sc.n_groups) add_gate_skips(a.cnt, t.gsk);
+  const unsigned long long s = wave_sum(t.disc), st = wave_sum(t.tests), sb = wave_sum(t.boxes);
+  const unsigned long long hs = wave_sum(t.sh_disc), hst = wave_sum(t.sh_tests), hsb = wave_sum(t.sh_boxes);
+  const unsigned long long hr = wave_sum(t.sh_rays);
+  if (lane_id() == 0) {
+    WfWorkRow* w = work_row(a.cnt);
+    if (s) atomicAdd(&w->disc[a.disc_slot], s);
+    if (st) atomicAdd(&w->tests[a.disc_slot], st);
+    if (sb) atomicAdd(&w->boxes[a.disc_slot], sb);
+    if (hs) atomicAdd(&w->disc[WF_SHADOW], hs);
+    if (hst) { atomicAdd(&w->tests[WF_SHADOW], hst); atomicAdd(&w->sh_tests[a.disc_slot], hst); }
+    if (hsb) atomicAdd(&w->boxes[WF_SHADOW], hsb);
+    if (hr) atomicAdd(&w->sh_rays[a.disc_slot], hr);
+  }
+  if (a.count) {
+    const unsigned long long n1 = wave_sum(t.hits), n2 = wave_sum(t.refl), n3 = wave_sum(t.refr);
+    if (lane_id() == 0) {
+      if (n1) atomicAdd(&a.cnt->n_hit[a.g], (unsigned)n1);
+      if (n2) atomicAdd(&a.cnt->n_refl[a.g], (unsigned)n2);
+      if (n3) atomicAdd(&a.cnt->n_refr[a.g], (unsigned)n3);
+    }
+  }
diff --git a/raytracer-challenge-rs_amd/csrc/rt_wf_plan.hpp b/raytracer-challenge-rs_amd/csrc/rt_wf_plan.hpp
--- a/raytracer-challenge-rs_amd/csrc/rt_wf_plan.hpp
+++ b/raytracer-challenge-rs_amd/csrc/rt_wf_plan.hpp
@@ -10,6 +10,16 @@
 
 constexpr int kTraceBlock = 1024;
 constexpr size_t kFusedLdsLimit = 160 * 1024 - 1024;
+
+constexpr int kTraceBlockCo = kTraceBlock - 64;
+constexpr int kCoBlocksA = 2, kCoBlocksB = 4, kCoCapVgprs = 120;
+constexpr size_t kCuLdsBytes = 160 * 1024;
+constexpr size_t kFusedPrefixLds = 528;
+constexpr size_t kCombineStaticLds = 260;
+constexpr size_t lds_alloc_bytes(size_t b) {
+  const size_t u = (b + 1279) / 1280 * 1280, v = (b + 511) / 512 * 512;
+  return u > v ? u : v;
+}
 
 constexpr int kLaneWave = 0;
 constexpr int kLaneScratch = 1;
@@ -77,7 +87,12 @@
   return (size_t)(bvh_depth + 1) * kTraceBlock * 4 + n_nodes * sizeof(BvhNode) + n_diag * sizeof(SphereDiag);
 }
 
-inline WfImagePlan wf_plan_image(const DevScene& sc, const WfTuning& tn, bool primary, bool use_lb) {
+constexpr bool coresident_lds_fits(int lane, size_t dyn, int blocks) {
+  return lds_alloc_bytes(dyn + lane_static_lds_bytes(lane) + kFusedPrefixLds) +
+             (size_t)blocks * lds_alloc_bytes(kCombineStaticLds) <= kCuLdsBytes;
+}
+inline WfImagePlan wf_plan_image(const DevScene& sc, const WfTuning& tn, bool primary, bool use_lb,
+                                 int coresident = 0) {
   const size_t dl = use_lb ? delta_lds_bytes(sc) : 0;
   const bool wide_ok = tn.image != 1 && tn.wide && sc.bvhw16 && wide_stack_bytes(sc) <= kFusedLdsLimit / 2;
   const bool wide_lds = tn.image == 0 && sc.bvhw && tn.lds_wide && wide_lds_bytes(sc) + dl <= kFusedLdsLimit;
@@ -101,6 +116,13 @@
     p.n_top = (unsigned)std::min<size_t>(n_nodes, (room - used()) / 64);
   }
   p.dyn = used();
+  p.threads = kTraceBlock;
+  if (p.lane == kLaneWideLds && coresident == 1 && coresident_lds_fits(p.lane, p.dyn, kCoBlocksA)) {
+    p.threads = kTraceBlockCo;
+    p.coresident = 1;
+  } else if (p.lane == kLaneWideLds && coresident == 2 && coresident_lds_fits(p.lane, p.dyn, kCoBlocksB)) {
+    p.coresident = 2;
+  }
   return p;
 }
 static_assert(sizeof(BvhNode) == 64 && sizeof(BvhWide16) == 64, "wf_plan_image: a treelet node is 64 B");
```

New measurement: 19020 Mrays/s, median of 6. 1.01x the previous value.
